# IamJerryXu/Multimodal-Diagnosis-HAM-Spine

Hardware: AMD Instinct MI355X
Metric: training images/sec, ResNet50+BERT-base 224px bs32 (higher is better)
Workload: dtype bf16; 1 GPU; C2: ResNet50 + BERT-base(L=128) + cross-attention FusionModule + MLP head, 224x224, batch 32 per GPU, CE(label_smoothing=0.02), fused AdamW, train-mode BatchNorm and dropout; per_gpu_batch=32, global_batch=32, seq_len=128, params=134897991, parallelism=dp1

## Files before the change

### include/hamspine.h

```cpp
#ifndef HAMSPINE_H
#define HAMSPINE_H

#include <stdint.h>

#ifdef __cplusplus
extern "C" {
#endif

typedef int hs_status;
enum { HS_OK = 0, HS_ERR_ARG = 1, HS_ERR_HIP = 2, HS_ERR_UNSUPPORTED = 3 };
enum { HS_F32 = 0, HS_BF16 = 1 };

const char* hs_last_error(void);
int hs_version(void);
int hs_device_ok(void);


enum {
    HS_A_KC = 0,
    HS_A_RC = 1,
    HS_A_CONV = 2,
    HS_A_DGRAD = 3
};
enum {
// ... 113 lines not shown
    const void* y;
    const void* x;
    const float* gamma;
    const float* save_mean;
    const float* save_invstd;
    void* dx;
    void* dres;
    float* dgamma;
    float* dbeta;
    void* ws;
    int64_t ws_bytes;
    const float* scale;
    const float* shift;
    int32_t partial_rows;
    int32_t sums_done;
} hs_bn_bwd_params;

hs_status hs_batchnorm_fwd(const hs_bn_params* p, void* stream);
hs_status hs_batchnorm_bwd(const hs_bn_bwd_params* p, void* stream);
int64_t hs_batchnorm_ws_bytes(int64_t M, int32_t C, int32_t dtype);

hs_status hs_layernorm_fwd(int32_t dtype, const void* x, const float* gamma, const float* beta, void* y,
                           float* mean, float* rstd, int64_t M, int32_t H, float eps, void* stream);
hs_status hs_layernorm_bwd(int32_t dtype, const void* dy, const void* x, const float* gamma, const float* mean,
                           const float* rstd, void* dx, float* dgamma, float* dbeta, void* ws, int64_t ws_bytes,
                           int64_t M, int32_t H, void* stream);
hs_status hs_layernorm_bwd_pre(int32_t dtype, const void* dy, const void* x, const float* gamma, const float* mean,
                               const float* rstd, void* dx, float* dgamma, float* dbeta, void* dx_dropped, float* dbias,
                               float dropout_p, uint64_t seed, void* ws, int64_t ws_bytes, int64_t M, int32_t H, void* stream);
int64_t hs_layernorm_bwd_ws_bytes(int64_t M, int32_t H);

#define HS_CAST_MAX 48
#define HS_ADAM_MAX 32

hs_status hs_maxpool_fwd(int32_t dtype, const void* x, void* y, void* idx, int32_t N, int32_t H, int32_t W, int32_t C,
                         int32_t ksize, int32_t stride, int32_t pad, void* stream);
hs_status hs_maxpool_bwd(int32_t dtype, const void* dy, const void* idx, void* dx, int32_t N, int32_t H, int32_t W,
                         int32_t C, int32_t ksize, int32_t stride, int32_t pad, void* stream);
hs_status hs_mean_tokens_fwd(int32_t dtype, const void* x, void* y, int32_t B, int32_t Nt, int32_t H, int32_t out_f32,
                             void* stream);
hs_status hs_mean_tokens_bwd(int32_t dtype, const void* dy, void* dx, int32_t B, int32_t Nt, int32_t H, int32_t dy_f32,
                             void* stream);
hs_status hs_pack_image(int32_t dtype, const float* x, void* y, int32_t N, int32_t Cin, int32_t H, int32_t W, int32_t Hp,
                        int32_t Wp, int32_t pad, void* stream);
hs_status hs_pack_stem_weight(int32_t dtype, const float* w, void* out, int32_t K, int32_t R, int32_t S, int32_t Cin,
                              void* stream);
hs_status hs_unpack_stem_wgrad(const float* g, float* dw, int32_t K, int32_t R, int32_t S, int32_t Cin, void* stream);
hs_status hs_cast_f32_to_bf16_multi(int32_t count, const float* const* src, void* const* dst, const int64_t* n,
                                    void* stream);
hs_status hs_transpose_bf16(const void* src, void* dst, int32_t R, int32_t C, int64_t ld_src, int64_t ld_dst, void* stream);
#define HS_TRANSPOSE_MAX 8
hs_status hs_transpose_bf16_multi(int32_t count, const void* const* src, void* const* dst, const int32_t* R, const int32_t* C,
                                  const int64_t* ld_src, const int64_t* ld_dst, void* stream);
hs_status hs_axpby(int32_t in_dtype, int32_t out_dtype, const void* x, const void* y, void* out, int64_t n, float a,
                   float b, void* stream);
hs_status hs_dropout(int32_t dtype, const void* x, void* out, int64_t n, float p, uint64_t seed, void* stream);
hs_status hs_relu_fwd(int32_t dtype, const void* x, void* out, int64_t n, void* stream);
hs_status hs_relu_bwd(int32_t dtype, const void* dy, const void* y, void* dx, int64_t n, void* stream);
hs_status hs_gelu_bwd(int32_t dtype, const void* dy, const void* u, void* dx, int64_t n, void* stream);
hs_status hs_mul_dev_scalar(const float* x, const float* scalar, float* out, int64_t n, void* stream);
hs_status hs_colsum(int32_t dtype, const void* x, int64_t M, int32_t N, int32_t ld, float* out, void* ws,
                    int64_t ws_bytes, int32_t accumulate, void* stream);
int64_t hs_colsum_ws_bytes(int64_t M, int32_t N);
hs_status hs_softmax_fwd(int32_t dtype, const float* S, const int64_t* mask, void* P, void* P_drop, int64_t rows,
                         int32_t Lk, int32_t ldS, int32_t ldP, int32_t rows_per_batch, float dropout_p, uint64_t seed,
                         void* stream);
hs_status hs_softmax_bwd(int32_t dtype, const float* dP, const void* P, void* dS, int64_t rows, int32_t Lk, int32_t ldG,
                         int32_t ldP, float dropout_p, uint64_t seed, void* stream);
hs_status hs_bert_embed_fwd(int32_t dtype, const int64_t* ids, const float* word, const float* pos, const float* type0,
                            const float* gamma, const float* beta, void* sum_out, void* y, float* mean, float* rstd,
                            int64_t tokens, int32_t L, int32_t H, int32_t V, float eps, float dropout_p, uint64_t seed,
                            void* stream);
hs_status hs_bert_embed_bwd(int32_t dtype, const int64_t* ids, const void* dsum, float* dword, float* dpos, int32_t B,
                            int32_t L, int32_t H, int32_t V, int32_t pad_id, void* stream);
hs_status hs_cross_entropy(const float* logits, const int64_t* labels, const float* weight, float label_smoothing,
                           int32_t B, int32_t C, float* loss, float* dlogits, float* row_loss, void* stream);
hs_status hs_adam_step_multi(int32_t count, float* const* params, const float* const* grads, float* const* exp_avg,
                             float* const* exp_avg_sq, const int64_t* n, float lr, float beta1, float beta2, float eps,
                             float weight_decay, int32_t step, int32_t decoupled, float grad_scale, void* stream);
hs_status hs_adam_step_multi_shadow(int32_t count, float* const* params, const float* const* grads, float* const* exp_avg,
                                    float* const* exp_avg_sq, void* const* bf16_shadow, const int64_t* n, float lr, float beta1,
                                    float beta2, float eps, float weight_decay, int32_t step, int32_t decoupled,
                                    float grad_scale, void* stream);
hs_status hs_wgrad_group_begin(void* stream);
hs_status hs_wgrad_group_end(void* stream);
hs_status hs_weight_shadow_set(const float* w, void* bf16);
void hs_weight_shadow_clear(void);

hs_status hs_sgd_step_multi(int32_t count, float* const* params, const float* const* grads, float* const* momentum_buf,
                            const int64_t* n, float lr, float momentum, float weight_decay, int32_t nesterov, int32_t first,
                            float grad_scale, void* stream);

#define HS_MUON_MAX 32
#define HS_MUON_PARTIALS 256
hs_status hs_muon_prepare_multi(int32_t dtype, int32_t count, float* const* momentum, const float* const* grads,
                                void* const* packed, const int32_t* rows, const int32_t* cols, float beta, float* partials,
                                void* stream);
hs_status hs_muon_orthogonalize(int32_t dtype, int32_t count, int32_t rows, int32_t cols, void* X, void* ws, int64_t ws_bytes,
                                void* stream);
int64_t hs_muon_ws_bytes(int32_t dtype, int32_t count, int32_t rows, int32_t cols);
hs_status hs_muon_apply_multi(int32_t dtype, int32_t count, float* const* params, void* const* bf16_shadow,
                              const void* const* packed, const int32_t* rows, const int32_t* cols, const float* scale,
                              float lr, float weight_decay, void* stream);

hs_status hs_select_token_fwd(int32_t dtype, const void* x, float* out, int32_t B, int32_t Nt, int32_t H, int32_t t,
                              void* stream);
// ... 120 lines not shown
hs_status hs_kan_features_fwd(const float* x, const float* grid, float* feat, int64_t B, int32_t in_f, int32_t grid_size,
                              int32_t order, int32_t base_act, void* stream);
hs_status hs_kan_features_bwd(const float* x, const float* grid, const float* dfeat, float* dx, int64_t B, int32_t in_f,
                              int32_t grid_size, int32_t order, int32_t base_act, void* stream);
hs_status hs_kan_pack_weight(const float* base_w, const float* spline_w, const float* scaler, float* wcat, int32_t out_f,
                             int32_t in_f, int32_t nb, void* stream);
hs_status hs_kan_unpack_wgrad(const float* dwcat, const float* spline_w, const float* scaler, float* d_base, float* d_spline,
                              float* d_scaler, int32_t out_f, int32_t in_f, int32_t nb, void* stream);
hs_status hs_moe_gate_fwd(const float* clean, const float* raw_noise, const float* noise, int32_t B, int32_t E, int32_t k, int32_t noisy,
                          float noise_eps, uint64_t seed, float coef, float* gates, float* p, int32_t* top, float* z,
                          float* sigma, float* loadrow, float* loss, float* d_imp, float* d_load, void* stream);
hs_status hs_moe_gate_bwd(const float* clean, const float* raw_noise, const float* p, const int32_t* top, const float* z,
                          const float* sigma, const float* dgates, const float* g_loss, const float* d_imp,
                          const float* d_load, int32_t B, int32_t E, int32_t k, int32_t noisy, float* d_clean, float* d_raw,
                          void* stream);
hs_status hs_moe_combine_fwd(const float* gates, const float* const* outs, float* y, int32_t B, int32_t E, int32_t O,
                             void* stream);
hs_status hs_moe_combine_bwd(const float* gates, const float* const* outs, const float* dy, float* const* douts,
                             float* dgates, int32_t B, int32_t E, int32_t O, void* stream);

int32_t hs_pointwise_stat_rows(int64_t M, int32_t N, int32_t K);
hs_status hs_pointwise_fwd(const void* x, int64_t M, int32_t K, int32_t ldx, const void* w, int32_t N, void* y, int32_t ldy,
                           float* stats, void* stream);

hs_status hs_moe_dispatch_index(const float* gates, int32_t B, int32_t E, int32_t* idx, int32_t* count, void* stream);
hs_status hs_rows_gather(const float* src, const int32_t* idx, float* dst, int32_t n, int32_t D, void* stream);
hs_status hs_rows_scatter_add(float* dst, const int32_t* idx, const float* scale, int32_t ld_scale, int32_t col, const float* src,
                              int32_t n, int32_t D, void* stream);
hs_status hs_rows_scatter_add_bwd(const float* dy, const int32_t* idx, const float* gates, int32_t E, int32_t col, const float* src,
                                  float* dsrc, float* dgates, int32_t n, int32_t D, void* stream);


typedef struct hs_attn_desc {
    int32_t dtype;
    int32_t B, H, Lq, Lk, hd;
    int64_t q_bs, k_bs, v_bs, o_bs;
    int32_t q_ld, k_ld, v_ld, o_ld;
    float scale;
    float dropout_p;
    uint64_t seed;
    const int64_t* key_mask;
} hs_attn_desc;
hs_status hs_attention_query(const hs_attn_desc* d, int64_t* saved_bytes, int64_t* ws_bytes);
hs_status hs_attention_fwd(const hs_attn_desc* d, const void* q, const void* k, const void* v, void* o, void* saved,
                           int64_t saved_bytes, void* ws, int64_t ws_bytes, void* stream);
hs_status hs_attention_bwd(const hs_attn_desc* d, const void* q, const void* k, const void* v, const void* d_o, void* dq,
                           void* dk, void* dv, void* saved, int64_t saved_bytes, void* ws, int64_t ws_bytes,
                           void* stream);

void hs_set_overlap(int32_t on);
hs_status hs_grad_milestones(int32_t n, const void* const* grad_ptrs, void* const* events);
int32_t hs_measure_build(void);
void hs_set_wgrad_nt(int32_t on);

typedef struct hs_conv_bn {
    int32_t Cin, Cout, R, stride, pad;
    const float* w;
    const float* gamma;
    const float* beta;
    float* running_mean;
    float* running_var;
    float* dw;
    float* dgamma;
    float* dbeta;
} hs_conv_bn;

typedef struct hs_resblock_desc {
    int32_t dtype;
    int32_t N, H, W;
    int32_t training;
    float eps, momentum;
    int32_t n_main;
    hs_conv_bn main[3];
    int32_t has_ds;
    hs_conv_bn ds;
    int32_t inference;
} hs_resblock_desc;
hs_status hs_resblock_query(const hs_resblock_desc* d, int64_t* saved_bytes, int64_t* ws_bytes);
hs_status hs_resblock_fwd(const hs_resblock_desc* d, const void* x, void* y, void* saved, int64_t saved_bytes, void* ws,
                          int64_t ws_bytes, void* stream);
hs_status hs_resblock_bwd(const hs_resblock_desc* d, const void* x, const void* y, const void* dy, void* dx, void* saved,
                          int64_t saved_bytes, void* ws, int64_t ws_bytes, void* stream);

typedef struct hs_stem_desc {
    int32_t dtype;
    int32_t N, H, W;
    int32_t training;
    float eps, momentum;
    hs_conv_bn cb;
    int32_t inference;
} hs_stem_desc;
hs_status hs_stem_query(const hs_stem_desc* d, int64_t* saved_bytes, int64_t* ws_bytes);
hs_status hs_stem_fwd(const hs_stem_desc* d, const float* image, void* y, void* saved, int64_t saved_bytes, void* ws,
                      int64_t ws_bytes, void* stream);
hs_status hs_stem_bwd(const hs_stem_desc* d, const void* y, const void* dy, void* saved, int64_t saved_bytes, void* ws,
                      int64_t ws_bytes, void* stream);

typedef struct hs_linear {
    int32_t in_f, out_f;
    const float* w;
    const float* b;
    float* dw;
    float* db;
} hs_linear;
typedef struct hs_norm {
    const float* gamma;
// ... 98 lines not shown
```

### multimodal-diagnosis-ham-spine_amd/hamspine/_lib.py

```python
import ctypes as C
import os
import re

_HERE = os.path.dirname(os.path.abspath(__file__))
LIB_PATH = os.path.join(_HERE, "libhamspine_hip.so")
HEADER_PATH = os.path.normpath(os.path.join(_HERE, "..", "..", "include", "hamspine.h"))

HS_OK = 0
HS_F32, HS_BF16 = 0, 1
A_KC, A_RC, A_CONV, A_DGRAD = 0, 1, 2, 3
B_KC, B_RC, B_WDGRAD, B_CONV = 0, 1, 2, 3
ACT_NONE, ACT_RELU, ACT_GELU = 0, 1, 2
MUL_NONE, MUL_GELU_GRAD, MUL_RELU_MASK = 0, 1, 2
CAST_MAX, ADAM_MAX = 48, 32
MUON_MAX, MUON_PARTIALS = 32, 256

i32, i64, u64, f32, vp = C.c_int32, C.c_int64, C.c_uint64, C.c_float, C.c_void_p


class HamspineError(RuntimeError):
    pass


class ConvGeom(C.Structure):
# ... 242 lines not shown
    l.hs_selective_scan_ws_bytes.argtypes = [i32, i32, i32]
    l.hs_selective_scan_ws_bytes.restype = i64
    l.hs_selective_scan_chunk_len.argtypes = []
    l.hs_selective_scan_chunk_len.restype = i32
    l.hs_selective_scan_chunk_len_n.argtypes = [i32]
    l.hs_selective_scan_chunk_len_n.restype = i32
    l.hs_selective_scan_ws_bytes_n.argtypes = [i32, i32, i32, i32]
    l.hs_selective_scan_ws_bytes_n.restype = i64
    l.hs_selective_scan_chunk_len_nogate.argtypes = [i32]
    l.hs_selective_scan_chunk_len_nogate.restype = i32
    l.hs_selective_scan_ws_bytes_nogate.argtypes = [i32, i32, i32, i32]
    l.hs_selective_scan_ws_bytes_nogate.restype = i64
    l.hs_conv1d_same_silu_fwd.argtypes = [i32, vp, i32, vp, vp, vp, i32, i32, i32, i32, i32, vp]
    l.hs_conv1d_same_silu_bwd.argtypes = [i32, vp, i32, vp, i32, vp, vp, vp, i32, vp, vp, vp, i64, i32, i32, i32, i32, vp]
    l.hs_conv1d_same_silu_ws_bytes.argtypes = [i32, i32]
    l.hs_conv1d_same_silu_ws_bytes.restype = i64
    l.hs_window_partition.argtypes = [i32, vp, vp, i32, i32, i32, i32, i32, vp]
    l.hs_window_reverse.argtypes = [i32, vp, vp, i32, i32, i32, i32, i32, vp]
    l.hs_conv3x3_fwd.argtypes = [i32, vp, vp, vp, vp, i32, i32, i32, i32, i32, i32, i32, i32, vp]
    l.hs_conv3x3_dgrad.argtypes = [i32, vp, vp, vp, i32, i32, i32, i32, i32, i32, i32, i32, vp]
    l.hs_conv3x3_pack_filter.argtypes = [i32, vp, vp, vp, i32, i32, i32, i32, vp]
    l.hs_conv3x3_unpack_wgrad.argtypes = [vp, vp, i32, i32, i32, vp]
    l.hs_pack_image_nhwc.argtypes = [i32, vp, vp, i32, i32, i32, i32, i32, vp]
    l.hs_unpack_image_nhwc.argtypes = [i32, vp, vp, i32, i32, i32, i32, i32, vp]
    l.hs_bn_gelu_tanh_fwd.argtypes = [i32, vp, vp, vp, vp, i64, i32, i32, vp]
    l.hs_bn_scale_residual_fwd.argtypes = [i32, vp, vp, vp, vp, vp, vp, vp, i64, i32, i32, i64, vp]
    l.hs_bn_epilogue_bwd.argtypes = [i32, i32, vp, vp, vp, vp, vp, vp, vp, vp, vp, vp, vp, vp, vp, vp, i32, i64, i32, i32, i64, vp, i64, vp]
    l.hs_bn_epilogue_ws_bytes.argtypes = [i64, i32]
    l.hs_bn_epilogue_ws_bytes.restype = i64
    l.hs_window_partition_nhwc.argtypes = [i32, vp, vp, i32, i32, i32, i32, i32, i32, vp]
    l.hs_window_reverse_nhwc.argtypes = [i32, vp, vp, i32, i32, i32, i32, i32, i32, vp]
    l.hs_add_token_bias_fwd.argtypes =[i32, vp, vp, vp, i32, i32, i32, vp]
    l.hs_add_token_bias_bwd.argtypes = [i32, vp, vp, i32, i32, i32, vp]
    l.hs_token_seq_assemble_fwd.argtypes = [vp, vp, vp, vp, vp, vp, i32, i32, i32, vp]
    l.hs_token_seq_assemble_bwd.argtypes = [vp, vp, vp, vp, vp, i32, i32, i32, vp]
    l.hs_transpose_batched_f32.argtypes = [vp, vp, i32, i32, i32, vp]
    l.hs_concat2_t.argtypes = [i32, vp, i32, vp, i32, vp, i64, vp]
    l.hs_split2_t.argtypes = [i32, vp, vp, i32, vp, i32, i64, vp]
    l.hs_prof_calibrate.argtypes = [vp, i32, C.POINTER(C.c_float)]
    l.hs_tta_expand.argtypes = [vp, vp, i64, i32, i32, P(i32), i32, vp]
    l.hs_group_mean.argtypes = [vp, vp, i32, i64, vp]
    l.hs_repeat.argtypes = [i32, vp, vp, i64, i32, vp]
    l.hs_gradcam.argtypes = [i32, vp, vp, vp, i32, i32, i32, vp]
    l.hs_stage_images_u8.argtypes = [vp, vp, i32, i32, i32, P(f32), P(f32), vp]
    l.hs_set_overlap.restype = None
    l.hs_grad_milestones.argtypes = [i32, P(vp), P(vp)]
    l.hs_pointwise_stat_rows.argtypes = [i64, i32, i32]
    l.hs_pointwise_stat_rows.restype = i32
    l.hs_pointwise_fwd.argtypes = [vp, i64, i32, i32, vp, i32, vp, i32, vp, vp]
    l.hs_measure_build.argtypes = []
    l.hs_measure_build.restype = i32
    l.hs_set_wgrad_nt.argtypes = [i32]
    l.hs_set_wgrad_nt.restype = None
    l.hs_bert_pack_rows_available.argtypes = []
    l.hs_bert_pack_rows_available.restype = i32
    l.hs_dwconv_ws_bytes.argtypes = [i32] * 5
    l.hs_dwconv_ws_bytes.restype = i64
    l.hs_dwconv_fwd.argtypes = [i32, vp, vp, vp, vp, i32, i32, i32, i32, i32, vp, i64, vp]
    l.hs_dwconv_bwd.argtypes = [i32, vp, vp, vp, vp, vp, vp, i32, i32, i32, i32, i32, vp, i64, vp]
    l.hs_layerscale_fwd.argtypes = [i32, vp, vp, vp, i32, vp, vp, i64, i32, vp]
    l.hs_layerscale_bwd.argtypes = [i32, vp, vp, vp, vp, i32, vp, vp, vp, i64, i64, i32, vp]
    l.hs_layerscale_ws_bytes.argtypes = [i64, i32]
    l.hs_layerscale_ws_bytes.restype = i64
    l.hs_patchify_fwd.argtypes = [i32, vp, vp, i32, i32, i32, i32, i32, i32, vp]
    l.hs_patchify_bwd.argtypes = [i32, vp, vp, i32, i32, i32, i32, i32, i32, vp]


ABI_STRUCTS = None


def abi_structs():
    return [(0, ConvGeom), (1, GemmParams), (2, BnParams), (3, BnBwdParams), (4, AttnDesc), (5, ConvBn), (6, ResblockDesc),
            (7, StemDesc), (8, Linear), (9, Norm), (10, BertLayerDesc), (11, ResnetDesc), (12, ResnetPlan), (13, BertDesc)]


def check(status, what=""):
    if status != HS_OK:
        msg = lib().hs_last_error().decode("utf-8", "replace")
        raise HamspineError(f"{what} failed (status {status}): {msg}")


def exported_symbols():
    txt = open(HEADER_PATH).read()
    txt = re.sub(r"/\*.*?\*/", "", txt, flags=re.S)
    return sorted(set(re.findall(r"\b(hs_[a-z0-9_]+)\s*\(", txt)))
```

### multimodal-diagnosis-ham-spine_amd/hamspine/csrc/blocks.hip

```cpp
#include <algorithm>
#include <mutex>
#include <unordered_map>
#include <vector>
#include <stdlib.h>
#include "hs_common.h"
#include "pw_stream.h"

namespace hs {

__global__ __launch_bounds__(256) void gather3_kernel(const float* __restrict__ a, const float* __restrict__ b,
                                                      const float* __restrict__ c, float* __restrict__ dst, int n) {
    const int i = blockIdx.x * 256 + threadIdx.x;
    if (i >= 3 * n) return;
    const int w = i / n, k = i - w * n;
    dst[i] = w == 0 ? a[k] : (w == 1 ? b[k] : c[k]);
}

int gemm_impl(const hs_gemm_params* p, hipStream_t stream);
int gemm_stat_rows(const hs_gemm_params* p);
int gemm_bn_finish_rows(const hs_gemm_params* p);
int gemm_tile_rows(const hs_gemm_params* p);
int gemm_bnb_finish_rows(const hs_gemm_params* p);
void gemm_group_set_immediate_hook(int (*fn)(void*), void* ctx);
struct GemmGroup;
GemmGroup* gemm_group_open(hipStream_t s, long long slot);
int gemm_group_add(GemmGroup* g, const hs_gemm_params* p, hipStream_t s);
int gemm_group_flush(GemmGroup* g, hipStream_t s);
bool fused_attention_enabled();
int attention_bwd_fused(const hs_attn_desc& d, const void* q, const void* k, const void* v, const void* dO, void* dq, void* dk,
                        void* dv, const void* P, int ldP, void* scratch, long long scratch_bytes, const void* O, hipStream_t s,
                        const int* cu);
int attention_fwd_fused(const hs_attn_desc& d, const void* q, const void* k, const void* v, void* o, void* P, void* Pd, int ldP,
                        hipStream_t s, const int* cu);
int ln_fwd(int dtype, const void* x, const float* gamma, const float* beta, void* y, float* mean, float* rstd, long long M, int H,
           float eps, hipStream_t s, const int* nrows);
int ln_bwd(int dtype, const void* dy, const void* x, const float* gamma, const float* mean, const float* rstd, void* dx, float* dgamma,
           float* dbeta, float* ws, long long ws_bytes, long long M, int H, hipStream_t s, const int* inv);
int ln_bwd_pre(int dtype, const void* dy, const void* x, const float* gamma, const float* mean, const float* rstd, void* dx,
               float* dgamma, float* dbeta, void* dx_dropped, float* dbias, float p, unsigned long long seed, float* ws,
               long long ws_bytes, long long M, int H, hipStream_t s, const int* inv);
int transpose_bf16_multi_rows(int count, const void* const* src, void* const* dst, const int32_t* R, const int32_t* Cc,
                              const int64_t* ld_src, const int64_t* ld_dst, const int* inv, const unsigned char* tok, hipStream_t stream);
int colsum_rows(int dtype, const void* x, long long M, int N, int ld, float* out, void* ws, long long ws_bytes, int accumulate,
                const int* inv, hipStream_t s);
int dropout_rows(int dtype, const void* x, void* out, long long M, int H, float p, unsigned long long seed, const int* nrows,
                 const int* row_of, hipStream_t s);
long long bert_row_map_bytes(int B, int L);
int bert_row_map(const int64_t* mask, int B, int L, int* map, hipStream_t s);
int bert_unpack_rows(const void* y, void* out, long long rows, long long row_bytes, const int* packed_of, hipStream_t s);
int bert_pack_rows(const void* dy, void* dst, long long rows, long long row_bytes, const int* nrows, const int* row_of,
                   hipStream_t s);
int bert_embed_fwd_rows(int dtype, const int64_t* ids, const float* word, const float* pos, const float* type0, const float* gamma,
                        const float* beta, void* sum_out, void* y, float* mean, float* rstd, long long tokens, int L, int H, int V,
                        float eps, float dropout_p, unsigned long long seed, const int* nrows, const int* row_of, hipStream_t stream);
int bert_embed_bwd_rows(int dtype, const int64_t* ids, const void* dsum, float* dword, float* dpos, int B, int L, int H, int V,
                        int pad_id, const int* nrows, const int* row_of, const int* packed_of, hipStream_t s);

static inline long long align_up(long long v, long long a) { return (v + a - 1) / a * a; }
static inline int esize(int dt) { return dt == HS_BF16 ? 2 : 4; }

struct Arena {
    char* base = nullptr;
    long long cap = 0, off = 0, peak = 0;
    bool plan = false;
    bool overflow = false;
    void* alloc(long long bytes) {
        bytes = align_up(bytes > 0 ? bytes : 1, 256);
        char* p = base ? base + off : nullptr;
        off += bytes;
        if (off > peak) peak = off;
        if (!plan && off > cap) overflow = true;
        return plan ? nullptr : p;
    }
    long long mark() const { return off; }
    void release(long long m) { off = m; }
};

struct Run {
    hipStream_t s;
    int dt;
    bool plan;
    Arena saved, ws;
    hipStream_t side = nullptr;
    bool side_used = false;
    bool defer_wgrad = false;
    GemmGroup *grp_pw = nullptr, *grp_conv = nullptr;
    bool group_nt = false;
    GemmGroup* grp_nt = nullptr;
    GemmGroup* tower_grp = nullptr;
    struct PendTr { const void* src; void* dst; int R, C; long long ld; bool tok; };
    std::vector<PendTr> pend_tr;
    const int *pk_T = nullptr, *pk_cu = nullptr, *pk_row = nullptr, *pk_inv = nullptr;
};

static hipStream_t g_side_stream[16] = {};
static hipEvent_t g_events[16][64] = {};
static int g_event_next[16] = {};
static std::mutex g_side_mu;
static int g_overlap = -1;
static bool overlap_enabled() {
    if (g_overlap < 0) {
        const char* e = getenv("HAMSPINE_OVERLAP");
        g_overlap = (e && e[0] == '1') ? 1 : 0;
    }
    return g_overlap == 1;
}
static int side_setup(Run& r) {
    if (r.plan || !overlap_enabled()) return HS_OK;
    int dev = 0;
    HS_CHECK_HIP(hipGetDevice(&dev));
    if (dev < 0 || dev >= 16) return HS_OK;
    std::lock_guard<std::mutex> lk(g_side_mu);
    if (!g_side_stream[dev]) HS_CHECK_HIP(hipStreamCreateWithFlags(&g_side_stream[dev], hipStreamNonBlocking));
    r.side = g_side_stream[dev];
    return HS_OK;
}
static int next_event(hipEvent_t* ev) {
    int dev = 0;
    HS_CHECK_HIP(hipGetDevice(&dev));
    std::lock_guard<std::mutex> lk(g_side_mu);
    int& n = g_event_next[dev & 15];
    hipEvent_t& e = g_events[dev & 15][n];
    n = (n + 1) & 63;
    if (!e) HS_CHECK_HIP(hipEventCreateWithFlags(&e, hipEventDisableTiming));
    *ev = e;
    return HS_OK;
}
template <typename F>
static int on_side(Run& r, F fn) {
    if (r.plan || !r.side) return fn();
    hipEvent_t ev;
    HS_PROPAGATE(next_event(&ev));
    HS_CHECK_HIP(hipEventRecord(ev, r.s));
    HS_CHECK_HIP(hipStreamWaitEvent(r.side, ev, 0));
    hipStream_t keep = r.s;
    r.s = r.side;
    const int st = fn();
    r.s = keep;
    r.side_used = true;
    return st;
}
static int side_join(Run& r) {
    if (r.plan || !r.side || !r.side_used) return HS_OK;
    hipEvent_t ev;
    HS_PROPAGATE(next_event(&ev));
// ... 240 lines not shown
    gk.b_elems = span_elems(d.B, d.q_bs, d.Lq, d.q_ld, d.H, d.hd);
    gk.lda = l.ldP; gk.ldb = d.q_ld;
    gk.batch = BH; gk.batch_inner = d.H;
    gk.a_bs0 = (long long)d.H * d.Lq * l.ldP; gk.a_bs1 = (long long)d.Lq * l.ldP;
    gk.b_bs0 = d.q_bs; gk.b_bs1 = d.hd;
    gk.d_bs0 = d.k_bs; gk.d_bs1 = d.hd;
    gk.D = dk; gk.ldd = d.k_ld;
    gk.alpha = d.scale;
    CALL(r, gemm_impl(&gk, r.s));
    RUN_CHECK_ARENAS(r, "attention_bwd");
    return HS_OK;
}

static int linear_fwd_run(Run& r, const void* x, long long M, int ldx, const hs_linear& lin, const void* w_c, void* y,
                          int ldy, int out_dtype, int act, void* preact, const void* residual, int ldr, float drop_p,
                          unsigned long long seed) {
    hs_gemm_params p = gemm_defaults(r.dt);
    p.a_kind = HS_A_KC; p.b_kind = HS_B_KC;
    p.M = (int)M; p.N = lin.out_f; p.K = lin.in_f;
    p.A = x; p.B = w_c;
    p.a_elems = (M - 1) * ldx + lin.in_f;
    p.b_elems = (long long)lin.out_f * lin.in_f;
    p.lda = ldx; p.ldb = lin.in_f;
    p.D = y; p.ldd = ldy; p.out_dtype = out_dtype;
    p.bias = lin.b;
    p.act = act;
    p.D_preact = preact;
    p.residual = residual; p.ldr = ldr;
    p.dropout_p = drop_p; p.dropout_seed = seed;
    p.m_rows = r.pk_T;
    p.drop_rows = drop_p > 0.f ? r.pk_row : nullptr;
    CALL(r, gemm_impl(&p, r.s));
    return HS_OK;
}
static bool fused_bias_grad_enabled() {
    static const bool on = [] {
        const char* e = getenv("HAMSPINE_FUSED_BIAS_GRAD");
        return !(e && e[0] == '0');
    }();
    return on;
}
static bool bias_in_wgrad(int dt, int out_f, int in_f, long long M) {
    return dt == HS_BF16 && fused_bias_grad_enabled() && hs_gemm_suggest_split(out_f, in_f, (int)M, dt) <= 1;
}
static std::mutex g_wg_mu;
static std::unordered_map<hipStream_t, GemmGroup*> g_wg_open;
static GemmGroup* open_wgrad_group(hipStream_t s) {
    std::lock_guard<std::mutex> lk(g_wg_mu);
    auto it = g_wg_open.find(s);
    return it == g_wg_open.end() ? nullptr : it->second;
}
static bool wgrad_nt_enabled();
static int linear_wgrad_nt_run(Run& r, const void* xT, const void* dyT, long long M, int in_f, int out_f, float* dw, float* db,
                               int seg_rows, float* const* dw_seg, float* const* db_seg);
static int linear_wgrad_run(Run& r, const void* x, long long M, int ldx, const hs_linear& lin, const void* dy, int ldy) {
    bool db_done = false;
    if (lin.dw && r.dt == HS_BF16 && wgrad_nt_enabled() && M >= 2048 && M % 8 == 0 && lin.in_f % 8 == 0 && lin.out_f % 8 == 0 &&
        ldx % 8 == 0 && ldy % 8 == 0 && ldx >= lin.in_f && ldy >= lin.out_f &&
        (long long)lin.in_f * lin.out_f >= 256ll * (lin.in_f + lin.out_f)) {
        const long long mk = r.ws.mark();
        char* tA = (char*)r.ws.alloc(M * (long long)lin.out_f * 2);
        char* tB = (char*)r.ws.alloc(M * (long long)lin.in_f * 2);
        const void* src[2] = {dy, x};
        void* dst[2] = {tA, tB};
        const int32_t R[2] = {(int32_t)M, (int32_t)M}, Cc[2] = {lin.out_f, lin.in_f};
        const int64_t lds[2] = {ldy, ldx}, ldd[2] = {M, M};
        const unsigned char tok[2] = {1, 1};
        CALLK(r, 4, transpose_bf16_multi_rows(2, src, dst, R, Cc, lds, ldd, r.pk_inv, tok, r.s));
        GemmGroup* og = r.plan ? nullptr : open_wgrad_group(r.s);
        const bool keep_flag = r.group_nt;
        GemmGroup* keep_grp = r.grp_nt;
        if (og) {
            r.group_nt = true;
            r.grp_nt = og;
        }
        const bool fused_b = lin.db && (r.group_nt || hs_gemm_suggest_split(lin.out_f, lin.in_f, (int)M, r.dt) <= 1) && fused_bias_grad_enabled();
        const int st_nt = linear_wgrad_nt_run(r, tB, tA, M, lin.in_f, lin.out_f, lin.dw, lin.db, 0, nullptr, nullptr);
        r.group_nt = keep_flag;
        r.grp_nt = keep_grp;
        HS_PROPAGATE(st_nt);
        if (lin.db && !fused_b) {
            const long long wsb = hs_colsum_ws_bytes(M, lin.out_f);
            void* w = r.ws.alloc(wsb);
            CALL(r, colsum_rows(r.dt, dy, M, lin.out_f, ldy, lin.db, w, wsb, 0, r.pk_inv, r.s));
        }
        if (!r.plan && !og && !r.side) r.ws.release(mk);
        return HS_OK;
    }
    if (lin.dw) {
        HS_REQUIRE(!r.pk_T, "linear_wgrad: packed rows need the transposed-operand weight gradients (HAMSPINE_WGRAD_NT)");
        hs_gemm_params p = gemm_defaults(r.dt);
        p.a_kind = HS_A_RC; p.b_kind = HS_B_RC;
        p.M = lin.out_f; p.N = lin.in_f; p.K = (int)M;
        p.A = dy; p.B = x;
        p.a_elems = (M - 1) * ldy + lin.out_f;
        p.b_elems = (M - 1) * ldx + lin.in_f;
        p.lda = ldy; p.ldb = ldx;
        p.D = lin.dw; p.ldd = lin.in_f; p.out_dtype = HS_F32;
        if (lin.db && bias_in_wgrad(r.dt, lin.out_f, lin.in_f, M)) {
            p.rowsum_a = lin.db;
            db_done = true;
        }
        HS_PROPAGATE(gemm_splitk(r, p));
    }
    if (lin.db && !db_done) {
        const long long mk = r.ws.mark();
        const long long wsb = hs_colsum_ws_bytes(M, lin.out_f);
        void* w = r.ws.alloc(wsb);
        CALL(r, colsum_rows(r.dt, dy, M, lin.out_f, ldy, lin.db, w, wsb, 0, r.pk_inv, r.s));
        if (r.plan ? !overlap_enabled() : !r.side) r.ws.release(mk);
    }
    return HS_OK;
}
static int g_wgrad_nt = -1;
static bool wgrad_nt_enabled() {
    if (g_wgrad_nt < 0) {
        const char* e = getenv("HAMSPINE_WGRAD_NT");
        g_wgrad_nt = (e && e[0] == '0') ? 0 : 1;
    }
    return g_wgrad_nt == 1;
}
static bool grouped_bert_wgrad_enabled() {
    static int v = -1;
    if (v < 0) {
        const char* e = getenv("HAMSPINE_GROUPED_BERT_WGRAD");
        v = (e && e[0] == '0') ? 0 : 1;
    }
    return v == 1;
}
static bool dgrad_nt_enabled() {
    static int v = -1;
    if (v < 0) {
        const char* e = getenv("HAMSPINE_DGRAD_NT");
        v = (e && e[0] == '0') ? 0 : 1;
    }
    return v == 1;
}
static bool deferred_transposes_enabled() {
    static const bool on = [] { const char* e = getenv("HAMSPINE_DEFER_TRANSPOSES"); return !(e && e[0] == '0'); }();
    return on;
}
static int transpose_run(Run& r, const void* src, void* dst, long long R, int Cc, int ld_src, bool for_grouped_wgrad = false,
                         bool tokens = false) {
    const bool tok = tokens && r.pk_T;
    if (for_grouped_wgrad && r.tower_grp && r.group_nt && !r.plan && deferred_transposes_enabled()) {
        r.pend_tr.push_back(Run::PendTr{src, dst, (int)R, Cc, ld_src, tok});
        return HS_OK;
    }
    if (tok) {
        const void* s1[1] = {src};
        void* d1[1] = {dst};
        const int32_t R1[1] = {(int32_t)R}, C1[1] = {Cc};
        const int64_t ls[1] = {ld_src}, ldst[1] = {R};
        const unsigned char t1[1] = {1};
        CALLK(r, 4, transpose_bf16_multi_rows(1, s1, d1, R1, C1, ls, ldst, r.pk_inv, t1, r.s));
        return HS_OK;
    }
    CALLK(r, 4, hs_transpose_bf16(src, dst, (int)R, Cc, ld_src, R, r.s));
    return HS_OK;
}
static int pending_transposes_flush(Run& r) {
    const int n = (int)r.pend_tr.size();
    if (n == 0) return HS_OK;
    std::vector<const void*> src(n);
    std::vector<void*> dst(n);
    std::vector<int32_t> R(n), Cc(n);
    std::vector<int64_t> lds(n), ldd(n);
    std::vector<unsigned char> tok(n);
    for (int i = 0; i < n; ++i) {
        src[i] = r.pend_tr[i].src; dst[i] = r.pend_tr[i].dst; R[i] = r.pend_tr[i].R; Cc[i] = r.pend_tr[i].C;
        lds[i] = r.pend_tr[i].ld; ldd[i] = r.pend_tr[i].R;
        tok[i] = r.pend_tr[i].tok ? 1 : 0;
    }
    r.pend_tr.clear();
    CALLK(r, 4, transpose_bf16_multi_rows(n, src.data(), dst.data(), R.data(), Cc.data(), lds.data(), ldd.data(), r.pk_inv, tok.data(), r.s));
    return HS_OK;
}
static int linear_wgrad_nt_run(Run& r, const void* xT, const void* dyT, long long M, int in_f, int out_f, float* dw, float* db,
                               int seg_rows, float* const* dw_seg, float* const* db_seg) {
    hs_gemm_params p = gemm_defaults(r.dt);
    p.a_kind = HS_A_KC; p.b_kind = HS_B_KC;
    p.M = out_f; p.N = in_f; p.K = (int)M;
    p.A = dyT; p.B = xT;
    p.a_elems = (long long)out_f * M;
    p.b_elems = (long long)in_f * M;
    p.lda = (int)M; p.ldb = (int)M;
    p.D = dw; p.ldd = in_f; p.out_dtype = HS_F32;
    if (seg_rows > 0) {
        p.seg_rows = seg_rows;
        p.D_seg[0] = dw_seg[0];
        p.D_seg[1] = dw_seg[1];
    }
    if (db && (r.group_nt || hs_gemm_suggest_split(out_f, in_f, (int)M, r.dt) <= 1) && fused_bias_grad_enabled()) {
        p.rowsum_a = db;
        if (seg_rows > 0) {
            p.rowsum_seg[0] = db_seg[0];
            p.rowsum_seg[1] = db_seg[1];
        }
    }
    if (r.group_nt) {
        if (!r.plan && !(knock() & 2)) HS_PROPAGATE(gemm_group_add(r.grp_nt, &p, r.s));
        return HS_OK;
    }
    if (!r.plan && (knock() & 2)) { const int sp = hs_gemm_suggest_split(p.M, p.N, p.K, p.dtype); p.split_k = sp; if (sp > 1) (void)r.ws.alloc(hs_gemm_splitk_ws_bytes(&p)); return HS_OK; }
    return gemm_splitk(r, p);
}
static int linear_dgrad_run(Run& r, const hs_linear& lin, const void* w_c, const void* dy, long long M, int ldy, void* dx,
                            int lddx, int dx_dtype, int mul_mode, const void* mul_src, int ldm, const void* residual,
                            const void* w_t = nullptr) {
    hs_gemm_params p = gemm_defaults(r.dt);
    p.a_kind = HS_A_KC; p.b_kind = HS_B_RC;
    p.M = (int)M; p.N = lin.in_f; p.K = lin.out_f;
    p.A = dy; p.B = w_c;
    p.a_elems = (M - 1) * ldy + lin.out_f;
    p.b_elems = (long long)lin.out_f * lin.in_f;
    p.lda = ldy; p.ldb = lin.in_f;
    long long mk = -1;
    if (!w_t && r.dt == HS_BF16 && dgrad_nt_enabled() && lin.out_f >= 1536 && M >= 2048 && lin.in_f % 8 == 0 && lin.out_f % 8 == 0) {
        mk = r.ws.mark();
        char* wt = (char*)r.ws.alloc((long long)lin.in_f * lin.out_f * 2);
        HS_PROPAGATE(transpose_run(r, w_c, wt, lin.out_f, lin.in_f, lin.in_f));
        w_t = wt;
    }
    if (w_t) {
        p.b_kind = HS_B_KC;
        p.B = w_t;
        p.ldb = lin.out_f;
    }
    p.D = dx; p.ldd = lddx; p.out_dtype = dx_dtype;
    p.mul_mode = mul_mode; p.mul_src = mul_src; p.ldm = ldm;
    p.residual = residual; p.ldr = lddx;
    p.m_rows = r.pk_T;
    CALLK(r, 1024, gemm_impl(&p, r.s));
    if (mk >= 0 && (r.plan ? !overlap_enabled() : !r.side)) r.ws.release(mk);
    return HS_OK;
}

struct ConvShape {
    int N, H, W, Cin, Cout, R, stride, pad, P, Q;
};
static ConvShape conv_shape(int N, int H, int W, const hs_conv_bn& c) {
    ConvShape s;
    s.N = N; s.H = H; s.W = W; s.Cin = c.Cin; s.Cout = c.Cout; s.R = c.R; s.stride = c.stride; s.pad = c.pad;
    s.P = (H + 2 * c.pad - c.R) / c.stride + 1;
    s.Q = (W + 2 * c.pad - c.R) / c.stride + 1;
    return s;
}
static hs_conv_geom geom_of(const ConvShape& s) {
    hs_conv_geom g;
    memset(&g, 0, sizeof(g));
    g.N = s.N; g.H = s.H; g.W = s.W; g.C = s.Cin; g.P = s.P; g.Q = s.Q; g.K = s.Cout; g.R = s.R; g.S = s.R;
    g.stride = s.stride; g.pad = s.pad;
    g.row_pitch = s.W * s.Cin;
    g.img_pitch = s.H * g.row_pitch;
// ... 680 lines not shown
    CALL(r, ln_fwd(r.dt, L.h2, d.ln2.gamma, d.ln2.beta, y, L.mean2, L.rstd2, M, Hd, d.ln_eps, r.s, r.pk_T));
    RUN_CHECK_ARENAS(r, "bert_layer_fwd");
    return HS_OK;
}
static int bert_layer_bwd_run(Run& r, const hs_bert_layer_desc& d, const void* x, const void* dy, void* dx) {
    BertLayout L;
    HS_PROPAGATE(bert_layout(r, d, L));
    const int Hd = d.hidden, I = d.inter;
    const long long M = (long long)d.B * d.L;
    const int es = esize(r.dt);
    hs_attn_desc a = bert_attn_desc(d, r.dt);
    void* dh2 = r.ws.alloc(M * Hd * es);
    void* dd2 = r.ws.alloc(M * Hd * es);
    void* dh1 = r.ws.alloc(M * Hd * es);
    void* dd1 = r.ws.alloc(M * Hd * es);
    void* du = r.ws.alloc(M * I * es);
    void* dx1 = r.ws.alloc(M * Hd * es);
    void* dctx = r.ws.alloc(M * Hd * es);
    void* dqkv = r.ws.alloc(M * 3 * Hd * es);
    const long long ln_ws_bytes = hs_layernorm_bwd_ws_bytes(M, Hd);
    float* ln_ws = (float*)r.ws.alloc(ln_ws_bytes);
    float* scratch = (float*)r.ws.alloc(2ll * Hd * 4);
    HS_PROPAGATE(side_setup(r));

    const bool fuse_ln = fused_ln_bwd_enabled();
    const void* g2 = d.hidden_dropout > 0.f ? dd2 : dh2;
    hs_linear out_l_w = d.out_l;
    if (fuse_ln) {
        CALL(r, ln_bwd_pre(r.dt, dy, L.h2, d.ln2.gamma, L.mean2, L.rstd2, dh2, d.ln2.dgamma ? d.ln2.dgamma : scratch,
                           d.ln2.dbeta ? d.ln2.dbeta : (scratch ? scratch + Hd : nullptr),
                           d.hidden_dropout > 0.f ? dd2 : nullptr, d.out_l.db, d.hidden_dropout, d.seed * 8 + 3,
                           ln_ws, ln_ws_bytes, M, Hd, r.s, r.pk_inv));
        out_l_w.db = nullptr;
    } else {
        CALLK(r, 128, ln_bwd(r.dt, dy, L.h2, d.ln2.gamma, L.mean2, L.rstd2, dh2, d.ln2.dgamma ? d.ln2.dgamma : scratch,
                             d.ln2.dbeta ? d.ln2.dbeta : (scratch ? scratch + Hd : nullptr), ln_ws, ln_ws_bytes, M, Hd, r.s, r.pk_inv));
        if (d.hidden_dropout > 0.f && r.pk_T) CALL(r, dropout_rows(r.dt, dh2, dd2, M, Hd, d.hidden_dropout, d.seed * 8 + 3, r.pk_T, r.pk_row, r.s));
        else if (d.hidden_dropout > 0.f) CALL(r, hs_dropout(r.dt, dh2, dd2, M * Hd, d.hidden_dropout, d.seed * 8 + 3, r.s));
    }
    const bool nt = r.dt == HS_BF16 && wgrad_nt_enabled() && M % 8 == 0 && Hd % 8 == 0 && I % 8 == 0;
    HS_REQUIRE(!r.pk_T || nt, "bert_layer_bwd: packed rows need the transposed-operand weight gradients (bf16, HAMSPINE_WGRAD_NT on)");
    const long long big_tiles = (long long)ceil_div(3 * Hd, 256) * ceil_div(Hd, 128) + (long long)ceil_div(Hd, 256) * ceil_div(Hd, 128) +
                                (long long)ceil_div(I, 256) * ceil_div(Hd, 128) + (long long)ceil_div(Hd, 256) * ceil_div(I, 128);
    const bool grouped = nt && grouped_bert_wgrad_enabled() && !overlap_enabled() && big_tiles >= 128;
    char* tA = nt ? (char*)r.ws.alloc(M * (long long)std::max(3 * Hd, I) * 2) : nullptr;
    char* tA_ffn2 = grouped ? (char*)r.ws.alloc(M * (long long)Hd * 2) : tA;
    char* tA_ao = grouped ? (char*)r.ws.alloc(M * (long long)Hd * 2) : tA;
    char* tA_qkv = grouped ? (char*)r.ws.alloc(M * 3ll * Hd * 2) : tA;
    r.group_nt = grouped;
    if (grouped && !r.plan) {
        r.grp_nt = r.tower_grp ? r.tower_grp : gemm_group_open(r.s, (long long)(uintptr_t)d.q.w + 16);
        HS_REQUIRE(r.grp_nt != nullptr, "bert_layer_bwd: cannot set up the grouped weight-gradient launch");
    }
    char* tX_g = nt ? (char*)r.ws.alloc(M * (long long)I * 2) : nullptr;
    char* tX_x1 = nt ? (char*)r.ws.alloc(M * (long long)Hd * 2) : nullptr;
    char* tX_ctx = nt ? (char*)r.ws.alloc(M * (long long)Hd * 2) : nullptr;
    char* tX_x = nt ? (char*)r.ws.alloc(M * (long long)Hd * 2) : nullptr;
    auto bias_by_colsum = [&](const hs_linear& lin, const void* dy_rm, int ldy) -> int {
        hs_linear only_b = lin;
        only_b.dw = nullptr;
        return linear_wgrad_run(r, nullptr, M, 0, only_b, dy_rm, ldy);
    };
    auto wgrad = [&](const void* x_rm, const void* xT, int in_f, const hs_linear& lin, const void* dy_rm, int ldy, char* tAk) -> int {
        if (!nt || !lin.dw) {
            const bool keep = r.group_nt;
            r.group_nt = false;
            const int st = linear_wgrad_run(r, x_rm, M, in_f, lin, dy_rm, ldy);
            r.group_nt = keep;
            return st;
        }
        HS_PROPAGATE(transpose_run(r, dy_rm, tAk, M, lin.out_f, ldy, true, true));
        const bool fused_b = lin.db && (r.group_nt || hs_gemm_suggest_split(lin.out_f, in_f, (int)M, r.dt) <= 1) && fused_bias_grad_enabled();
        HS_PROPAGATE(linear_wgrad_nt_run(r, xT, tAk, M, in_f, lin.out_f, lin.dw, lin.db, 0, nullptr, nullptr));
        if (lin.db && !fused_b) HS_PROPAGATE(bias_by_colsum(lin, dy_rm, ldy));
        return HS_OK;
    };
    const bool dnt = r.dt == HS_BF16 && dgrad_nt_enabled() && Hd % 8 == 0 && I % 8 == 0;
    char* wo_t = dnt ? (char*)r.ws.alloc((long long)Hd * I * 2) : nullptr;
    char* wi_t = dnt ? (char*)r.ws.alloc((long long)Hd * I * 2) : nullptr;
    char* wqkv_t = dnt ? (char*)r.ws.alloc(3ll * Hd * Hd * 2) : nullptr;
    {
        const void* src[7];
        void* dst[7];
        int32_t R[7], Cc[7];
        int64_t lds[7], ldd[7];
        unsigned char tok[7];
        int n = 0;
        auto add = [&](const void* s_, void* d_, long long rows, int cols, bool tokens = false) {
            src[n] = s_; dst[n] = d_; R[n] = (int32_t)rows; Cc[n] = cols; lds[n] = cols; ldd[n] = rows; tok[n] = tokens ? 1 : 0;
            ++n;
        };
        if (nt) {
            add(L.g, tX_g, M, I, true);
            add(L.x1, tX_x1, M, Hd, true);
            add(L.ctx, tX_ctx, M, Hd, true);
            add(x, tX_x, M, Hd, true);
        }
        if (dnt) {
            add(L.wo, wo_t, Hd, I);
            add(L.wi, wi_t, I, Hd);
            add(L.wqkv, wqkv_t, 3 * Hd, Hd);
        }
        if (n > 0) CALLK(r, 4, transpose_bf16_multi_rows(n, src, dst, R, Cc, lds, ldd, r.pk_inv, tok, r.s));
    }
    HS_PROPAGATE(on_side(r, [&]() { return wgrad(L.g, tX_g, I, out_l_w, g2, Hd, tA_ffn2); }));
    HS_PROPAGATE(linear_dgrad_run(r, d.out_l, L.wo, g2, M, Hd, du, I, r.dt, HS_MUL_GELU_GRAD, L.u, I, nullptr, wo_t));
    HS_PROPAGATE(on_side(r, [&]() { return wgrad(L.x1, tX_x1, Hd, d.inter_l, du, I, tA); }));
    HS_PROPAGATE(linear_dgrad_run(r, d.inter_l, L.wi, du, M, I, dx1, Hd, r.dt, HS_MUL_NONE, nullptr, 0, dh2, wi_t));
    const void* g1 = d.hidden_dropout > 0.f ? dd1 : dh1;
    hs_linear ao_w = d.ao;
    if (fuse_ln) {
        CALL(r, ln_bwd_pre(r.dt, dx1, L.h1, d.ln1.gamma, L.mean1, L.rstd1, dh1, d.ln1.dgamma ? d.ln1.dgamma : scratch,
                           d.ln1.dbeta ? d.ln1.dbeta : (scratch ? scratch + Hd : nullptr),
                           d.hidden_dropout > 0.f ? dd1 : nullptr, d.ao.db, d.hidden_dropout, d.seed * 8 + 2,
                           ln_ws, ln_ws_bytes, M, Hd, r.s, r.pk_inv));
        ao_w.db = nullptr;
    } else {
        CALLK(r, 128, ln_bwd(r.dt, dx1, L.h1, d.ln1.gamma, L.mean1, L.rstd1, dh1, d.ln1.dgamma ? d.ln1.dgamma : scratch,
                             d.ln1.dbeta ? d.ln1.dbeta : (scratch ? scratch + Hd : nullptr), ln_ws, ln_ws_bytes, M, Hd, r.s, r.pk_inv));
        if (d.hidden_dropout > 0.f && r.pk_T) CALL(r, dropout_rows(r.dt, dh1, dd1, M, Hd, d.hidden_dropout, d.seed * 8 + 2, r.pk_T, r.pk_row, r.s));
        else if (d.hidden_dropout > 0.f) CALL(r, hs_dropout(r.dt, dh1, dd1, M * Hd, d.hidden_dropout, d.seed * 8 + 2, r.s));
    }
    HS_PROPAGATE(on_side(r, [&]() { return wgrad(L.ctx, tX_ctx, Hd, ao_w, g1, Hd, tA_ao); }));
    HS_PROPAGATE(linear_dgrad_run(r, d.ao, L.wao, g1, M, Hd, dctx, Hd, r.dt, HS_MUL_NONE, nullptr, 0, nullptr));
    const char* qkv = (const char*)L.qkv;
    char* dq = (char*)dqkv;
    HS_PROPAGATE(attention_bwd_run(r, a, qkv, qkv ? qkv + (long long)Hd * es : nullptr, qkv ? qkv + 2ll * Hd * es : nullptr,
                                   dctx, dq, dq ? dq + (long long)Hd * es : nullptr, dq ? dq + 2ll * Hd * es : nullptr, L.ctx));
    HS_PROPAGATE(on_side(r, [&]() -> int {
        const bool fused = d.q.dw && d.k.dw && d.v.dw;
        if (fused && nt) {
            HS_PROPAGATE(transpose_run(r, dqkv, tA_qkv, M, 3 * Hd, 3 * Hd, true, true));
            const bool bias_too = d.q.db && d.k.db && d.v.db && (r.group_nt || hs_gemm_suggest_split(3 * Hd, Hd, (int)M, r.dt) <= 1) &&
                                  fused_bias_grad_enabled();
            float* dws[2] = {d.k.dw, d.v.dw};
            float* dbs[2] = {d.k.db, d.v.db};
            HS_PROPAGATE(linear_wgrad_nt_run(r, tX_x, tA_qkv, M, Hd, 3 * Hd, d.q.dw, bias_too ? d.q.db : nullptr, Hd, dws, dbs));
            if (bias_too) return HS_OK;
            const hs_linear* lins[3] = {&d.q, &d.k, &d.v};
            for (int i = 0; i < 3; ++i) HS_PROPAGATE(bias_by_colsum(*lins[i], dq ? dq + (long long)i * Hd * es : nullptr, 3 * Hd));
            return HS_OK;
        }
        if (fused) {
            hs_gemm_params p = gemm_defaults(r.dt);
            p.a_kind = HS_A_RC; p.b_kind = HS_B_RC;
            p.M = 3 * Hd; p.N = Hd; p.K = (int)M;
            p.A = dqkv; p.B = x;
            p.a_elems = M * 3 * Hd;
            p.b_elems = M * Hd;
            p.lda = 3 * Hd; p.ldb = Hd;
            p.D = d.q.dw; p.ldd = Hd; p.out_dtype = HS_F32;
            p.seg_rows = Hd;
            p.D_seg[0] = d.k.dw;
            p.D_seg[1] = d.v.dw;
            const bool bias_too = d.q.db && d.k.db && d.v.db && bias_in_wgrad(r.dt, 3 * Hd, Hd, M);
            if (bias_too) {
                p.rowsum_a = d.q.db;
                p.rowsum_seg[0] = d.k.db;
                p.rowsum_seg[1] = d.v.db;
            }
            HS_PROPAGATE(gemm_splitk(r, p));
            if (bias_too) return HS_OK;
        }
        const hs_linear* lins[3] = {&d.q, &d.k, &d.v};
        for (int i = 0; i < 3; ++i) {
            hs_linear li = *lins[i];
            if (fused) li.dw = nullptr;
            HS_PROPAGATE(linear_wgrad_run(r, x, M, Hd, li, dq ? dq + (long long)i * Hd * es : nullptr, 3 * Hd));
        }
        return HS_OK;
    }));
    if (dx) {
        hs_linear qkv_lin;
        memset(&qkv_lin, 0, sizeof(qkv_lin));
        qkv_lin.in_f = Hd; qkv_lin.out_f = 3 * Hd;
        HS_PROPAGATE(linear_dgrad_run(r, qkv_lin, L.wqkv, dqkv, M, 3 * Hd, dx, Hd, r.dt, HS_MUL_NONE, nullptr, 0, dh1, wqkv_t));
    }
    if (r.group_nt && !r.plan && !r.tower_grp) HS_PROPAGATE(gemm_group_flush(r.grp_nt, r.s));
    r.group_nt = false;
    HS_PROPAGATE(side_join(r));
    RUN_CHECK_ARENAS(r, "bert_layer_bwd");
    return HS_OK;
}


static long long out_bytes_of(const hs_resblock_desc& d, int dt, int* Cout, int* Ho, int* Wo) {
    int H = d.H, W = d.W;
    for (int i = 0; i < d.n_main; ++i) {
        const hs_conv_bn& c = d.main[i];
        H = (H + 2 * c.pad - c.R) / c.stride + 1;
        W = (W + 2 * c.pad - c.R) / c.stride + 1;
    }
    const int C = d.main[d.n_main - 1].Cout;
    if (Cout) *Cout = C;
    if (Ho) *Ho = H;
    if (Wo) *Wo = W;
    return (long long)d.N * H * W * C * esize(dt);
}
struct ResnetLayout {
    long long y_off[HS_RESNET_MAX_BLOCKS + 1];
    long long lay_off[HS_RESNET_MAX_BLOCKS + 1];
    long long y_bytes[HS_RESNET_MAX_BLOCKS + 1];
    long long max_act = 0;
};
static int resnet_check(const hs_resnet_desc& d) {
    HS_REQUIRE(d.n_blocks >= 1 && d.n_blocks <= HS_RESNET_MAX_BLOCKS, "resnet: n_blocks %d out of range", d.n_blocks);
    HS_REQUIRE(d.n_taps >= 1 && d.n_taps <= HS_RESNET_MAX_TAPS, "resnet: n_taps %d out of range", d.n_taps);
    for (int t = 0; t < d.n_taps; ++t)
        HS_REQUIRE(d.tap_block[t] >= 0 && d.tap_block[t] < d.n_blocks && (t == 0 || d.tap_block[t] > d.tap_block[t - 1]),
                   "resnet: tap blocks must be ascending block indices");
    HS_REQUIRE(d.tap_block[d.n_taps - 1] == d.n_blocks - 1, "resnet: the last tap must be the last block");
    for (int i = 0; i < d.n_blocks; ++i)
        HS_REQUIRE(d.blocks[i].dtype == d.stem.dtype && d.blocks[i].N == d.stem.N, "resnet: block %d dtype / batch mismatch", i);
    return HS_OK;
}
static int resnet_fwd_run(Run& r, const hs_resnet_desc& d, const float* image, ResnetLayout& lo) {
    const int dt = d.stem.dtype;
    const int es = esize(dt);
    const int P = (d.stem.H + 6 - 7) / 2 + 1, Q = (d.stem.W + 6 - 7) / 2 + 1;
    const int P2 = (P + 2 - 3) / 2 + 1, Q2 = (Q + 2 - 3) / 2 + 1;
    lo.y_off[0] = r.saved.mark();
    lo.y_bytes[0] = (long long)d.stem.N * P2 * Q2 * d.stem.cb.Cout * es;
    lo.max_act = lo.y_bytes[0];
    char* x = (char*)r.saved.alloc(lo.y_bytes[0]);
    lo.lay_off[0] = r.saved.mark();
    long long wm = r.ws.mark();
    HS_PROPAGATE(stem_fwd_run(r, d.stem, image, x));
    r.ws.release(wm);
    HS_REQUIRE(d.blocks[0].H == P2 && d.blocks[0].W == Q2 && d.blocks[0].main[0].Cin == d.stem.cb.Cout,
               "resnet: block 0 does not take the stem's output shape");
    int C = d.stem.cb.Cout, H = P2, W = Q2;
    for (int i = 0; i < d.n_blocks; ++i) {
// ... 85 lines not shown
        HS_PROPAGATE(resblock_bwd_run(r, d.blocks[i], x, y, dy, dx, nb, own_next.rows > 0 ? &own_next : nullptr));
        own_next = OwnSums{};
        if (nb && xs_rows > 0) own_next = OwnSums{xs_buf[i & 1], xs_bytes, xs_rows, xs_done};
        if (!r.defer_wgrad) r.ws.release(wm);
        if (staged) {
            const hs_resblock_desc& bd = d.blocks[i];
            for (int k = 0; k < bd.n_main; ++k) {
                seg_ptrs.push_back(bd.main[k].dw); seg_ptrs.push_back(bd.main[k].dgamma); seg_ptrs.push_back(bd.main[k].dbeta);
            }
            if (bd.has_ds) {
                seg_ptrs.push_back(bd.ds.dw); seg_ptrs.push_back(bd.ds.dgamma); seg_ptrs.push_back(bd.ds.dbeta);
            }
            if (bd.has_ds && i > 0) {
                HS_PROPAGATE(gemm_group_flush(r.grp_pw, r.s));
                HS_PROPAGATE(gemm_group_flush(r.grp_conv, r.s));
                HS_PROPAGATE(milestones_hit(r, seg_ptrs.data(), (int)seg_ptrs.size()));
                seg_ptrs.clear();
                ++seg;
                r.grp_pw = gemm_group_open(r.s, 8 + 2 * seg);
                r.grp_conv = gemm_group_open(r.s, 9 + 2 * seg);
                HS_REQUIRE(r.grp_pw && r.grp_conv, "resnet_bwd: cannot set up the grouped weight-gradient launches");
            }
        }
        dy = dx;
        cur ^= 1;
    }
    if (r.defer_wgrad && !r.plan) {
        HS_PROPAGATE(gemm_group_flush(r.grp_pw, r.s));
        HS_PROPAGATE(gemm_group_flush(r.grp_conv, r.s));
    }
    r.defer_wgrad = false;
    const hs_conv_bn& cb = d.stem.cb;
    if (cb.dw || cb.dgamma || cb.dbeta) {
        r.saved.off = lo.lay_off[0];
        const long long wm = r.ws.mark();
        HS_PROPAGATE(stem_bwd_run(r, d.stem, r.saved.base ? r.saved.base + lo.y_off[0] : nullptr, dy));
        r.ws.release(wm);
    }
    return milestones_flush(r);
}

struct BertTowerLayout {
    long long ssum_off, stats_off;
    long long y_off[HS_BERT_MAX_LAYERS + 1], lay_off[HS_BERT_MAX_LAYERS + 1];
    long long act_bytes;
    long long map_off, out_off;
};
static void bert_pack_pointers(Run& r, const hs_bert_desc& d, const BertTowerLayout& lo) {
    const int* map = (const int*)(r.saved.base + lo.map_off);
    r.pk_T = map;
    r.pk_cu = map + 4;
    r.pk_row = r.pk_cu + (d.B + 1 + 3) / 4 * 4;
    r.pk_inv = r.pk_row + (long long)d.B * d.L;
}
static int bert_check(const hs_bert_desc& d) {
    HS_REQUIRE(d.n_layers >= 0 && d.n_layers <= HS_BERT_MAX_LAYERS, "bert: n_layers %d out of range", d.n_layers);
    HS_REQUIRE(d.B > 0 && d.L > 0 && d.hidden > 0 && d.vocab > 0, "bert: bad dims");
    HS_REQUIRE(d.word && d.pos && d.type0 && d.gamma && d.beta, "bert: null embedding parameter");
    for (int i = 0; i < d.n_layers; ++i)
        HS_REQUIRE(d.layers[i].dtype == d.dtype && d.layers[i].B == d.B && d.layers[i].L == d.L && d.layers[i].hidden == d.hidden,
                   "bert: layer %d shape mismatch", i);
    if (d.pack_rows) {
        HS_REQUIRE(d.dtype == HS_BF16 && d.L <= 128 && d.hidden % 8 == 0 && ((long long)d.B * d.L) % 8 == 0, "bert: pack_rows needs bf16, L <= 128 and hidden %% 8 == 0");
        for (int i = 0; i < d.n_layers; ++i) {
            const hs_bert_layer_desc& l = d.layers[i];
            HS_REQUIRE(l.heads > 0 && d.hidden == 64 * l.heads && l.inter % 8 == 0, "bert: pack_rows needs head dim 64 (layer %d)", i);
            const int wanted = (l.q.dw != nullptr) + (l.k.dw != nullptr) + (l.v.dw != nullptr);
            HS_REQUIRE(wanted == 0 || wanted == 3, "bert: pack_rows needs the q / k / v weight gradients of layer %d all wanted or all frozen", i);
        }
    }
    return HS_OK;
}
static hs_bert_layer_desc bert_layer_of(const hs_bert_desc& d, int i, const int64_t* mask) {
    hs_bert_layer_desc l = d.layers[i];
    l.attention_mask = mask;
    l.seed = d.seed + 16ull * (unsigned)(i + 1);
    return l;
}
static int bert_fwd_run(Run& r, const hs_bert_desc& d, const int64_t* ids, const int64_t* mask, BertTowerLayout& lo) {
    const long long M = (long long)d.B * d.L;
    const int es = esize(d.dtype);
    lo.act_bytes = M * d.hidden * es;
    lo.map_off = lo.out_off = 0;
    char* out_pad = nullptr;
    if (d.pack_rows) {
        HS_REQUIRE(r.plan || mask, "bert_fwd: pack_rows needs an attention mask");
        lo.map_off = r.saved.mark();
        int* map = (int*)r.saved.alloc(bert_row_map_bytes(d.B, d.L));
        lo.out_off = r.saved.mark();
        out_pad = (char*)r.saved.alloc(lo.act_bytes);
        if (!r.plan) {
            RUN_CHECK_ARENAS(r, "bert_fwd(row map)");
            HS_PROPAGATE(bert_row_map(mask, d.B, d.L, map, r.s));
            bert_pack_pointers(r, d, lo);
        }
    }
    lo.ssum_off = r.saved.mark();
    void* ssum = r.saved.alloc(lo.act_bytes);
    lo.stats_off = r.saved.mark();
    float* stats = (float*)r.saved.alloc(2 * M * 4);
    lo.y_off[0] = r.saved.mark();
    char* x = (char*)r.saved.alloc(lo.act_bytes);
    lo.lay_off[0] = r.saved.mark();
    CALL(r, bert_embed_fwd_rows(d.dtype, ids, d.word, d.pos, d.type0, d.gamma, d.beta, ssum, x, stats, stats + M, M, d.L, d.hidden,
                                d.vocab, d.ln_eps, d.embed_dropout, d.seed, r.pk_T, r.pk_row, r.s));
    for (int i = 0; i < d.n_layers; ++i) {
        lo.y_off[i + 1] = r.saved.mark();
        char* y = (char*)r.saved.alloc(lo.act_bytes);
        lo.lay_off[i + 1] = r.saved.mark();
        const hs_bert_layer_desc l = bert_layer_of(d, i, mask);
        const long long wm = r.ws.mark();
        HS_PROPAGATE(bert_layer_fwd_run(r, l, x, y));
        r.ws.release(wm);
        x = y;
    }
    if (d.pack_rows) CALL(r, bert_unpack_rows(x, out_pad, M, (long long)d.hidden * es, r.pk_inv, r.s));
    return HS_OK;
}
static int bert_bwd_run(Run& r, const hs_bert_desc& d, const int64_t* ids, const int64_t* mask, const void* dy_in,
                        const BertTowerLayout& lo) {
    const long long M = (long long)d.B * d.L;
    const int Hd = d.hidden;
    char* dy_packed = d.pack_rows ? (char*)r.ws.alloc(lo.act_bytes) : nullptr;
    char* gbuf[2] = {(char*)r.ws.alloc(lo.act_bytes), (char*)r.ws.alloc(lo.act_bytes)};
    int cur = 0;
    const void* dy = dy_in;
    char* base = r.saved.base;
    if (d.pack_rows && !r.plan) {
        RUN_CHECK_ARENAS(r, "bert_bwd(row map)");
        bert_pack_pointers(r, d, lo);
        HS_PROPAGATE(bert_pack_rows(dy_in, dy_packed, M, (long long)Hd * esize(d.dtype), r.pk_T, r.pk_row, r.s));
        dy = dy_packed;
    }
    static const int span = [] { const char* e = getenv("HAMSPINE_WGRAD_LAYERS"); const int v = e ? atoi(e) : 2; return v >= 1 && v <= 8 ? v : 2; }();
    int pending = 0;
    long long wm = 0;
    const void* gps[8][16];
    struct HookGuard {
        explicit HookGuard(Run* rr) { gemm_group_set_immediate_hook([](void* c) -> int { return pending_transposes_flush(*(Run*)c); }, rr); }
        ~HookGuard() { gemm_group_set_immediate_hook(nullptr, nullptr); }
    } hook_guard(&r);
    for (int i = d.n_layers - 1; i >= 0; --i) {
        const hs_bert_layer_desc l = bert_layer_of(d, i, mask);
        char* dx = gbuf[cur];
        r.saved.off = lo.lay_off[i + 1];
        if (pending == 0) {
            wm = r.ws.mark();
            r.tower_grp = (span > 1 && !r.plan) ? gemm_group_open(r.s, (long long)(uintptr_t)l.q.w + 24) : nullptr;
        }
        HS_PROPAGATE(bert_layer_bwd_run(r, l, base ? base + lo.y_off[i] : nullptr, dy, dx));
        {
            const void* gp[16] = {l.q.dw, l.q.db, l.k.dw, l.k.db, l.v.dw, l.v.db, l.ao.dw, l.ao.db, l.ln1.dgamma, l.ln1.dbeta,
                                  l.inter_l.dw, l.inter_l.db, l.out_l.dw, l.out_l.db, l.ln2.dgamma, l.ln2.dbeta};
            memcpy(gps[pending], gp, sizeof(gp));
        }
        ++pending;
        if (pending == span || i == 0) {
            HS_PROPAGATE(pending_transposes_flush(r));
            if (r.tower_grp) HS_PROPAGATE(gemm_group_flush(r.tower_grp, r.s));
            r.tower_grp = nullptr;
            r.ws.release(wm);
            for (int k = 0; k < pending; ++k) HS_PROPAGATE(milestones_hit(r, gps[k], 16));
            pending = 0;
        }
        dy = dx;
        cur ^= 1;
    }
    const bool any = d.dword || d.dpos || d.dtype0 || d.dgamma || d.dbeta;
    if (!any) return milestones_flush(r);
    const void* g = dy;
    if (d.embed_dropout > 0.f) {
        char* gd = gbuf[cur];
        if (r.pk_T) CALL(r, dropout_rows(d.dtype, dy, gd, M, Hd, d.embed_dropout, d.seed, r.pk_T, r.pk_row, r.s));
        else CALL(r, hs_dropout(d.dtype, dy, gd, M * Hd, d.embed_dropout, d.seed, r.s));
        g = gd;
        cur ^= 1;
    }
    char* dsum = gbuf[cur];
    const long long lnb = hs_layernorm_bwd_ws_bytes(M, Hd);
    const long long csb = hs_colsum_ws_bytes(M, Hd);
    void* lnws = r.ws.alloc(lnb);
    void* csws = r.ws.alloc(csb);
    float* scratch = (float*)r.ws.alloc(2ll * Hd * 4);
    const float* stats = base ? (const float*)(base + lo.stats_off) : nullptr;
// ... 403 lines not shown
        HS_REQUIRE(pl.saved.peak <= saved_bytes && pl.ws.peak <= ws_bytes,
                   "bert_fwd: arena too small (saved %lld needed / %lld given, ws %lld needed / %lld given)", pl.saved.peak,
                   (long long)saved_bytes, pl.ws.peak, (long long)ws_bytes);
    }
    Run r;
    run_init(r, d->dtype, false, saved, saved_bytes, ws, ws_bytes, (hipStream_t)stream);
    HS_PROPAGATE(bert_fwd_run(r, *d, ids, mask, lo));
    RUN_CHECK_ARENAS(r, "bert_fwd");
    return HS_OK;
}
hs_status hs_bert_bwd(const hs_bert_desc* d, const int64_t* ids, const int64_t* mask, const void* dy, void* saved,
                      int64_t saved_bytes, void* ws, int64_t ws_bytes, void* stream) {
    HS_REQUIRE(d && ids && dy && saved && ws, "bert_bwd: null argument");
    HS_PROPAGATE(bert_check(*d));
    BertTowerLayout lo;
    {
        Run pl;
        run_init(pl, d->dtype, true, nullptr, 0, nullptr, 0, nullptr);
        HS_PROPAGATE(bert_fwd_run(pl, *d, nullptr, nullptr, lo));
        Run pb;
        run_init(pb, d->dtype, true, nullptr, 0, nullptr, 0, nullptr);
        HS_PROPAGATE(bert_bwd_run(pb, *d, nullptr, nullptr, nullptr, lo));
        HS_REQUIRE(pl.saved.peak <= saved_bytes && pb.ws.peak <= ws_bytes,
                   "bert_bwd: arena too small (saved %lld needed / %lld given, ws %lld needed / %lld given)", pl.saved.peak,
                   (long long)saved_bytes, pb.ws.peak, (long long)ws_bytes);
    }
    Run r;
    run_init(r, d->dtype, false, saved, saved_bytes, ws, ws_bytes, (hipStream_t)stream);
    HS_PROPAGATE(bert_bwd_run(r, *d, ids, mask, dy, lo));
    RUN_CHECK_ARENAS(r, "bert_bwd");
    return HS_OK;
}
void hs_set_overlap(int32_t on) { hs::g_overlap = on ? 1 : 0; }
int32_t hs_bert_pack_rows_available(void) { return (hs::wgrad_nt_enabled() && hs::fused_attention_enabled()) ? 1 : 0; }
hs_status hs_grad_milestones(int32_t n, const void* const* grad_ptrs, void* const* events) {
    HS_REQUIRE(n >= 0 && n <= kMaxMilestones, "grad_milestones: %d entries (max %d)", n, kMaxMilestones);
    HS_REQUIRE(n == 0 || (grad_ptrs && events), "grad_milestones: null argument");
    g_ms.n = n;
    for (int i = 0; i < n; ++i) {
        HS_REQUIRE(grad_ptrs[i] && events[i], "grad_milestones: null entry %d", i);
        g_ms.ptr[i] = grad_ptrs[i];
        g_ms.ev[i] = (hipEvent_t)events[i];
    }
    return HS_OK;
}
int32_t hs_measure_build(void) {
#ifdef HS_MEASURE
    return 1;
#else
    return 0;
#endif
}
void hs_set_wgrad_nt(int32_t on) { hs::g_wgrad_nt = on ? 1 : 0; }
}
```

### multimodal-diagnosis-ham-spine_amd/hamspine/csrc/elem.hip

```cpp
#include <algorithm>
#include "hs_common.h"

namespace hs {

static inline int grid_for(long long n, int cap = 4096) {
    long long b = (n + 255) / 256;
    if (b > cap) b = cap;
    if (b < 1) b = 1;
    return (int)b;
}

template <typename T>
__global__ __launch_bounds__(256) void maxpool_fwd_kernel(const T* __restrict__ x, T* __restrict__ y,
                                                          unsigned char* __restrict__ idx, int N, int H, int W, int C,
                                                          int P, int Q, int ks, int st, int pad) {
    constexpr int E = Chunk<T>::N;
    const int cg = C / E;
    const long long total = (long long)N * P * Q * cg;
    for (long long i = (long long)blockIdx.x * 256 + threadIdx.x; i < total; i += (long long)gridDim.x * 256) {
        const int c = (int)(i % cg);
        long long t = i / cg;
        const int q = (int)(t % Q);
        t /= Q;
        const int p = (int)(t % P);
// ... 643 lines not shown
        if (lane >= o) incl += up;
    }
    if (lane == 63) s_wave[wv] = incl;
    __syncthreads();
    int off = incl - c;
    for (int w = 0; w < wv; ++w) off += s_wave[w];
    const int n = s_wave[0] + s_wave[1] + s_wave[2] + s_wave[3];
    for (int i = lo; i < hi; ++i)
        if (id_at(i) == id) s_list[off++] = i;
    __syncthreads();
    if (s_list[0] != t) return;
    for (int h = threadIdx.x; h < H; h += 256) {
        float acc = 0.f;
        for (int k = 0; k < n; ++k) acc += to_f32(dsum[(long long)s_list[k] * H + h]);
        dword[id * H + h] = acc;
    }
}
template <typename T>
__global__ __launch_bounds__(256) void embed_word_bwd_atomic_kernel(const long long* __restrict__ ids,
                                                                    const T* __restrict__ dsum, float* __restrict__ dword,
                                                                    long long tokens_pad, int H, int V, int pad_id,
                                                                    const int* __restrict__ nrows, const int* __restrict__ row_of) {
    const long long total = packed_rows(nrows, tokens_pad) * H;
    for (long long i = (long long)blockIdx.x * 256 + threadIdx.x; i < total; i += (long long)gridDim.x * 256) {
        const long long t = i / H;
        const int h = (int)(i % H);
        long long srow = row_of ? (long long)row_of[t] : t;
        if (srow < 0 || srow >= tokens_pad) srow = t;
        const long long id = clamp_id(ids[srow], V);
        if (id == pad_id) continue;
        atomicAdd(dword + id * H + h, to_f32(dsum[i]));
    }
}
template <typename T>
__global__ __launch_bounds__(256) void embed_pos_bwd_kernel(const T* __restrict__ dsum, float* __restrict__ dpos, int B,
                                                            int L, int H, const int* __restrict__ packed_of) {
    const long long total = (long long)L * H;
    for (long long i = (long long)blockIdx.x * 256 + threadIdx.x; i < total; i += (long long)gridDim.x * 256) {
        float acc = 0.f;
        if (packed_of) {
            const int l = (int)(i / H), h = (int)(i - (long long)l * H);
            for (int b = 0; b < B; ++b) {
                const int pr = packed_of[(long long)b * L + l];
                if (pr >= 0 && pr < B * L) acc += to_f32(dsum[(long long)pr * H + h]);
            }
        } else {
            for (int b = 0; b < B; ++b) acc += to_f32(dsum[(long long)b * L * H + i]);
        }
        dpos[i] = acc;
    }
}

__global__ __launch_bounds__(256) void bert_row_map_kernel(const long long* __restrict__ mask, int B, int L, int* __restrict__ map) {
    int* cu = map + 4;
    int* row_of = cu + (B + 1 + 3) / 4 * 4;
    int* packed_of = row_of + (long long)B * L;
    const int lane = threadIdx.x & 63, wave = threadIdx.x >> 6;
    for (int b = wave; b < B; b += 4) {
        int n = 0;
        for (int l0 = 0; l0 < L; l0 += 64) {
            const int l = l0 + lane;
            const bool v = l < L && mask[(long long)b * L + l] != 0;
            n += __popcll(__ballot(v));
        }
        if (lane == 0) cu[b + 1] = n;
    }
    __syncthreads();
    if (threadIdx.x == 0) {
        int run = 0;
        cu[0] = 0;
        for (int b = 0; b < B; ++b) {
            run += cu[b + 1];
            cu[b + 1] = run;
        }
        map[0] = run;
        map[1] = map[2] = map[3] = 0;
    }
    __syncthreads();
    const int T = cu[B];
    for (int b = wave; b < B; b += 4) {
        int at = cu[b];
        for (int l0 = 0; l0 < L; l0 += 64) {
            const int l = l0 + lane;
            const bool v = l < L && mask[(long long)b * L + l] != 0;
            const unsigned long long bal = __ballot(v);
            const int before = __popcll(bal & ((1ull << lane) - 1ull));
            if (l < L) {
                if (v) {
                    row_of[at + before] = b * L + l;
                    packed_of[(long long)b * L + l] = at + before;
                } else {
                    packed_of[(long long)b * L + l] = -1;
                }
            }
            at += __popcll(bal);
        }
    }
    for (int t = T + (int)threadIdx.x; t < B * L; t += 256) row_of[t] = t;
}
__global__ __launch_bounds__(256) void bert_unpack_rows_kernel(const u32x4* __restrict__ y, u32x4* __restrict__ out, long long rows, int cpr,
                                                               const int* __restrict__ packed_of) {
    const long long total = rows * cpr;
    for (long long i = (long long)blockIdx.x * 256 + threadIdx.x; i < total; i += (long long)gridDim.x * 256) {
        const long long r = i / cpr;
        const int pr = packed_of[r];
        u32x4 v = {0u, 0u, 0u, 0u};
        if (pr >= 0 && pr < rows) v = y[(long long)pr * cpr + (i - r * cpr)];
        out[i] = v;
    }
}
__global__ __launch_bounds__(256) void bert_pack_rows_kernel(const u32x4* __restrict__ dy, u32x4* __restrict__ dst, long long rows, int cpr,
                                                             const int* __restrict__ nrows, const int* __restrict__ row_of) {
    const long long T = packed_rows(nrows, rows), total = T * cpr;
    for (long long i = (long long)blockIdx.x * 256 + threadIdx.x; i < total; i += (long long)gridDim.x * 256) {
        const long long t = i / cpr;
        long long srow = row_of[t];
        if (srow < 0 || srow >= rows) srow = t;
        dst[i] = dy[srow * cpr + (i - t * cpr)];
    }
}

__device__ __forceinline__ void transpose_bf16_tile(const unsigned short* __restrict__ src, unsigned short* __restrict__ dst,
                                                    int R, int Cc, long long lds_, long long ldd, int bx, int by,
                                                    unsigned (*tile)[33], const int* __restrict__ inv) {
    const int r0 = by * 64, c0 = bx * 64;
    for (int i = threadIdx.x; i < 512; i += 256) {
        const int r = i >> 3, ch = i & 7;
        u32x4 v = {0u, 0u, 0u, 0u};
        int sr = r0 + r;
        if (inv && sr < R) {
            sr = inv[sr];
            if (sr >= R) sr = -1;
        }
        if (sr >= 0 && sr < R && c0 + ch * 8 < Cc) v = *(const u32x4*)(src + (long long)sr * lds_ + c0 + ch * 8);
#pragma unroll
        for (int w = 0; w < 4; ++w) tile[r][(ch * 4 + w) ^ ((r >> 5) << 2)] = v[w];
    }
    __syncthreads();
    for (int i = threadIdx.x; i < 512; i += 256) {
        const int j = i >> 3, k = i & 7;
        if (c0 + j >= Cc || r0 + k * 8 >= R) continue;
        unsigned e[8];
#pragma unroll
        for (int q = 0; q < 8; ++q) {
            const unsigned w = tile[k * 8 + q][(j >> 1) ^ (((k * 8 + q) >> 5) << 2)];
            e[q] = (j & 1) ? (w >> 16) : (w & 0xffffu);
        }
        const u32x4 o = {e[0] | (e[1] << 16), e[2] | (e[3] << 16), e[4] | (e[5] << 16), e[6] | (e[7] << 16)};
        *(u32x4*)(dst + (long long)(c0 + j) * ldd + r0 + k * 8) = o;
    }
}
__global__ __launch_bounds__(256) void transpose_bf16_kernel(const unsigned short* __restrict__ src,
                                                             unsigned short* __restrict__ dst, int R, int Cc, long long lds_,
                                                             long long ldd) {
    __shared__ unsigned tile[64][33];
    transpose_bf16_tile(src, dst, R, Cc, lds_, ldd, blockIdx.x, blockIdx.y, tile, nullptr);
}
struct TransposeTable {
    const unsigned short* src[HS_TRANSPOSE_MAX];
    unsigned short* dst[HS_TRANSPOSE_MAX];
    int R[HS_TRANSPOSE_MAX], C[HS_TRANSPOSE_MAX];
    long long ld_src[HS_TRANSPOSE_MAX], ld_dst[HS_TRANSPOSE_MAX];
    int first[HS_TRANSPOSE_MAX + 1];
    int count;
    const int* inv;
    unsigned tok_mask;
};
__global__ __launch_bounds__(256) void transpose_bf16_multi_kernel(const TransposeTable t) {
    __shared__ unsigned tile[64][33];
    int e = 0;
    for (int i = 1; i < t.count; ++i) e += (int)blockIdx.x >= t.first[i];
    const int local = blockIdx.x - t.first[e];
    const int tx = (t.C[e] + 63) / 64;
    const int* inv = (t.inv && ((t.tok_mask >> e) & 1u)) ? t.inv : nullptr;
    transpose_bf16_tile(t.src[e], t.dst[e], t.R[e], t.C[e], t.ld_src[e], t.ld_dst[e], local % tx, local / tx, tile, inv);
}

__global__ __launch_bounds__(1024) void ce_kernel(const float* __restrict__ logits, const long long* __restrict__ labels,
                                                 const float* __restrict__ weight, float smoothing, int B, int C,
                                                 float* __restrict__ loss_out, float* __restrict__ dlogits,
                                                 float* __restrict__ row_loss) {
    __shared__ float s_num[16], s_den[16];
    const int lane = threadIdx.x & 63, wv = threadIdx.x >> 6, nwv = blockDim.x >> 6;
    float num = 0.f, den = 0.f;
    for (int r = wv; r < B; r += nwv) {
        const float* z = logits + (long long)r * C;
        float mx = -INFINITY;
        for (int c = lane; c < C; c += 64) mx = fmaxf(mx, z[c]);
        mx = wave_max(mx);
        float se = 0.f;
        for (int c = lane; c < C; c += 64) se += __expf(z[c] - mx);
        const float lse = mx + __logf(wave_sum(se));
        const int y = (int)labels[r];
        const float wy = weight ? weight[y] : 1.f;
        float sm = 0.f;
        for (int c = lane; c < C; c += 64) sm += (weight ? weight[c] : 1.f) * (lse - z[c]);
        sm = wave_sum(sm);
        const float l = (1.f - smoothing) * wy * (lse - z[y]) + smoothing / (float)C * sm;
        if (lane == 0 && row_loss) row_loss[r] = l;
        num += l;
        den += wy;
    }
    if (lane == 0) {
        s_num[wv] = num;
        s_den[wv] = den;
    }
    __syncthreads();
    float tn = 0.f, td = 0.f;
    for (int w = 0; w < nwv; ++w) {
        tn += s_num[w];
        td += s_den[w];
    }
    if (threadIdx.x == 0) loss_out[0] = tn / td;
    if (!dlogits) return;
    for (int r = wv; r < B; r += nwv) {
        const float* z = logits + (long long)r * C;
        float mx = -INFINITY;
        for (int c = lane; c < C; c += 64) mx = fmaxf(mx, z[c]);
        mx = wave_max(mx);
        float se = 0.f;
        for (int c = lane; c < C; c += 64) se += __expf(z[c] - mx);
        const float inv = 1.f / wave_sum(se);
        const int y = (int)labels[r];
        const float wy = weight ? weight[y] : 1.f;
        float wsum = 0.f;
        for (int c = lane; c < C; c += 64) wsum += weight ? weight[c] : 1.f;
        wsum = wave_sum(wsum);
        for (int c = lane; c < C; c += 64) {
// ... 155 lines not shown
    if (direct) return HS_OK;
    hipLaunchKernelGGL(colsum_final_kernel, dim3(ceil_div(N, 64)), dim3(256), 0, s, ws, gy, N, out, accumulate);
    HS_LAUNCH_CHECK();
    return HS_OK;
}

static inline int softmax_group(int Lk, int ldP) {
    if (Lk % 4 || ldP % 4 || ldP > 256) return 0;
    const int need = ldP / 4;
    return need <= 16 ? 16 : (need <= 32 ? 32 : 64);
}
template <typename T>
static int softmax_fwd_t(const float* S, const long long* mask, void* P, void* Pd, long long rows, int Lk, int ldS,
                         int ldP, int rpb, float p, unsigned long long seed, hipStream_t s) {
    HS_REQUIRE(Lk <= 64 * SM_MAXV && ldP <= 64 * SM_MAXV, "softmax: Lk=%d too long (max %d)", Lk, 64 * SM_MAXV);
    const unsigned th = p > 0.f ? dropout_thresh(p) : 0u;
    const float ik = p > 0.f ? 1.f / (1.f - p) : 1.f;
    const int G = (ldS % 4 == 0 && ((((uintptr_t)S) | ((uintptr_t)P) | ((uintptr_t)Pd)) & 15) == 0) ? softmax_group(Lk, ldP) : 0;
#define SM_FWD(GG)                                                                                                       \
    hipLaunchKernelGGL((softmax_fwd_vec_kernel<T, GG>), dim3(ceil_div(rows, 4 * (64 / GG))), dim3(256), 0, s, S, mask, (T*)P, \
                       (T*)Pd, rows, Lk, ldS, ldP, rpb, th, ik, seed)
    if (G == 16) SM_FWD(16);
    else if (G == 32) SM_FWD(32);
    else if (G == 64) SM_FWD(64);
    else
        hipLaunchKernelGGL(softmax_fwd_kernel<T>, dim3(ceil_div(rows, 4)), dim3(256), 0, s, S, mask, (T*)P, (T*)Pd, rows, Lk,
                           ldS, ldP, rpb, th, ik, seed);
#undef SM_FWD
    HS_LAUNCH_CHECK();
    return HS_OK;
}
template <typename T>
static int softmax_bwd_t(const float* dP, const void* P, void* dS, long long rows, int Lk, int ldG, int ldP, float p,
                         unsigned long long seed, hipStream_t s) {
    HS_REQUIRE(Lk <= 64 * SM_MAXV && ldP <= 64 * SM_MAXV, "softmax_bwd: Lk=%d too long", Lk);
    const unsigned th = p > 0.f ? dropout_thresh(p) : 0u;
    const float ik = p > 0.f ? 1.f / (1.f - p) : 1.f;
    const int G = (ldG % 4 == 0 && ((((uintptr_t)dP) | ((uintptr_t)P) | ((uintptr_t)dS)) & 15) == 0) ? softmax_group(Lk, ldP) : 0;
#define SM_BWD(GG)                                                                                                      \
    hipLaunchKernelGGL((softmax_bwd_vec_kernel<T, GG>), dim3(ceil_div(rows, 4 * (64 / GG))), dim3(256), 0, s, dP, (const T*)P, \
                       (T*)dS, rows, Lk, ldG, ldP, th, ik, seed)
    if (G == 16) SM_BWD(16);
    else if (G == 32) SM_BWD(32);
    else if (G == 64) SM_BWD(64);
    else
        hipLaunchKernelGGL(softmax_bwd_kernel<T>, dim3(ceil_div(rows, 4)), dim3(256), 0, s, dP, (const T*)P, (T*)dS, rows, Lk,
                           ldG, ldP, th, ik, seed);
#undef SM_BWD
    HS_LAUNCH_CHECK();
    return HS_OK;
}

int transpose_bf16_multi_rows(int count, const void* const* src, void* const* dst, const int32_t* R, const int32_t* Cc,
                              const int64_t* ld_src, const int64_t* ld_dst, const int* inv, const unsigned char* tok, hipStream_t stream) {
    HS_REQUIRE(count >= 0 && (count == 0 || (src && dst && R && Cc && ld_src && ld_dst)), "transpose_bf16_multi: bad argument");
    for (int base = 0; base < count; base += HS_TRANSPOSE_MAX) {
        TransposeTable t;
        memset(&t, 0, sizeof(t));
        t.count = std::min(HS_TRANSPOSE_MAX, count - base);
        int blocks = 0;
        for (int i = 0; i < t.count; ++i) {
            const int k = base + i;
            HS_REQUIRE(src[k] && dst[k] && R[k] > 0 && Cc[k] > 0 && R[k] % 8 == 0 && Cc[k] % 8 == 0 && ld_src[k] % 8 == 0 &&
                           ld_dst[k] % 8 == 0 && ld_src[k] >= Cc[k] && ld_dst[k] >= R[k] &&
                           (((uintptr_t)src[k] | (uintptr_t)dst[k]) & 15) == 0,
                       "transpose_bf16_multi: entry %d: dims / leading dimensions must be multiples of 8 and bases 16-byte aligned", k);
            t.src[i] = (const unsigned short*)src[k];
            t.dst[i] = (unsigned short*)dst[k];
            t.R[i] = R[k]; t.C[i] = Cc[k];
            t.ld_src[i] = ld_src[k]; t.ld_dst[i] = ld_dst[k];
            t.first[i] = blocks;
            blocks += ceil_div(Cc[k], 64) * ceil_div(R[k], 64);
            if (inv && tok && tok[k]) t.tok_mask |= 1u << i;
        }
        t.first[t.count] = blocks;
        t.inv = t.tok_mask ? inv : nullptr;
        hipLaunchKernelGGL(transpose_bf16_multi_kernel, dim3(blocks), dim3(256), 0, stream, t);
        HS_LAUNCH_CHECK();
    }
    return HS_OK;
}
int colsum_rows(int dtype, const void* x, long long M, int N, int ld, float* out, void* ws, long long ws_bytes, int accumulate,
                const int* inv, hipStream_t s) {
    HS_REQUIRE(x && out && M > 0 && N > 0, "colsum: bad argument");
    return DISPATCH_T(dtype, colsum_t, x, M, N, ld, out, (float*)ws, ws_bytes, accumulate, s, inv);
}
int dropout_rows(int dtype, const void* x, void* out, long long M, int H, float p, unsigned long long seed, const int* nrows,
                 const int* row_of, hipStream_t s) {
    HS_REQUIRE(x && out && nrows && row_of && p >= 0.f && p < 1.f, "dropout_rows: bad argument");
    HS_REQUIRE(H % 8 == 0 && al16(x, out), "dropout_rows: H %% 8 != 0 or unaligned base");
    const unsigned th = dropout_thresh(p);
    const float ik = 1.f / (1.f - p);
    if (dtype == HS_BF16)
        hipLaunchKernelGGL(dropout_rows_kernel<bf16_t>, dim3(grid_for(M * (H / 8))), dim3(256), 0, s, (const bf16_t*)x, (bf16_t*)out, M, H,
                           nrows, row_of, th, ik, seed);
    else
        hipLaunchKernelGGL(dropout_rows_kernel<float>, dim3(grid_for(M * (H / 4))), dim3(256), 0, s, (const float*)x, (float*)out, M, H,
                           nrows, row_of, th, ik, seed);
    HS_LAUNCH_CHECK();
    return HS_OK;
}
long long bert_row_map_bytes(int B, int L) { return (4ll + (B + 1 + 3) / 4 * 4 + 2ll * B * L) * 4; }
int bert_row_map(const int64_t* mask, int B, int L, int* map, hipStream_t s) {
    HS_REQUIRE(mask && map && B > 0 && L > 0, "bert_row_map: bad argument");
    hipLaunchKernelGGL(bert_row_map_kernel, dim3(1), dim3(256), 0, s, (const long long*)mask, B, L, map);
    HS_LAUNCH_CHECK();
    return HS_OK;
}
int bert_unpack_rows(const void* y, void* out, long long rows, long long row_bytes, const int* packed_of, hipStream_t s) {
    HS_REQUIRE(y && out && packed_of && row_bytes % 16 == 0 && al16(y, out), "bert_unpack_rows: bad argument");
    const int cpr = (int)(row_bytes / 16);
    hipLaunchKernelGGL(bert_unpack_rows_kernel, dim3(grid_for(rows * cpr)), dim3(256), 0, s, (const u32x4*)y, (u32x4*)out, rows, cpr, packed_of);
    HS_LAUNCH_CHECK();
    return HS_OK;
}
int bert_pack_rows(const void* dy, void* dst, long long rows, long long row_bytes, const int* nrows, const int* row_of,
                   hipStream_t s) {
    HS_REQUIRE(dy && dst && nrows && row_of && row_bytes % 16 == 0 && al16(dy, dst), "bert_pack_rows: bad argument");
    const int cpr = (int)(row_bytes / 16);
    hipLaunchKernelGGL(bert_pack_rows_kernel, dim3(grid_for(rows * cpr)), dim3(256), 0, s, (const u32x4*)dy, (u32x4*)dst, rows, cpr, nrows,
                       row_of);
    HS_LAUNCH_CHECK();
    return HS_OK;
}
int bert_embed_fwd_rows(int dtype, const int64_t* ids, const float* word, const float* pos, const float* type0, const float* gamma,
                        const float* beta, void* sum_out, void* y, float* mean, float* rstd, long long tokens, int L, int H, int V,
                        float eps, float dropout_p, unsigned long long seed, const int* nrows, const int* row_of, hipStream_t stream) {
    HS_REQUIRE(ids && word && pos && type0 && gamma && beta && sum_out && y && mean && rstd, "bert_embed: null argument");
    HS_REQUIRE(H % 4 == 0 && H <= 1024, "bert_embed: H=%d unsupported", H);
    const unsigned th = dropout_p > 0.f ? dropout_thresh(dropout_p) : 0u;
    const float ik = dropout_p > 0.f ? 1.f / (1.f - dropout_p) : 1.f;
    const dim3 g(ceil_div(tokens, 4)), b(256);
    if (dtype == HS_BF16)
        hipLaunchKernelGGL(embed_fwd_kernel<bf16_t>, g, b, 0, stream, (const long long*)ids, word, pos, type0,
                           gamma, beta, (bf16_t*)sum_out, (bf16_t*)y, mean, rstd, tokens, L, H, V, eps, th, ik, seed, nrows, row_of);
    else
        hipLaunchKernelGGL(embed_fwd_kernel<float>, g, b, 0, stream, (const long long*)ids, word, pos, type0,
                           gamma, beta, (float*)sum_out, (float*)y, mean, rstd, tokens, L, H, V, eps, th, ik, seed, nrows, row_of);
    HS_LAUNCH_CHECK();
    return HS_OK;
}
int bert_embed_bwd_rows(int dtype, const int64_t* ids, const void* dsum, float* dword, float* dpos, int B, int L, int H, int V,
                        int pad_id, const int* nrows, const int* row_of, const int* packed_of, hipStream_t s) {
    HS_REQUIRE(ids && dsum, "bert_embed_bwd: null argument");
    const long long tokens = (long long)B * L;
    if (dword) {
        const bool det = tokens <= 15360;
        const size_t lds = det ? (size_t)(tokens + 8) * sizeof(int) : 0;
        if (det && dtype == HS_BF16)
            hipLaunchKernelGGL(embed_word_bwd_kernel<bf16_t>, dim3((unsigned)tokens), dim3(256), lds, s, (const long long*)ids,
                               (const bf16_t*)dsum, dword, (int)tokens, H, V, pad_id, nrows, row_of);
        else if (det)
            hipLaunchKernelGGL(embed_word_bwd_kernel<float>, dim3((unsigned)tokens), dim3(256), lds, s, (const long long*)ids,
                               (const float*)dsum, dword, (int)tokens, H, V, pad_id, nrows, row_of);
        else if (dtype == HS_BF16)
            hipLaunchKernelGGL(embed_word_bwd_atomic_kernel<bf16_t>, dim3(grid_for(tokens * H)), dim3(256), 0, s,
                               (const long long*)ids, (const bf16_t*)dsum, dword, tokens, H, V, pad_id, nrows, row_of);
        else
            hipLaunchKernelGGL(embed_word_bwd_atomic_kernel<float>, dim3(grid_for(tokens * H)), dim3(256), 0, s,
                               (const long long*)ids, (const float*)dsum, dword, tokens, H, V, pad_id, nrows, row_of);
        HS_LAUNCH_CHECK();
    }
    if (dpos) {
        if (dtype == HS_BF16)
            hipLaunchKernelGGL(embed_pos_bwd_kernel<bf16_t>, dim3(grid_for((long long)L * H)), dim3(256), 0, s,
                               (const bf16_t*)dsum, dpos, B, L, H, packed_of);
        else
            hipLaunchKernelGGL(embed_pos_bwd_kernel<float>, dim3(grid_for((long long)L * H)), dim3(256), 0, s,
                               (const float*)dsum, dpos, B, L, H, packed_of);
        HS_LAUNCH_CHECK();
    }
    return HS_OK;
}
}
// ... 135 lines not shown
    else
        hipLaunchKernelGGL(gelu_bwd_kernel<float>, dim3(grid_for(n)), dim3(256), 0, (hipStream_t)stream, (const float*)dy,
                           (const float*)u, (float*)dx, n, (int)al16(dy, u, dx));
    HS_LAUNCH_CHECK();
    return HS_OK;
}
hs_status hs_mul_dev_scalar(const float* x, const float* scalar, float* out, int64_t n, void* stream) {
    HS_REQUIRE(x && scalar && out, "mul_dev_scalar: null argument");
    hipLaunchKernelGGL(mul_dev_scalar_kernel, dim3(grid_for(n)), dim3(256), 0, (hipStream_t)stream, x, scalar, out, n);
    HS_LAUNCH_CHECK();
    return HS_OK;
}
hs_status hs_colsum(int32_t dtype, const void* x, int64_t M, int32_t N, int32_t ld, float* out, void* ws,
                    int64_t ws_bytes, int32_t accumulate, void* stream) {
    HS_REQUIRE(x && out && M > 0 && N > 0, "colsum: bad argument");
    return DISPATCH_T(dtype, colsum_t, x, M, N, ld, out, (float*)ws, ws_bytes, accumulate, (hipStream_t)stream);
}
int64_t hs_colsum_ws_bytes(int64_t M, int32_t N) { return (int64_t)colsum_gy(M, N) * N * 4; }
hs_status hs_softmax_fwd(int32_t dtype, const float* S, const int64_t* mask, void* P, void* P_drop, int64_t rows,
                         int32_t Lk, int32_t ldS, int32_t ldP, int32_t rows_per_batch, float dropout_p, uint64_t seed,
                         void* stream) {
    HS_REQUIRE(S && P && rows > 0 && Lk > 0 && rows_per_batch > 0, "softmax: bad argument");
    return DISPATCH_T(dtype, softmax_fwd_t, S, (const long long*)mask, P, P_drop, rows, Lk, ldS, ldP, rows_per_batch,
                      dropout_p, seed, (hipStream_t)stream);
}
hs_status hs_softmax_bwd(int32_t dtype, const float* dP, const void* P, void* dS, int64_t rows, int32_t Lk, int32_t ldG,
                         int32_t ldP, float dropout_p, uint64_t seed, void* stream) {
    HS_REQUIRE(dP && P && dS && rows > 0 && Lk > 0, "softmax_bwd: bad argument");
    return DISPATCH_T(dtype, softmax_bwd_t, dP, P, dS, rows, Lk, ldG, ldP, dropout_p, seed, (hipStream_t)stream);
}
hs_status hs_bert_embed_fwd(int32_t dtype, const int64_t* ids, const float* word, const float* pos, const float* type0,
                            const float* gamma, const float* beta, void* sum_out, void* y, float* mean, float* rstd,
                            int64_t tokens, int32_t L, int32_t H, int32_t V, float eps, float dropout_p, uint64_t seed,
                            void* stream) {
    return hs::bert_embed_fwd_rows(dtype, ids, word, pos, type0, gamma, beta, sum_out, y, mean, rstd, tokens, L, H, V, eps, dropout_p,
                                   seed, nullptr, nullptr, (hipStream_t)stream);
}
hs_status hs_bert_embed_bwd(int32_t dtype, const int64_t* ids, const void* dsum, float* dword, float* dpos, int32_t B,
                            int32_t L, int32_t H, int32_t V, int32_t pad_id, void* stream) {
    return hs::bert_embed_bwd_rows(dtype, ids, dsum, dword, dpos, B, L, H, V, pad_id, nullptr, nullptr, nullptr, (hipStream_t)stream);
}
hs_status hs_transpose_bf16(const void* src, void* dst, int32_t R, int32_t Cc, int64_t ld_src, int64_t ld_dst, void* stream) {
    HS_REQUIRE(src && dst && R > 0 && Cc > 0, "transpose_bf16: bad argument");
    HS_REQUIRE(R % 8 == 0 && Cc % 8 == 0 && ld_src % 8 == 0 && ld_dst % 8 == 0 && ld_src >= Cc && ld_dst >= R &&
                   (((uintptr_t)src | (uintptr_t)dst) & 15) == 0,
               "transpose_bf16: dims / leading dimensions must be multiples of 8 and bases 16-byte aligned");
    hipLaunchKernelGGL(transpose_bf16_kernel, dim3(ceil_div(Cc, 64), ceil_div(R, 64)), dim3(256), 0, (hipStream_t)stream,
                       (const unsigned short*)src, (unsigned short*)dst, R, Cc, (long long)ld_src, (long long)ld_dst);
    HS_LAUNCH_CHECK();
    return HS_OK;
}
hs_status hs_transpose_bf16_multi(int32_t count, const void* const* src, void* const* dst, const int32_t* R, const int32_t* Cc,
                                  const int64_t* ld_src, const int64_t* ld_dst, void* stream) {
    return hs::transpose_bf16_multi_rows(count, src, dst, R, Cc, ld_src, ld_dst, nullptr, nullptr, (hipStream_t)stream);
}
hs_status hs_cross_entropy(const float* logits, const int64_t* labels, const float* weight, float label_smoothing,
                           int32_t B, int32_t C, float* loss, float* dlogits, float* row_loss, void* stream) {
    HS_REQUIRE(logits && labels && loss && B > 0 && C > 0, "cross_entropy: bad argument");
    const int waves = B >= 32 ? 16 : B >= 16 ? 8 : 4;
    hipLaunchKernelGGL(ce_kernel, dim3(1), dim3(64 * waves), 0, (hipStream_t)stream, logits, (const long long*)labels, weight,
                       label_smoothing, B, C, loss, dlogits, row_loss);
    HS_LAUNCH_CHECK();
    return HS_OK;
}
hs_status hs_sgd_step_multi(int32_t count, float* const* params, const float* const* grads, float* const* momentum_buf,
                            const int64_t* n, float lr, float momentum, float weight_decay, int32_t nesterov, int32_t first,
                            float grad_scale, void* stream) {
    HS_REQUIRE(count >= 0 && (momentum == 0.f || momentum_buf), "sgd: bad argument");
    for (int base = 0; base < count; base += HS_ADAM_MAX) {
        AdamTable t;
        memset(&t, 0, sizeof(t));
        const int cnt = std::min(HS_ADAM_MAX, count - base);
        long long mx = 0;
        for (int i = 0; i < cnt; ++i) {
            t.p[i] = params[base + i];
            t.g[i] = grads[base + i];
            t.m[i] = momentum != 0.f ? momentum_buf[base + i] : nullptr;
            t.n[i] = n[base + i];
            mx = std::max<long long>(mx, t.n[i]);
        }
        const int gx = (int)std::min<long long>(std::max<long long>((mx + 1023) / 1024, 1), 512);
        hipLaunchKernelGGL(sgd_multi_kernel, dim3(gx, cnt), dim3(256), 0, (hipStream_t)stream, t, lr, momentum, weight_decay,
                           nesterov, first, grad_scale);
        HS_LAUNCH_CHECK();
    }
    return HS_OK;
}
hs_status hs_adam_step_multi(int32_t count, float* const* params, const float* const* grads, float* const* exp_avg,
                             float* const* exp_avg_sq, const int64_t* n, float lr, float beta1, float beta2, float eps,
                             float weight_decay, int32_t step, int32_t decoupled, float grad_scale, void* stream) {
    return hs_adam_step_multi_shadow(count, params, grads, exp_avg, exp_avg_sq, nullptr, n, lr, beta1, beta2, eps, weight_decay, step,
                                     decoupled, grad_scale, stream);
}
hs_status hs_adam_step_multi_shadow(int32_t count, float* const* params, const float* const* grads, float* const* exp_avg,
                                    float* const* exp_avg_sq, void* const* bf16_shadow, const int64_t* n, float lr, float beta1,
                                    float beta2, float eps, float weight_decay, int32_t step, int32_t decoupled,
                                    float grad_scale, void* stream) {
    HS_REQUIRE(count >= 0 && step >= 1, "adam: bad argument");
    const float bc1 = 1.f - powf(beta1, (float)step);
    const float bc2s = sqrtf(1.f - powf(beta2, (float)step));
    for (int base = 0; base < count; base += HS_ADAM_MAX) {
        AdamTable t;
        memset(&t, 0, sizeof(t));
        const int cnt = std::min(HS_ADAM_MAX, count - base);
        long long mx = 0;
        for (int i = 0; i < cnt; ++i) {
            t.p[i] = params[base + i];
// ... 16 lines not shown
```

### multimodal-diagnosis-ham-spine_amd/hamspine/csrc/gemm.hip

```cpp
#include <mutex>
#include <unordered_set>
#include <vector>
#include <stdarg.h>
#include <math.h>
#include <map>
#include <tuple>
#include "gemm_launch.h"
#include "gemm_p8.h"

namespace hs {

static thread_local char g_err[512] = "";
void set_error(const char* fmt, ...) {
    va_list ap;
    va_start(ap, fmt);
    vsnprintf(g_err, sizeof(g_err), fmt, ap);
    va_end(ap);
}
const char* last_error() { return g_err; }

bool lds_attr_needed(const void* fn) {
    static std::mutex mu;
    static std::unordered_set<const void*> seen;
    std::lock_guard<std::mutex> lk(mu);
    return seen.insert(fn).second;
}

struct ProfRec {
    hipEvent_t a, b;
    double flops;
    int cls;
    int M, N, K, combo, cfg, split, batch, conv_r, conv_stride;
    double bytes = 0;
};
static std::mutex g_prof_mu;
static bool g_prof_on = false;
static std::vector<ProfRec> g_prof;
static std::vector<std::pair<hipEvent_t, hipEvent_t>> g_prof_pool;

static bool prof_begin(hipStream_t s, double flops, int cls, ProfRec& r) {
    std::lock_guard<std::mutex> lk(g_prof_mu);
    if (!g_prof_on) return false;
    if (!g_prof_pool.empty()) {
        r.a = g_prof_pool.back().first;
        r.b = g_prof_pool.back().second;
        g_prof_pool.pop_back();
    } else if (hipEventCreate(&r.a) != hipSuccess || hipEventCreate(&r.b) != hipSuccess) {
        return false;
    }
    r.flops = flops;
    r.cls = cls;
    (void)hipEventRecord(r.a, s);
// ... 51 lines not shown
    const long long z = (long long)(p->batch > 0 ? p->batch : 1) * (p->split_k > 1 ? p->split_k : 1);
    const long long t12864 = (long long)ceil_div(p->M, 128) * ceil_div(p->N, 64) * z;
    const long long t128 = (long long)ceil_div(p->M, 128) * ceil_div(p->N, 128) * z;
    if (p->dtype == HS_BF16) {
        const bool plain = (p->a_kind == HS_A_KC || p->a_kind == HS_A_RC) && (p->b_kind == HS_B_KC || p->b_kind == HS_B_RC);
        if (plain && batch_is_one(p)) {
            if (p->a_kind == HS_A_KC && p->split_k <= 1 && p->N >= 2048 && p->K <= 1024 && p->M >= 2048 && p->K % 32 == 0) return CFG_128x128x32;
            if (p->a_kind == HS_A_KC && p->b_kind == HS_B_KC && p->split_k <= 1 && p->K >= 2048 && t12864 >= 256) return CFG_128x64;
        }
        return t12864 >= 1536 ? CFG_128x64 : CFG_64x64;
    }
    return (vec && t128 >= 200) ? CFG_128x128 : CFG_64x64;
}
static bool conv3_enabled() {
    static const bool on = [] { const char* e = getenv("HAMSPINE_CONV3"); return !(e && e[0] == '0'); }();
    return on;
}
static bool conv3_plan(const hs_gemm_params* p, int* rows, int* tpi, int* fm) {
    if (!conv3_enabled() || g_dbg_cfg >= 0) return false;
    const hs_conv_geom& g = p->g;
    if (p->dtype != HS_BF16 || p->a_kind != HS_A_CONV || p->b_kind != HS_B_KC || p->split_k > 1 || p->batch > 1) return false;
    if (g.R != 3 || g.S != 3 || g.stride != 1 || g.pad != 1 || g.P != g.H || g.Q != g.W || g.C % 64 != 0 || p->N % 64 != 0) return false;
    if (g.row_pitch != g.W * g.C || g.img_pitch != g.H * g.W * g.C || g.qstep != g.C || g.no_bounds) return false;
    if (p->bias || p->colscale || p->act != HS_ACT_NONE || p->residual || p->D_preact || p->mul_mode != HS_MUL_NONE || p->dropout_p > 0.f ||
        p->accumulate || p->seg_rows > 0 || p->alpha != 1.f || p->out_dtype != HS_BF16 || p->rowsum_a || p->bnb_partials)
        return false;
    if (p->ldd % 8 != 0 || (((uintptr_t)p->D) & 15) != 0 || p->ldb != 9 * g.C || p->K != 9 * g.C || p->N != g.K) return false;
    if (g.W > 112 || g.W < 1) return false;
    const int rmax = std::min(g.H, 112 / g.W);
    const int t = ceil_div(g.H, rmax), r = ceil_div(g.H, t);
    const int tp = r * g.W;
    if (tp < 32 || (r + 2) * (g.W + 2) > 256) return false;
    *rows = r;
    *tpi = t;
    *fm = tp > 64 ? 7 : 4;
    return true;
}
int gemm_stat_rows(const hs_gemm_params* p) {
    if (!p || p->dtype != HS_BF16 || p->split_k > 1 || p->batch > 1) return 0;
    {
        int r, t, fm;
        if (conv3_plan(p, &r, &t, &fm)) return p->g.N * t;
    }
    int cfg = (p->a_kind == HS_A_CONV && p->b_kind == HS_B_KC && p->g.C % 64 != 0) ? CFG_STEM : auto_cfg(p, true);
    if (g_dbg_cfg >= 0 && g_dbg_cfg <= CFG_64x64 && cfg != CFG_STEM) cfg = g_dbg_cfg;
    if (g_dbg_cfg >= CFG_256x128 && g_dbg_cfg <= CFG_256x128x32 && !(p->a_kind == HS_A_CONV || p->a_kind == HS_A_DGRAD || p->b_kind == HS_B_CONV)) cfg = g_dbg_cfg;
    return ceil_div(p->M, cfg == CFG_64x64 ? 64 : (cfg == CFG_256x128 || cfg == CFG_256x128x32) ? 256 : 128);
}

static bool bn_finish_variant(int cfg, int combo) {
    return (combo == 0 && (cfg == CFG_64x64 || cfg == CFG_128x64)) || (combo == 3 && (cfg == CFG_64x64 || cfg == CFG_128x64 || cfg == CFG_STEM || cfg == CFG_C3));
}

struct Prepared {
    GemmArgs a;
    int cfg, combo, split, batch;
    bool bf16, conv, vec;
    dim3 grid;
    double flops;
};
static int gemm_prepare(const hs_gemm_params* p, hipStream_t stream, Prepared& q, int force_cfg = -1) {
    HS_REQUIRE(p != nullptr, "hs_gemm: null params");
    HS_REQUIRE(p->dtype == HS_F32 || p->dtype == HS_BF16, "hs_gemm: bad dtype %d", p->dtype);
    HS_REQUIRE(p->M > 0 && p->N > 0 && p->K >= 0, "hs_gemm: bad dims %d %d %d", p->M, p->N, p->K);
    HS_REQUIRE(p->A && p->B && p->D, "hs_gemm: null operand");
    const int combo = combo_of(p->a_kind, p->b_kind);
    HS_REQUIRE(combo >= 0, "hs_gemm: unsupported operand kinds (%d,%d)", p->a_kind, p->b_kind);
    const bool bf16 = p->dtype == HS_BF16;
    const int esz = bf16 ? 2 : 4, epc = bf16 ? 8 : 4;
    const int batch = p->batch > 0 ? p->batch : 1;
    const int split = p->split_k > 1 ? p->split_k : 1;
    HS_REQUIRE(!(batch > 1 && split > 1), "hs_gemm: batch and split_k are exclusive");
    HS_REQUIRE((long long)p->a_elems * esz < 0x7fffff00ll && (long long)p->b_elems * esz < 0x7fffff00ll,
               "hs_gemm: operand larger than 2 GiB");
    HS_REQUIRE(p->out_dtype == HS_F32 || p->out_dtype == p->dtype, "hs_gemm: out_dtype must be f32 or the operand type");
    HS_REQUIRE(!p->accumulate || p->out_dtype == HS_F32, "hs_gemm: accumulate needs an f32 output");

    GemmArgs a;
    memset(&a, 0, sizeof(a));
    a.A = (const char*)p->A;
    a.B = (const char*)p->B;
    a.a_bytes = (unsigned long long)p->a_elems * esz;
    a.b_bytes = (unsigned long long)p->b_elems * esz;
    a.lda = p->lda;
    a.ldb = p->ldb;
    a.M = p->M;
    a.N = p->N;
    a.K = p->K;
    a.g = p->g;
    a.batch_inner = p->batch_inner > 0 ? p->batch_inner : 1;
    a.a_bs0 = p->a_bs0; a.a_bs1 = p->a_bs1;
    a.b_bs0 = p->b_bs0; a.b_bs1 = p->b_bs1;
    a.d_bs0 = p->d_bs0; a.d_bs1 = p->d_bs1;
    a.D = (char*)p->D;
    a.ldd = p->ldd;
    a.out_f32 = p->out_dtype == HS_F32;
    a.alpha = p->alpha;
    a.bias = p->bias;
    a.act = p->act;
    a.D_preact = (char*)p->D_preact;
    a.residual = (const char*)p->residual;
    a.ldr = p->ldr;
    if (p->dropout_p > 0.f) {
        HS_REQUIRE(p->dropout_p < 1.f, "hs_gemm: dropout_p must be < 1");
        a.drop_thresh = dropout_thresh(p->dropout_p);
        a.drop_inv_keep = 1.f / (1.f - p->dropout_p);
// ... 191 lines not shown
                   "hs_gemm: bnb_finish needs bnb_partials and a launch hs_gemm_bnb_finish_rows accepts");
        HS_REQUIRE(f->C == p->N && f->M > 0 && f->dgamma && f->dbeta, "hs_gemm: bnb_finish needs the BatchNorm's C, M, dgamma, dbeta");
        HS_REQUIRE((long long)a.tiles_n * (1 + stat_groups(a.tiles_m)) <= kTicketPool, "hs_gemm: bnb_finish: too many column tiles");
        a.bnb_gamma = f->gamma; a.bnb_dgamma = f->dgamma; a.bnb_dbeta = f->dbeta;
        a.bnb_invm = 1.f / (float)f->M; a.bnb_train = f->training;
        a.bnb_tickets = ticket_pool(stream);
        HS_REQUIRE(a.bnb_tickets != nullptr, "hs_gemm: cannot allocate the arrival counters");
    }
    if (p->bn_finish) {
        const hs_bn_params* f = p->bn_finish;
        HS_REQUIRE(a.colstats && bn_finish_variant(cfg, combo), "hs_gemm: bn_finish needs colstats and a tile / layout hs_gemm_bn_finish_rows accepts");
        HS_REQUIRE(f->training && f->C == p->N && f->M == p->M && f->save_mean && f->save_invstd && f->scale && f->shift,
                   "hs_gemm: bn_finish needs a training-mode hs_bn_params of the result's shape with save_mean / save_invstd / scale / shift");
        HS_REQUIRE((long long)a.tiles_n * (1 + stat_groups(a.tiles_m)) <= kTicketPool, "hs_gemm: bn_finish: too many column tiles");
        a.bnf_gamma = f->gamma; a.bnf_beta = f->beta;
        a.bnf_rmean = f->running_var ? f->running_mean : nullptr; a.bnf_rvar = f->running_var;
        a.bnf_mean = f->save_mean; a.bnf_invstd = f->save_invstd; a.bnf_scale = f->scale; a.bnf_shift = f->shift;
        a.bnf_eps = f->eps; a.bnf_momentum = f->momentum;
        a.bnf_tickets = ticket_pool(stream);
        HS_REQUIRE(a.bnf_tickets != nullptr, "hs_gemm: cannot allocate the arrival counters");
    }
    {
        static const bool hist = [] { const char* e = getenv("HAMSPINE_EPI_HIST"); return e && e[0] == '1'; }();
        if (hist) {
            static std::mutex mu;
            static std::map<std::pair<unsigned, int>, long long> cnt;
            static const bool reg = [] {
                atexit([] {
                    for (auto& kv : cnt) fprintf(stderr, "[epi] flags 0x%05x bf16 %d : %lld launches\n", kv.first.first, kv.first.second, kv.second);
                });
                return true;
            }();
            (void)reg;
            unsigned f = 0;
            if (p->bias) f |= EPI_BIAS;
            if (p->colscale) f |= EPI_COLSCALE;
            if (p->mul_mode == HS_MUL_GELU_GRAD) f |= EPI_MUL_GELU;
            else if (p->mul_mode != HS_MUL_NONE) f |= EPI_MUL_RELU;
            if (p->seg_rows > 0) f |= EPI_SEG;
            if (p->D_preact) f |= EPI_PREACT;
            if (p->residual) f |= p->residual_before_act ? EPI_RES_PRE : EPI_RES_POST;
            if (p->act == HS_ACT_RELU) f |= EPI_RELU;
            else if (p->act == HS_ACT_GELU) f |= EPI_GELU;
            if (p->dropout_p > 0.f) f |= EPI_DROP;
            if (p->out_dtype == HS_F32) f |= EPI_OUT_F32;
            if (p->accumulate) f |= EPI_ACCUM;
            if (a.vec_store) f |= EPI_VEC;
            if (a.parity) f |= EPI_PARITY;
            if (split > 1) f |= 0x80000;
            std::lock_guard<std::mutex> lk(mu);
            cnt[{f, p->dtype == HS_BF16 ? 1 : 0}]++;
        }
    }
    dim3 grid(a.tiles_m * a.tiles_n, 1, split > 1 ? split : batch);
    {
        static const bool on = [] { const char* e = getenv("HAMSPINE_PERSISTENT"); return e && e[0] == '1'; }();
        static const int cus = [] { hipDeviceProp_t pr; int d = 0; return (hipGetDevice(&d) == hipSuccess && hipGetDeviceProperties(&pr, d) == hipSuccess) ? pr.multiProcessorCount : 256; }();
        if ((on || (g_dbg_ablate & 64)) && bf16 && split == 1 && batch == 1 && !a.stamps && !a.m_rows && !a.drop_rows && !p->rowsum_a && !p->bnb_partials && !p->bn_finish && (cfg == CFG_64x64 || cfg == CFG_128x64) &&
            (combo == 0 || combo == 1 || combo == 3 || combo == 4)) {
            const int lds = a.lds_stages * (BM + BN) * 64 * 2;
            const int per_cu = std::max(1, std::min(cfg == CFG_64x64 ? 3 : 2, (160 * 1024) / lds));
            const int slots = cus * per_cu;
            if ((int)grid.x > slots) {
                a.persist = slots;
                grid.x = slots;
            }
        }
    }
    double flops = 2.0 * p->M * p->N * (double)p->K * batch;
    if (a.parity) {
        int kept = 0;
        for (int c = 0; c < 4; ++c)
            for (int r = 0; r < p->g.R; ++r)
                for (int q = 0; q < p->g.S; ++q)
                    kept += ((((c >> 1) + p->g.pad - r) & 1) == 0 && (((c & 1) + p->g.pad - q) & 1) == 0) ? 1 : 0;
        flops *= (double)kept / (4.0 * p->g.R * p->g.S);
    }
    q.a = a;
    q.cfg = cfg; q.combo = combo; q.split = split; q.batch = batch;
    q.bf16 = bf16; q.conv = conv; q.vec = vec;
    q.grid = grid;
    q.flops = flops;
    return HS_OK;
}

int gemm_tile_rows(const hs_gemm_params* p) {
    if (!p) return 0;
    hs_gemm_params c = *p;
    unsigned char dummy[16];
    if (c.split_k > 1 && !c.splitk_ws) c.splitk_ws = (float*)dummy;
    Prepared q;
    if (gemm_prepare(&c, nullptr, q) != HS_OK) return 0;
    return q.a.tiles_m;
}

int gemm_bn_finish_rows(const hs_gemm_params* p) {
    if (!p || !p->colstats) return 0;
    hs_gemm_params c = *p;
    c.bn_finish = nullptr;
    Prepared q;
    if (gemm_prepare(&c, nullptr, q) != HS_OK) return 0;
    if (!q.bf16 || q.split != 1 || q.batch != 1 || q.a.persist > 0 || !bn_finish_variant(q.cfg, q.combo)) return 0;
    if ((long long)q.a.tiles_n * (1 + stat_groups(q.a.tiles_m)) > kTicketPool) return 0;
    return q.a.tiles_m + stat_groups(q.a.tiles_m);
}

// ... 103 lines not shown
    fw[n] = g->total;
    memcpy(host.data() + kHead, g->items.data(), (size_t)n * sizeof(GemmArgs));
    if (host != g->shadow) {
        static const bool dbg = [] { const char* e = getenv("HAMSPINE_GROUP_DEBUG"); return e && e[0] == '1'; }();
        if (dbg) {
            size_t diff = 0;
            for (size_t i = 0; i < std::min(host.size(), g->shadow.size()); ++i) diff += host[i] != g->shadow[i];
            fprintf(stderr, "[group] table upload: %d problems, %zu bytes (%zu before), %zu bytes differ\n", n, bytes, g->shadow.size(), diff);
        }
        HS_CHECK_HIP(hipStreamSynchronize(s));
        if (bytes > g->dev_cap) {
            if (g->dev) (void)hipFree(g->dev);
            g->dev = nullptr;
            g->dev_cap = 0;
            HS_CHECK_HIP(hipMalloc(&g->dev, bytes * 2));
            g->dev_cap = bytes * 2;
        }
        HS_CHECK_HIP(hipMemcpy(g->dev, host.data(), bytes, hipMemcpyHostToDevice));
        g->shadow.swap(host);
    }
    ProfRec rec;
    const bool timed = prof_begin(s, g->flops, g->combo == 5 ? 1 : 0, rec);
    const int st = g->combo == 5   ? launch_bf16_grouped_conv(5, (const GemmArgs*)(g->dev + kHead), (const int*)g->dev, n, g->total, s)
                   : (g->combo == 0 && g->cfg == CFG_P8_256) ? launch_bf16_p8_grouped((const GemmArgs*)(g->dev + kHead), (const int*)g->dev, n, g->total, g->rs, s)
                   : g->combo == 0 ? launch_bf16_grouped_big(0, (const GemmArgs*)(g->dev + kHead), (const int*)g->dev, n, g->total, s)
                                   : launch_bf16_grouped_plain(2, (const GemmArgs*)(g->dev + kHead), (const int*)g->dev, n, g->total, s);
    if (timed) {
        rec.M = n; rec.N = 0; rec.K = 0; rec.combo = g->combo == 5 ? 7 : g->combo == 0 ? 8 : 6;
        rec.cfg = g->combo == 0 ? (g->cfg == CFG_P8_256 ? CFG_P8_256 : CFG_256x128) : CFG_64x64; rec.split = 0; rec.batch = 1;
        rec.conv_r = 0; rec.conv_stride = 0;
        rec.bytes = g->bytes;
        prof_end(s, rec);
    }
    g->combo = -1;
    g->cfg = -1;
    g->rs = false;
    g->items.clear();
    g->first.clear();
    g->total = 0;
    g->ticket_off = 0;
    g->flops = g->bytes = 0;
    return st;
}
static thread_local int (*g_group_immediate_hook)(void*) = nullptr;
static thread_local void* g_group_immediate_ctx = nullptr;
void gemm_group_set_immediate_hook(int (*fn)(void*), void* ctx) {
    g_group_immediate_hook = fn;
    g_group_immediate_ctx = ctx;
}
static int launch_ungrouped(const hs_gemm_params* p, hipStream_t s) {
    if (g_group_immediate_hook) HS_PROPAGATE(g_group_immediate_hook(g_group_immediate_ctx));
    return gemm_impl(p, s);
}
int gemm_group_add(GemmGroup* g, const hs_gemm_params* p, hipStream_t s) {
    if (!g) return launch_ungrouped(p, s);
    Prepared q;
    const bool big = p->a_kind == HS_A_KC && p->b_kind == HS_B_KC;
    static const bool p8w = [] { const char* e = getenv("HAMSPINE_P8_WGRAD"); return !(e && e[0] == '0'); }();
    const bool want_p8 = big && p8w && p->dtype == HS_BF16 && p->M % 256 == 0 && p->N % 256 == 0 && p->K % 64 == 0 && p->K >= 2048 &&
                         (p->batch <= 1) && p->split_k <= 1 && g_dbg_cfg < 0 && (g->items.empty() || g->combo != 0 || g->cfg == CFG_P8_256);
    HS_PROPAGATE(gemm_prepare(p, s, q, big ? (want_p8 ? CFG_P8_256 : CFG_256x128) : -1));
    if (want_p8 && !(p8_epilogue_supported(q.a) && !q.a.colstats && !q.a.bnb_partials && (long long)p->M * p->lda * 2 < 0x7fffff00ll &&
                     (long long)p->N * p->ldb * 2 < 0x7fffff00ll))
        HS_PROPAGATE(gemm_prepare(p, s, q, CFG_256x128));
    const bool ok = big ? (q.bf16 && (q.cfg == CFG_256x128 || q.cfg == CFG_P8_256) && q.combo == 0 && q.batch == 1 && q.split == 1 && !q.a.stamps && !q.a.colstats)
                        : (q.bf16 && q.cfg == CFG_64x64 && (q.combo == 2 || q.combo == 5) && q.batch == 1 && !q.a.stamps &&
                           (q.split == 1 || q.a.tickets != nullptr) && !q.a.rowsum[0] && !q.a.colstats);
    if (!ok) return launch_ungrouped(p, s);
    const long long ngroups = q.split > 1 ? (q.split + kSplitGroup - 1) / kSplitGroup : 0;
    const long long need = q.split > 1 ? (long long)q.a.tiles_m * q.a.tiles_n * (1 + (ngroups > 1 ? ngroups : 0)) : 0;
    if (!g->items.empty() && (g->combo != q.combo || (big && g->cfg != q.cfg) || (int)g->items.size() >= kGroupMax || g->ticket_off + need > kTicketPool)) {
        if (g_group_immediate_hook) HS_PROPAGATE(g_group_immediate_hook(g_group_immediate_ctx));
        HS_PROPAGATE(gemm_group_flush(g, s));
    }
    if (need > kTicketPool) return launch_ungrouped(p, s);
    g->combo = q.combo;
    if (big) {
        g->cfg = q.cfg;
        g->rs = g->rs || q.a.rowsum[0] != nullptr;
    }
    if (q.split > 1) q.a.tickets += g->ticket_off;
    g->ticket_off += (int)need;
    g->first.push_back(g->total);
    g->total += (int)(q.grid.x * q.grid.z);
    g->items.push_back(q.a);
    g->flops += q.flops;
    const double R2 = q.conv ? (double)p->g.R * p->g.S : 1.0, st2 = q.conv ? (double)p->g.stride * p->g.stride : 1.0;
    g->bytes += 2.0 * ((double)p->M * p->K + (double)p->N * p->K / R2 * st2) + 4.0 * (double)p->M * p->N;
    return HS_OK;
}

}

extern "C" {
void hs_gemm_debug_stamps(void* device_buffer) { hs::g_dbg_stamps = (unsigned long long*)device_buffer; }
void hs_gemm_debug(int32_t cfg_override, int32_t ablate) {
    hs::g_dbg_cfg = cfg_override;
    hs::g_dbg_ablate = ablate;
}
void hs_prof_enable(int32_t on) {
    std::lock_guard<std::mutex> lk(hs::g_prof_mu);
    hs::g_prof_on = on != 0;
}
hs_status hs_prof_collect(double* flops, double* ms, int64_t* launches) {
    HS_CHECK_HIP(hipDeviceSynchronize());
    std::lock_guard<std::mutex> lk(hs::g_prof_mu);
    for (int i = 0; i < 4; ++i) {
        flops[i] = 0;
        ms[i] = 0;
        launches[i] = 0;
    }
    for (auto& r : hs::g_prof) {
        float t = 0.f;
        if (hipEventElapsedTime(&t, r.a, r.b) == hipSuccess) {
            flops[r.cls] += r.flops;
            ms[r.cls] += t;
            launches[r.cls] += 1;
        }
        hs::g_prof_pool.emplace_back(r.a, r.b);
    }
    hs::g_prof.clear();
    return HS_OK;
}
hs_status hs_prof_calibrate(void* stream, int32_t n, float* avg_us) {
    HS_REQUIRE(n > 0 && avg_us, "hs_prof_calibrate: bad argument");
    hipStream_t s = (hipStream_t)stream;
    std::vector<std::pair<hipEvent_t, hipEvent_t>> ev(n);
    for (auto& e : ev) {
        HS_CHECK_HIP(hipEventCreate(&e.first));
        HS_CHECK_HIP(hipEventCreate(&e.second));
    }
    for (auto& e : ev) {
        HS_CHECK_HIP(hipEventRecord(e.first, s));
        hipLaunchKernelGGL(hs::null_kernel, dim3(1), dim3(64), 0, s);
        HS_CHECK_HIP(hipEventRecord(e.second, s));
    }
    HS_CHECK_HIP(hipStreamSynchronize(s));
    double tot = 0;
    for (auto& e : ev) {
        float t = 0.f;
        HS_CHECK_HIP(hipEventElapsedTime(&t, e.first, e.second));
        tot += t;
        (void)hipEventDestroy(e.first);
        (void)hipEventDestroy(e.second);
    }
    *avg_us = (float)(tot / n * 1e3);
    return HS_OK;
}
// ... 57 lines not shown
```

### multimodal-diagnosis-ham-spine_amd/hamspine/csrc/gemm_core.h

```cpp
#pragma once
#include <type_traits>
#include "hs_common.h"

namespace hs {

struct GemmArgs {
    const char* A;
    const char* B;
    unsigned long long a_bytes, b_bytes;
    int lda, ldb;
    int M, N, K;
    hs_conv_geom g;
    FastDiv div_mhw, div_mw;
    FastDiv div_sc, div_c;
    int batch_inner;
    long long a_bs0, a_bs1, b_bs0, b_bs1, d_bs0, d_bs1;
    int tiles_m, tiles_n;
    int group_m;
    int parity;
    int quarter;
    FastDiv div_qhw, div_qw;
    const float* colscale;
    int res_pre_act;
    float* colstats;
    int persist;
    int lds_stages;
    int split_k;
    int k_per_split;
    float* splitk_ws;
    unsigned* tickets;
    char* D;
    int ldd;
    int out_f32;
    float alpha;
    const float* bias;
    int act;
    char* D_preact;
    const char* residual;
    int ldr;
    unsigned drop_thresh;
    float drop_inv_keep;
    unsigned long long drop_seed;
    int mul_mode;
    const char* mul_src;
    int ldm;
    int accumulate;
    int vec_store;
    int seg_rows;
    char* D_seg[2];
    const char* bnb_x;
    const float *bnb_scale, *bnb_shift, *bnb_mean, *bnb_invstd;
    float* bnb_partials;
    const char* bnb_y;
    const float* bnb_gamma;
    float *bnb_dgamma, *bnb_dbeta;
    float bnb_invm;
    int bnb_train;
    unsigned* bnb_tickets;
    const float *bnf_gamma, *bnf_beta;
    float *bnf_rmean, *bnf_rvar, *bnf_mean, *bnf_invstd, *bnf_scale, *bnf_shift;
    float bnf_eps, bnf_momentum;
    unsigned* bnf_tickets;
    float* rowsum[3];
    int c3_rows, c3_tpi, c3_fm;
    int vec16;
    int epi_generic;
    int dbg;
    unsigned long long* stamps;
    const int* m_rows;
    const int* drop_rows;
};

#define HS_STAMP(k)                                                                                              \
    do {                                                                                                         \
        if (a.stamps && threadIdx.x == 0)                                                                        \
            a.stamps[((long long)blockIdx.z * gridDim.x + blockIdx.x) * 6 + (k)] = __builtin_readcyclecounter(); \
    } while (0)

__device__ __forceinline__ int parity_class(const GemmArgs& a, int m) {
    return (m >= a.quarter) + (m >= 2 * a.quarter) + (m >= 3 * a.quarter);
}
__device__ __forceinline__ void parity_pixel(const GemmArgs& a, int m, unsigned& n, unsigned& h, unsigned& w) {
    const int cls = parity_class(a, m);
    const unsigned idx = m - cls * a.quarter;
    n = fdiv(idx, a.div_qhw);
    const unsigned ij = idx - n * a.div_qhw.d;
    const unsigned i = fdiv(ij, a.div_qw);
    h = 2 * i + (cls >> 1);
    w = 2 * (ij - i * a.div_qw.d) + (cls & 1);
}
__device__ __forceinline__ long long parity_row(const GemmArgs& a, int m) {
    unsigned n, h, w;
    parity_pixel(a, m, n, h, w);
    return ((long long)n * a.g.H + h) * a.g.W + w;
}


#define HS_GLOBAL __attribute__((address_space(1)))
template <typename T>
__device__ __forceinline__ void load4(const char* base, long long idx, bool vec, int nvalid, float* f) {
    const HS_GLOBAL T* p = (const HS_GLOBAL T*)((const T*)base + idx);
    if (vec) {
        if constexpr (sizeof(T) == 4) {
            f32x4 v = *(const HS_GLOBAL f32x4*)p;
            f[0] = v[0]; f[1] = v[1]; f[2] = v[2]; f[3] = v[3];
        } else {
            u32x2 v = *(const HS_GLOBAL u32x2*)p;
            f[0] = __uint_as_float(v[0] << 16);
            f[1] = __uint_as_float(v[0] & 0xffff0000u);
            f[2] = __uint_as_float(v[1] << 16);
            f[3] = __uint_as_float(v[1] & 0xffff0000u);
        }
    } else {
#pragma unroll
        for (int j = 0; j < 4; ++j) f[j] = j < nvalid ? to_f32(p[j]) : 0.f;
    }
}
template <typename T>
__device__ __forceinline__ void store4(char* base, long long idx, bool vec, int nvalid, const float* f) {
    HS_GLOBAL T* p = (HS_GLOBAL T*)((T*)base + idx);
    if (vec) {
        if constexpr (sizeof(T) == 4) {
            f32x4 v = {f[0], f[1], f[2], f[3]};
// ... 282 lines not shown
    }
    return ok ? (unsigned)off * ESZ : kOOB;
}

template <typename T>
__device__ __forceinline__ u32x4 load_chunk(__amdgpu_buffer_rsrc_t rs, unsigned off, bool vec, int nvalid) {
    if (vec) return buf_load16(rs, off);
    u32x4 c = {0, 0, 0, 0};
    if (off == kOOB) return c;
    if constexpr (sizeof(T) == 4) {
#pragma unroll
        for (int j = 0; j < 4; ++j)
            if (j < nvalid) c[j] = buf_load4(rs, off + 4 * j);
    } else {
#pragma unroll
        for (int j = 0; j < 8; ++j)
            if (j < nvalid) {
                unsigned v = buf_load2(rs, off + 2 * j);
                c[j >> 1] |= (j & 1) ? (v << 16) : v;
            }
    }
    return c;
}

template <typename T>
__device__ __forceinline__ void mask_tail(u32x4& c, int nvalid) {
    if constexpr (sizeof(T) == 4) {
#pragma unroll
        for (int j = 0; j < 4; ++j)
            if (j >= nvalid) c[j] = 0u;
    } else {
#pragma unroll
        for (int j = 0; j < 8; ++j)
            if (j >= nvalid) c[j >> 1] &= (j & 1) ? 0x0000ffffu : 0xffff0000u;
    }
}

template <int I, int N, typename F>
__device__ __forceinline__ void static_for(F&& f) {
    if constexpr (I < N) {
        f(std::integral_constant<int, I>{});
        static_for<I + 1, N>(f);
    }
}

constexpr int kSplitGroup = 8;
constexpr int kStatGroup = 32;
__host__ __device__ inline int stat_groups(int tiles_m) { return tiles_m <= kStatGroup ? 0 : (tiles_m + kStatGroup - 1) / kStatGroup; }
inline long long splitk_slabs(int split) { return split <= kSplitGroup ? split : split + (split + kSplitGroup - 1) / kSplitGroup; }

constexpr bool a_is_rc(int k) { return k == HS_A_RC; }
constexpr bool b_is_rc(int k) { return k != HS_B_KC; }

__device__ __forceinline__ void tile_from_block(const GemmArgs& a, int& tm, int& tn, int bid) {
    const int nwg = a.tiles_m * a.tiles_n;
    const int xcd = bid & 7, q = nwg >> 3, r = nwg & 7;
    const int id = (xcd < r ? xcd * (q + 1) : r * (q + 1) + (xcd - r) * q) + (bid >> 3);
    const int gsz = a.group_m * a.tiles_n;
    const int grp = id / gsz;
    const int first_m = grp * a.group_m;
    const int gm = min(a.group_m, a.tiles_m - first_m);
    const int within = id - grp * gsz;
    tn = within / gm;
    tm = first_m + (within - tn * gm);
}

template <int BR>
__device__ __forceinline__ int rc_logical_chunk(int k, int pcc) {
    constexpr int G = BR / 16;
    int f;
    if constexpr (G >= 8) f = (k & 3) | (((k >> 3) & 1) << 2);
    else f = ((k >> 1) & 1) | (((k >> 3) & 1) << 1);
    return ((((pcc >> 1) ^ f) & (G - 1)) << 1) | (pcc & 1);
}

template <typename T, int CF, bool FULL, int FM, int FN, int WM, int WN>
__device__ __forceinline__ void run_epilogue(const GemmArgs& a, const unsigned epi, f32x4 (&acc)[FM][FN], int m0, int n0, int wm,
                                             int wn, int l15, int g, long long d_boff, int z, const int (&mdrop)[FM]) {
        if constexpr (FULL && CF >= 0 && !(CF & (EPI_OUT_F32 | EPI_SEG | EPI_PARITY)) && (FN % 2 == 0) && sizeof(T) == 2) {
            const bool odd = g & 1;
#pragma unroll
            for (int i = 0; i < FM; ++i) {
                const int m = m0 + wm * WM + i * 16 + l15;
#pragma unroll
                for (int j = 0; j < FN; j += 2) {
                    const int n = n0 + wn * WN + j * 16 + 4 * g;
                    float v0[4] = {acc[i][j][0], acc[i][j][1], acc[i][j][2], acc[i][j][3]};
                    float v1[4] = {acc[i][j + 1][0], acc[i][j + 1][1], acc[i][j + 1][2], acc[i][j + 1][3]};
                    float p0[4], p1[4];
                    epilogue4<T, CF, true, true>(a, epi, d_boff, z, m, n, v0, p0, mdrop[i]);
                    epilogue4<T, CF, true, true>(a, epi, d_boff, z, m, n + 16, v1, p1, mdrop[i]);
                    const long long didx = d_boff + (long long)m * a.ldd + (odd ? n + 12 : n);
                    auto pair_store = [&](char* base, const float* x0, const float* x1) {
                        const bf16x4 b0 = {(bf16_t)x0[0], (bf16_t)x0[1], (bf16_t)x0[2], (bf16_t)x0[3]};
                        const bf16x4 b1 = {(bf16_t)x1[0], (bf16_t)x1[1], (bf16_t)x1[2], (bf16_t)x1[3]};
                        const u32x2 a0 = __builtin_bit_cast(u32x2, b0), a1 = __builtin_bit_cast(u32x2, b1);
                        const u32x2 send = odd ? a0 : a1;
                        u32x2 recv;
                        recv[0] = __shfl_xor(send[0], 16, 64);
                        recv[1] = __shfl_xor(send[1], 16, 64);
                        const u32x4 o = odd ? u32x4{recv[0], recv[1], a1[0], a1[1]} : u32x4{a0[0], a0[1], recv[0], recv[1]};
                        *(HS_GLOBAL u32x4*)((HS_GLOBAL bf16_t*)base + didx) = o;
                    };
                    if constexpr (CF & EPI_PREACT) pair_store(a.D_preact, p0, p1);
                    pair_store(a.D, v0, v1);
                    if (i == 0 && j == 0) HS_STAMP(5);
                }
            }
            return;
        }
#pragma unroll
        for (int i = 0; i < FM; ++i) {
            const int m = m0 + wm * WM + i * 16 + l15;
#pragma unroll
// ... 193 lines not shown
                __hip_atomic_store(o, t1, __ATOMIC_RELAXED, __HIP_MEMORY_SCOPE_AGENT);
                __hip_atomic_store(o + 1, t2, __ATOMIC_RELAXED, __HIP_MEMORY_SCOPE_AGENT);
            }
            first = tiles_m;
            count = ngroups;
            ticket = a.bnb_tickets + tn;
        }
    }
    if (sub == 0 && cok) {
        float* coef = a.bnb_partials + (long long)(tiles_m + ngroups) * a.N * 2;
        a.bnb_dbeta[n] = t1;
        a.bnb_dgamma[n] = t2;
        const float gm = a.bnb_gamma ? a.bnb_gamma[n] : 1.f, is = a.bnb_invstd[n];
        const float ca = gm * is;
        coef[n] = ca;
        coef[a.N + n] = a.bnb_train ? -ca * is * t2 * a.bnb_invm : 0.f;
        coef[2 * a.N + n] = a.bnb_train ? -ca * t1 * a.bnb_invm : 0.f;
        coef[3 * a.N + n] = a.bnb_mean[n];
    }
}
template <int BM, int BN, int BK, int AK, int BKIND, bool VEC, int WGM = 2, bool RS = false, int NS = 3, bool SK = true, bool PS = false,
          bool BNS = false, bool BNF = false>
__device__ __forceinline__ void gemm_bf16_body(const GemmArgs& a, const int bx, const int bz) {
    typedef bf16_t T;
    constexpr int ESZ = 2;
    constexpr bool A_RC = a_is_rc(AK), B_RC = b_is_rc(BKIND);
    constexpr bool ROWSUM = A_RC || RS;
    constexpr int NW = 2 * WGM;
    constexpr int WM = BM / WGM, WN = BN / 2, FM = WM / 16, FN = WN / 16;
    constexpr int A_BYTES = BM * BK * 2, B_BYTES = BN * BK * 2, STAGE = A_BYTES + B_BYTES;
    constexpr int A_NI = A_BYTES / 1024 / NW, B_NI = B_BYTES / 1024 / NW;
    constexpr int CPR = BK / 8;
    static_assert(A_NI >= 1 && B_NI >= 1, "tile too small for its DMA waves");
    extern __shared__ __attribute__((aligned(16))) char smem[];
    typedef __attribute__((address_space(3))) char lds_char;

    const int tid = threadIdx.x, lane = tid & 63;
    const int wave = __builtin_amdgcn_readfirstlane(tid >> 6);
    const int wm = wave >> 1, wn = wave & 1;
    const int g = lane >> 4, l15 = lane & 15;
    int tm, tn;
    const unsigned long long t_entry = __builtin_readcyclecounter();
    {
        const int q0 = a.tiles_m, q1 = a.tiles_n, q2 = a.group_m, q3 = a.split_k, q4 = a.k_per_split, q5 = a.batch_inner;
        const int q6 = a.M, q7 = a.N, q8 = a.K, q9 = a.lda, q10 = a.ldb;
        const char* pa = a.A;
        const char* pb = a.B;
        const unsigned long long ba = a.a_bytes, bb = a.b_bytes;
        asm volatile("" ::"s"(q0), "s"(q1), "s"(q2), "s"(q3), "s"(q4), "s"(q5), "s"(q6), "s"(q7), "s"(q8), "s"(q9), "s"(q10),
                     "s"(pa), "s"(pb), "s"(ba), "s"(bb));
    }
    int m0, n0;
    const int z = bz;
    if (a.m_rows) {
        tile_from_block(a, tm, tn, bx);
        if (tm * BM >= __builtin_amdgcn_readfirstlane(a.m_rows[0])) return;
    }

    long long a_boff = 0, b_boff = 0, d_boff = 0;
    int kbeg = 0, kend = a.K;
    if (a.split_k > 1) {
        kbeg = z * a.k_per_split;
        kend = min(a.K, kbeg + a.k_per_split);
    } else {
        const int zo = z / a.batch_inner, zi = z - zo * a.batch_inner;
        a_boff = zo * a.a_bs0 + zi * a.a_bs1;
        b_boff = zo * a.b_bs0 + zi * a.b_bs1;
        d_boff = zo * a.d_bs0 + zi * a.d_bs1;
    }
    const unsigned long long a_rem = a.a_bytes - (unsigned long long)a_boff * ESZ;
    const unsigned long long b_rem = a.b_bytes - (unsigned long long)b_boff * ESZ;
    const __amdgpu_buffer_rsrc_t rsA = make_rsrc(a.A + a_boff * ESZ, (unsigned)min(a_rem, 0x7fffff00ull));
    const __amdgpu_buffer_rsrc_t rsB = make_rsrc(a.B + b_boff * ESZ, (unsigned)min(b_rem, 0x7fffff00ull));

    KcRow<A_RC ? HS_A_KC : AK> a_rows[A_RC ? 1 : A_NI];
    KcRow<HS_A_KC> b_rows[B_RC ? 1 : B_NI];
    RcCol a_cols[A_RC ? A_NI : 1], b_cols[B_RC ? B_NI : 1];
    int a_kl[A_NI], b_kl[B_NI];
    constexpr int NDMA = A_NI + B_NI;
    static_assert(NS >= 3 && NS <= 8 && (NS - 1) * NDMA <= 63, "ring depth: the vmcnt field holds 6 bits");
    constexpr int KS = BK / 32;
    int ntiles = 0;
    unsigned long long taps = 0;
    int tiles_per_tap = 1;
    bool filtered = false;
    auto setup_tile = [&](const int vb) {
    tile_from_block(a, tm, tn, vb);
    m0 = tm * BM;
    n0 = tn * BN;
#pragma unroll
    for (int i = 0; i < A_NI; ++i) {
        const int s = (wave * A_NI + i) * 64 + lane;
        if constexpr (!A_RC) {
            const int r = s / CPR;
            kc_row_setup<AK>(a, m0 + r, a_rows[i]);
            a_kl[i] = ((s % CPR) ^ kc_swz<CPR>(r)) * 8;
        } else {
            const int k = s / (BM / 8);
            a_kl[i] = k;
            rc_col_setup<AK, true>(a, m0 + rc_logical_chunk<BM>(k, s % (BM / 8)) * 8, a_cols[i]);
        }
    }
#pragma unroll
    for (int i = 0; i < B_NI; ++i) {
        const int s = (wave * B_NI + i) * 64 + lane;
        if constexpr (!B_RC) {
            const int r = s / CPR;
            const int n = n0 + r;
            b_rows[i].valid = n < a.N;
            b_rows[i].base = n * a.ldb;
            b_rows[i].hb = b_rows[i].wb = 0;
            b_kl[i] = ((s % CPR) ^ kc_swz<CPR>(r)) * 8;
        } else {
            const int k = s / (BN / 8);
            b_kl[i] = k;
            rc_col_setup<BKIND, false>(a, n0 + rc_logical_chunk<BN>(k, s % (BN / 8)) * 8, b_cols[i]);
        }
    }
    ntiles = (kend - kbeg + BK - 1) / BK;
    taps = 0;
    tiles_per_tap = 1;
    filtered = false;
    if constexpr (AK == HS_A_DGRAD) {
        if (a.parity) {
            const int c_first = parity_class(a, m0), c_last = parity_class(a, min(m0 + BM, a.M) - 1);
            if (c_first == c_last) {
                filtered = true;
                tiles_per_tap = a.g.K / BK;
                int kept = 0;
                for (int r = 0; r < a.g.R; ++r)
                    for (int q = 0; q < a.g.S; ++q)
                        if ((((c_first >> 1) + a.g.pad - r) & 1) == 0 && (((c_first & 1) + a.g.pad - q) & 1) == 0) {
                            taps |= (unsigned long long)(r * a.g.S + q) << (4 * kept);
                            ++kept;
                        }
                ntiles = kept * tiles_per_tap;
            }
        }
    }
    };
// ... 596 lines not shown
__global__ __launch_bounds__(256) __attribute__((amdgpu_waves_per_eu(3, 3))) void gemm_bf16_kernel_w3(const GemmArgs a) {
    gemm_bf16_body<128, 128, 32, AK, BKIND, true, 2, false, HS_W3_RING, false>(a, blockIdx.x, blockIdx.z);
}

template <int AK, int BKIND>
__global__ __launch_bounds__(256) void gemm_bf16_grouped_kernel(const GemmArgs* __restrict__ list, const int* __restrict__ first_wg, int n) {
    const int bid = blockIdx.x, lane = threadIdx.x & 63;
    const int lo = lane < n ? first_wg[lane] : 0x7fffffff;
    const int p = __builtin_amdgcn_readfirstlane(__popcll(__ballot(lo <= bid)) - 1);
    const int local = bid - __builtin_amdgcn_readfirstlane(first_wg[p]);
    const GemmArgs& a = list[p];
    const int tiles = a.tiles_m * a.tiles_n;
    const int bz = local / tiles;
    gemm_bf16_body<64, 64, 64, AK, BKIND, true>(a, local - bz * tiles, bz);
}

template <int AK, int BKIND>
__global__ __launch_bounds__(512) void gemm_bf16_grouped_big_kernel(const GemmArgs* __restrict__ list, const int* __restrict__ first_wg, int n) {
    const int bid = blockIdx.x, lane = threadIdx.x & 63;
    const int lo = lane < n ? first_wg[lane] : 0x7fffffff;
    const int p = __builtin_amdgcn_readfirstlane(__popcll(__ballot(lo <= bid)) - 1);
    const int local = bid - __builtin_amdgcn_readfirstlane(first_wg[p]);
    gemm_bf16_body<256, 128, 64, AK, BKIND, true, 4, true, 3, false>(list[p], local, 0);
}

struct GemmArgsPack4 {
    GemmArgs a[4];
    int first[5];
    int n;
};
template <int AK, int BKIND>
__global__ __launch_bounds__(512) void gemm_bf16_grouped_big4_kernel(const GemmArgsPack4 pk) {
    const int bid = blockIdx.x;
    int p = 0;
    for (int i = 1; i < pk.n; ++i) p += bid >= pk.first[i];
    p = __builtin_amdgcn_readfirstlane(p);
    gemm_bf16_body<256, 128, 64, AK, BKIND, true, 4, true, 3, false>(pk.a[p], bid - pk.first[p], 0);
}

template <int BM, int BN, int AK, int BKIND, bool VEC>
__global__ __launch_bounds__(256) void gemm_f32_kernel(const GemmArgs a) {
    typedef float T;
    constexpr int BK = 32, EPC = 4, ESZ = 4;
    constexpr bool A_RC = a_is_rc(AK), B_RC = b_is_rc(BKIND);
    constexpr int WM = BM / 2, WN = BN / 2, FM = WM / 32, FN = WN / 32;
    constexpr int A_BYTES = BM * BK * 4, B_BYTES = BN * BK * 4, STAGE = A_BYTES + B_BYTES;
    constexpr int A_NCH = BM * BK / 4 / 256, B_NCH = BN * BK / 4 / 256;
    extern __shared__ __attribute__((aligned(16))) char smem[];

    const int tid = threadIdx.x, lane = tid & 63, wave = tid >> 6;
    const int wm = wave >> 1, wn = wave & 1;
    const int l31 = lane & 31, hh = lane >> 5;
    int tm, tn;
    tile_from_block(a, tm, tn, blockIdx.x);
    const int m0 = tm * BM, n0 = tn * BN;
    const int z = blockIdx.z;

    long long a_boff = 0, b_boff = 0, d_boff = 0;
    int kbeg = 0, kend = a.K;
    if (a.split_k > 1) {
        kbeg = z * a.k_per_split;
        kend = min(a.K, kbeg + a.k_per_split);
    } else {
        const int zo = z / a.batch_inner, zi = z - zo * a.batch_inner;
        a_boff = zo * a.a_bs0 + zi * a.a_bs1;
        b_boff = zo * a.b_bs0 + zi * a.b_bs1;
        d_boff = zo * a.d_bs0 + zi * a.d_bs1;
    }
    const unsigned long long a_rem = a.a_bytes - (unsigned long long)a_boff * ESZ;
    const unsigned long long b_rem = a.b_bytes - (unsigned long long)b_boff * ESZ;
    const __amdgpu_buffer_rsrc_t rsA = make_rsrc(a.A + a_boff * ESZ, (unsigned)min(a_rem, 0x7fffff00ull));
    const __amdgpu_buffer_rsrc_t rsB = make_rsrc(a.B + b_boff * ESZ, (unsigned)min(b_rem, 0x7fffff00ull));

    KcRow<A_RC ? HS_A_KC : AK> a_row;
    KcRow<HS_A_KC> b_row;
    RcCol a_col, b_col;
    if constexpr (!A_RC) kc_row_setup<AK>(a, m0 + tid % BM, a_row);
    else rc_col_setup<AK, true>(a, m0 + (tid % (BM / 4)) * 4, a_col);
    if constexpr (!B_RC) {
        const int n = n0 + tid % BN;
        b_row.valid = n < a.N;
        b_row.base = n * a.ldb;
        b_row.hb = b_row.wb = 0;
    } else {
        rc_col_setup<BKIND, false>(a, n0 + (tid % (BN / 4)) * 4, b_col);
    }

    u32x4 a_reg[A_NCH], b_reg[B_NCH];
    auto stage_load = [&](int k0) {
        KTile kta = {0, 0, 0}, ktb = {0, 0, 0};
        if constexpr (AK == HS_A_CONV) kta = ktile_rsc(k0, a.g.C, a.g.S);
        if constexpr (AK == HS_A_DGRAD) kta = ktile_rsc(k0, a.g.K, a.g.S);
        if constexpr (BKIND == HS_B_WDGRAD) ktb = ktile_rsc(k0, a.g.K, a.g.S);
#pragma unroll
        for (int i = 0; i < A_NCH; ++i) {
            const int id = tid + 256 * i;
            unsigned off;
            int nvalid = 4;
            if constexpr (!A_RC) {
                const int k = k0 + (id / BM) * 4;
                off = kc_chunk_off<AK, ESZ>(a, a_row, kta, k, kend);
                nvalid = kend - k;
            } else {
                const int k = k0 + id / (BM / 4);
                off = rc_chunk_off<AK, true, ESZ>(a, a_col, kta, k, kend);
                if constexpr (!VEC) nvalid = a.M - a_col.base;
            }
// ... 133 lines not shown
```

### multimodal-diagnosis-ham-spine_amd/hamspine/csrc/gemm_p8.h

```cpp
#pragma once
#include "gemm_core.h"

namespace hs {

template <int N>
__device__ __forceinline__ void wait_vmcnt() {
    asm volatile("s_waitcnt vmcnt(%0)" ::"n"(N) : "memory");
}

template <int BM, int BN, int WGM, int WGN, bool RS, bool STAG, bool DIAG = false, int TAG = 0>
__device__ __forceinline__ void gemm_bf16_p8_body(const GemmArgs& a, const int bx) {
    typedef bf16_t T;
    constexpr int BK = 64, NW = WGM * WGN;
    constexpr int WM = BM / WGM, WN = BN / WGN;
    constexpr int QM = WM / 2, QN = WN / 2;
    constexpr int FMQ = QM / 16, FNQ = QN / 16;
    constexpr int FM = 2 * FMQ, FN = 2 * FNQ;
    constexpr int A_SLOT = (BM / 2) * BK * 2, B_SLOT = (BN / 2) * BK * 2;
    constexpr int BUF = 2 * A_SLOT + 2 * B_SLOT;
    constexpr int NA = A_SLOT / 1024 / NW, NB = B_SLOT / 1024 / NW;
    static_assert(QM % 16 == 0 && QN % 16 == 0 && NA >= 1 && NB >= 1 && A_SLOT % (1024 * NW) == 0 && B_SLOT % (1024 * NW) == 0, "tile / wave shape");
    static_assert(3 * NA + 3 * NB <= 63, "vmcnt field");
    extern __shared__ __attribute__((aligned(16))) char smem[];
    typedef __attribute__((address_space(3))) char lds_char;

    const int tid = threadIdx.x, lane = tid & 63;
    const int wave = __builtin_amdgcn_readfirstlane(tid >> 6);
    const int wm = wave / WGN, wn = wave % WGN;
    const int g = lane >> 4, l15 = lane & 15;
    int tm, tn;
    tile_from_block(a, tm, tn, bx);
    const int m0 = tm * BM, n0 = tn * BN;
    if (a.m_rows && m0 >= __builtin_amdgcn_readfirstlane(a.m_rows[0])) return;
    const int ntiles = a.K / BK;

    const __amdgpu_buffer_rsrc_t rsA = make_rsrc(a.A, (unsigned)min(a.a_bytes, 0x7fffff00ull));
    const __amdgpu_buffer_rsrc_t rsB = make_rsrc(a.B, (unsigned)min(a.b_bytes, 0x7fffff00ull));

    unsigned offA[2][NA], offB[2][NB];
#pragma unroll
    for (int q = 0; q < 2; ++q) {
#pragma unroll
        for (int i = 0; i < NA; ++i) {
            const int r = 8 * (wave * NA + i) + (lane >> 3);
            const int row = m0 + (r / QM) * WM + q * QM + (r % QM);
            offA[q][i] = (unsigned)row * (unsigned)a.lda * 2u + (unsigned)(((lane & 7) ^ kc_swz<8>(r)) << 4);
        }
#pragma unroll
        for (int i = 0; i < NB; ++i) {
            const int r = 8 * (wave * NB + i) + (lane >> 3);
            const int col = n0 + (r / QN) * WN + q * QN + (r % QN);
            offB[q][i] = (unsigned)col * (unsigned)a.ldb * 2u + (unsigned)(((lane & 7) ^ kc_swz<8>(r)) << 4);
        }
    }
    auto dma_a = [&](int t, int q) {
        if (t >= ntiles) return;
        lds_char* dst = (lds_char*)smem + (t & 1) * BUF + q * A_SLOT + wave * (NA * 1024);
        const int koff = t * (BK * 2);
#pragma unroll
        for (int i = 0; i < NA; ++i)
            __builtin_amdgcn_raw_ptr_buffer_load_lds(rsA, (__attribute__((address_space(3))) void*)(dst + i * 1024), 16, offA[q][i], koff, 0, 0);
    };
    auto dma_b = [&](int t, int q) {
        if (t >= ntiles) return;
        lds_char* dst = (lds_char*)smem + (t & 1) * BUF + 2 * A_SLOT + q * B_SLOT + wave * (NB * 1024);
        const int koff = t * (BK * 2);
#pragma unroll
        for (int i = 0; i < NB; ++i)
            __builtin_amdgcn_raw_ptr_buffer_load_lds(rsB, (__attribute__((address_space(3))) void*)(dst + i * 1024), 16, offB[q][i], koff, 0, 0);
    };

    bf16x8 af[FMQ][2], bq[2][FNQ][2];
    auto read_a = [&](int buf, int q) {
        const char* s = smem + buf * BUF + q * A_SLOT;
#pragma unroll
        for (int i = 0; i < FMQ; ++i)
#pragma unroll
            for (int ks = 0; ks < 2; ++ks) af[i][ks] = *(const bf16x8*)(s + kc_off_bf16<BK>(wm * QM + i * 16 + l15, ks * 4 + g));
    };
    auto read_b = [&](int buf, auto qc) {
        constexpr int q = decltype(qc)::value;
        const char* s = smem + buf * BUF + 2 * A_SLOT + q * B_SLOT;
#pragma unroll
        for (int j = 0; j < FNQ; ++j)
#pragma unroll
            for (int ks = 0; ks < 2; ++ks) bq[q][j][ks] = *(const bf16x8*)(s + kc_off_bf16<BK>(wn * QN + j * 16 + l15, ks * 4 + g));
    };
// ... 231 lines not shown
```

Before: 3058 images/s.

## Compact padded-token K columns in BERT weight-gradient GEMMs and spread packed tiles across XCDs

The row-map kernel now also builds a list of 32-token chunks that contain any unmasked token, plus a count. The token transposes feeding BERT weight-gradient GEMMs place only those chunks contiguously, so the grouped NT GEMMs can stop their K loop early and skip padded tokens. A second change remaps the tile-to-block assignment for row-packed GEMMs so the live tiles are spread evenly over XCDs rather than leaving idle blocks that exit early. This adds device-side bookkeeping and a new transpose mode, and risks mistakes in indexing or masking when reading the K bound from the device.

```diff
diff --git a/include/hamspine.h b/include/hamspine.h
--- a/include/hamspine.h
+++ b/include/hamspine.h
@@ -189,6 +189,10 @@
 #define HS_TRANSPOSE_MAX 8
 hs_status hs_transpose_bf16_multi(int32_t count, const void* const* src, void* const* dst, const int32_t* R, const int32_t* C,
                                   const int64_t* ld_src, const int64_t* ld_dst, void* stream);
+int64_t hs_bert_row_map_bytes(int32_t B, int32_t L);
+hs_status hs_bert_row_map(const int64_t* mask, int32_t B, int32_t L, int32_t* map, void* stream);
+hs_status hs_transpose_bf16_tokens(const void* src, void* dst, int32_t R, int32_t C, int64_t ld_src, int64_t ld_dst,
+                                   const int32_t* packed_of, const int32_t* kc_n, const int32_t* kc_pos, void* stream);
 hs_status hs_axpby(int32_t in_dtype, int32_t out_dtype, const void* x, const void* y, void* out, int64_t n, float a,
                    float b, void* stream);
 hs_status hs_dropout(int32_t dtype, const void* x, void* out, int64_t n, float p, uint64_t seed, void* stream);
@@ -415,6 +419,9 @@
 hs_status hs_grad_milestones(int32_t n, const void* const* grad_ptrs, void* const* events);
 int32_t hs_measure_build(void);
 void hs_set_wgrad_nt(int32_t on);
+void hs_set_bert_wgrad_chunks(int32_t on);
+void hs_set_pack_xcd_spread(int32_t on);
+int64_t hs_gemm_k_cols_queued(void);
 
 typedef struct hs_conv_bn {
     int32_t Cin, Cout, R, stride, pad;
diff --git a/multimodal-diagnosis-ham-spine_amd/hamspine/_lib.py b/multimodal-diagnosis-ham-spine_amd/hamspine/_lib.py
--- a/multimodal-diagnosis-ham-spine_amd/hamspine/_lib.py
+++ b/multimodal-diagnosis-ham-spine_amd/hamspine/_lib.py
@@ -318,6 +318,16 @@
     l.hs_measure_build.restype = i32
     l.hs_set_wgrad_nt.argtypes = [i32]
     l.hs_set_wgrad_nt.restype = None
+    l.hs_set_bert_wgrad_chunks.argtypes = [i32]
+    l.hs_set_bert_wgrad_chunks.restype = None
+    l.hs_set_pack_xcd_spread.argtypes = [i32]
+    l.hs_set_pack_xcd_spread.restype = None
+    l.hs_gemm_k_cols_queued.argtypes = []
+    l.hs_gemm_k_cols_queued.restype = i64
+    l.hs_bert_row_map_bytes.argtypes = [i32, i32]
+    l.hs_bert_row_map_bytes.restype = i64
+    l.hs_bert_row_map.argtypes = [vp, i32, i32, vp, vp]
+    l.hs_transpose_bf16_tokens.argtypes = [vp, vp, i32, i32, i64, i64, vp, vp, vp, vp]
     l.hs_bert_pack_rows_available.argtypes = []
     l.hs_bert_pack_rows_available.restype = i32
     l.hs_dwconv_ws_bytes.argtypes = [i32] * 5
diff --git a/multimodal-diagnosis-ham-spine_amd/hamspine/csrc/blocks.hip b/multimodal-diagnosis-ham-spine_amd/hamspine/csrc/blocks.hip
--- a/multimodal-diagnosis-ham-spine_amd/hamspine/csrc/blocks.hip
+++ b/multimodal-diagnosis-ham-spine_amd/hamspine/csrc/blocks.hip
@@ -24,7 +24,8 @@
 void gemm_group_set_immediate_hook(int (*fn)(void*), void* ctx);
 struct GemmGroup;
 GemmGroup* gemm_group_open(hipStream_t s, long long slot);
-int gemm_group_add(GemmGroup* g, const hs_gemm_params* p, hipStream_t s);
+int gemm_group_add(GemmGroup* g, const hs_gemm_params* p, hipStream_t s, const int* k_cols = nullptr);
+bool gemm_group_takes_k_cols();
 int gemm_group_flush(GemmGroup* g, hipStream_t s);
 bool fused_attention_enabled();
 int attention_bwd_fused(const hs_attn_desc& d, const void* q, const void* k, const void* v, const void* dO, void* dq, void* dk,
@@ -40,7 +41,8 @@
                float* dgamma, float* dbeta, void* dx_dropped, float* dbias, float p, unsigned long long seed, float* ws,
                long long ws_bytes, long long M, int H, hipStream_t s, const int* inv);
 int transpose_bf16_multi_rows(int count, const void* const* src, void* const* dst, const int32_t* R, const int32_t* Cc,
-                              const int64_t* ld_src, const int64_t* ld_dst, const int* inv, const unsigned char* tok, hipStream_t stream);
+                              const int64_t* ld_src, const int64_t* ld_dst, const int* inv, const unsigned char* tok, const int* kc,
+                              const int* kc_pos, hipStream_t stream);
 int colsum_rows(int dtype, const void* x, long long M, int N, int ld, float* out, void* ws, long long ws_bytes, int accumulate,
                 const int* inv, hipStream_t s);
 int dropout_rows(int dtype, const void* x, void* out, long long M, int H, float p, unsigned long long seed, const int* nrows,
@@ -49,7 +51,7 @@
 int bert_row_map(const int64_t* mask, int B, int L, int* map, hipStream_t s);
 int bert_unpack_rows(const void* y, void* out, long long rows, long long row_bytes, const int* packed_of, hipStream_t s);
 int bert_pack_rows(const void* dy, void* dst, long long rows, long long row_bytes, const int* nrows, const int* row_of,
-                   hipStream_t s);
+                   const int* word_src, int* word_dst, hipStream_t s);
 int bert_embed_fwd_rows(int dtype, const int64_t* ids, const float* word, const float* pos, const float* type0, const float* gamma,
                         const float* beta, void* sum_out, void* y, float* mean, float* rstd, long long tokens, int L, int H, int V,
                         float eps, float dropout_p, unsigned long long seed, const int* nrows, const int* row_of, hipStream_t stream);
@@ -88,9 +90,11 @@
     bool group_nt = false;
     GemmGroup* grp_nt = nullptr;
     GemmGroup* tower_grp = nullptr;
-    struct PendTr { const void* src; void* dst; int R, C; long long ld; bool tok; };
+    struct PendTr { const void* src; void* dst; int R, C; long long ld; unsigned char tok; };
     std::vector<PendTr> pend_tr;
     const int *pk_T = nullptr, *pk_cu = nullptr, *pk_row = nullptr, *pk_inv = nullptr;
+    const int *pk_kc = nullptr, *pk_kcpos = nullptr, *pk_kcols = nullptr;
+    bool kc_on = false;
 };
 
 static hipStream_t g_side_stream[16] = {};
@@ -437,7 +441,7 @@
 }
 static bool wgrad_nt_enabled();
 static int linear_wgrad_nt_run(Run& r, const void* xT, const void* dyT, long long M, int in_f, int out_f, float* dw, float* db,
-                               int seg_rows, float* const* dw_seg, float* const* db_seg);
+                               int seg_rows, float* const* dw_seg, float* const* db_seg, const int* k_cols = nullptr);
 static int linear_wgrad_run(Run& r, const void* x, long long M, int ldx, const hs_linear& lin, const void* dy, int ldy) {
     bool db_done = false;
     if (lin.dw && r.dt == HS_BF16 && wgrad_nt_enabled() && M >= 2048 && M % 8 == 0 && lin.in_f % 8 == 0 && lin.out_f % 8 == 0 &&
@@ -451,7 +455,7 @@
         const int32_t R[2] = {(int32_t)M, (int32_t)M}, Cc[2] = {lin.out_f, lin.in_f};
         const int64_t lds[2] = {ldy, ldx}, ldd[2] = {M, M};
         const unsigned char tok[2] = {1, 1};
-        CALLK(r, 4, transpose_bf16_multi_rows(2, src, dst, R, Cc, lds, ldd, r.pk_inv, tok, r.s));
+        CALLK(r, 4, transpose_bf16_multi_rows(2, src, dst, R, Cc, lds, ldd, r.pk_inv, tok, nullptr, nullptr, r.s));
         GemmGroup* og = r.plan ? nullptr : open_wgrad_group(r.s);
         const bool keep_flag = r.group_nt;
         GemmGroup* keep_grp = r.grp_nt;
@@ -505,6 +509,14 @@
     }
     return g_wgrad_nt == 1;
 }
+static int g_bert_wgrad_chunks = -1;
+static bool bert_wgrad_chunks_enabled() {
+    if (g_bert_wgrad_chunks < 0) {
+        const char* e = getenv("HAMSPINE_BERT_WGRAD_CHUNKS");
+        g_bert_wgrad_chunks = (e && e[0] == '0') ? 0 : 1;
+    }
+    return g_bert_wgrad_chunks == 1;
+}
 static bool grouped_bert_wgrad_enabled() {
     static int v = -1;
     if (v < 0) {
@@ -527,7 +539,7 @@
 }
 static int transpose_run(Run& r, const void* src, void* dst, long long R, int Cc, int ld_src, bool for_grouped_wgrad = false,
                          bool tokens = false) {
-    const bool tok = tokens && r.pk_T;
+    const unsigned char tok = (tokens && r.pk_T) ? ((for_grouped_wgrad && r.kc_on) ? 2 : 1) : 0;
     if (for_grouped_wgrad && r.tower_grp && r.group_nt && !r.plan && deferred_transposes_enabled()) {
         r.pend_tr.push_back(Run::PendTr{src, dst, (int)R, Cc, ld_src, tok});
         return HS_OK;
@@ -537,8 +549,8 @@
         void* d1[1] = {dst};
         const int32_t R1[1] = {(int32_t)R}, C1[1] = {Cc};
         const int64_t ls[1] = {ld_src}, ldst[1] = {R};
-        const unsigned char t1[1] = {1};
-        CALLK(r, 4, transpose_bf16_multi_rows(1, s1, d1, R1, C1, ls, ldst, r.pk_inv, t1, r.s));
+        const unsigned char t1[1] = {tok};
+        CALLK(r, 4, transpose_bf16_multi_rows(1, s1, d1, R1, C1, ls, ldst, r.pk_inv, t1, r.pk_kc, r.pk_kcpos, r.s));
         return HS_OK;
     }
     CALLK(r, 4, hs_transpose_bf16(src, dst, (int)R, Cc, ld_src, R, r.s));
@@ -555,14 +567,16 @@
     for (int i = 0; i < n; ++i) {
         src[i] = r.pend_tr[i].src; dst[i] = r.pend_tr[i].dst; R[i] = r.pend_tr[i].R; Cc[i] = r.pend_tr[i].C;
         lds[i] = r.pend_tr[i].ld; ldd[i] = r.pend_tr[i].R;
-        tok[i] = r.pend_tr[i].tok ? 1 : 0;
+        tok[i] = r.pend_tr[i].tok;
     }
     r.pend_tr.clear();
-    CALLK(r, 4, transpose_bf16_multi_rows(n, src.data(), dst.data(), R.data(), Cc.data(), lds.data(), ldd.data(), r.pk_inv, tok.data(), r.s));
+    CALLK(r, 4, transpose_bf16_multi_rows(n, src.data(), dst.data(), R.data(), Cc.data(), lds.data(), ldd.data(), r.pk_inv, tok.data(), r.pk_kc,
+                                          r.pk_kcpos, r.s));
     return HS_OK;
 }
 static int linear_wgrad_nt_run(Run& r, const void* xT, const void* dyT, long long M, int in_f, int out_f, float* dw, float* db,
-                               int seg_rows, float* const* dw_seg, float* const* db_seg) {
+                               int seg_rows, float* const* dw_seg, float* const* db_seg, const int* k_cols) {
+    HS_REQUIRE(!k_cols || r.group_nt, "linear_wgrad_nt: chunk-compacted operands outside a grouped weight-gradient grid");
     hs_gemm_params p = gemm_defaults(r.dt);
     p.a_kind = HS_A_KC; p.b_kind = HS_B_KC;
     p.M = out_f; p.N = in_f; p.K = (int)M;
@@ -584,7 +598,7 @@
         }
     }
     if (r.group_nt) {
-        if (!r.plan && !(knock() & 2)) HS_PROPAGATE(gemm_group_add(r.grp_nt, &p, r.s));
+        if (!r.plan && !(knock() & 2)) HS_PROPAGATE(gemm_group_add(r.grp_nt, &p, r.s, k_cols));
         return HS_OK;
     }
     if (!r.plan && (knock() & 2)) { const int sp = hs_gemm_suggest_split(p.M, p.N, p.K, p.dtype); p.split_k = sp; if (sp > 1) (void)r.ws.alloc(hs_gemm_splitk_ws_bytes(&p)); return HS_OK; }
@@ -1371,6 +1385,8 @@
         r.grp_nt = r.tower_grp ? r.tower_grp : gemm_group_open(r.s, (long long)(uintptr_t)d.q.w + 16);
         HS_REQUIRE(r.grp_nt != nullptr, "bert_layer_bwd: cannot set up the grouped weight-gradient launch");
     }
+    r.kc_on = r.pk_T && r.pk_kcols && grouped && !r.plan && bert_wgrad_chunks_enabled() && gemm_group_takes_k_cols();
+    const int* const k_cols = r.kc_on ? r.pk_kcols : nullptr;
     char* tX_g = nt ? (char*)r.ws.alloc(M * (long long)I * 2) : nullptr;
     char* tX_x1 = nt ? (char*)r.ws.alloc(M * (long long)Hd * 2) : nullptr;
     char* tX_ctx = nt ? (char*)r.ws.alloc(M * (long long)Hd * 2) : nullptr;
@@ -1390,7 +1406,7 @@
         }
         HS_PROPAGATE(transpose_run(r, dy_rm, tAk, M, lin.out_f, ldy, true, true));
         const bool fused_b = lin.db && (r.group_nt || hs_gemm_suggest_split(lin.out_f, in_f, (int)M, r.dt) <= 1) && fused_bias_grad_enabled();
-        HS_PROPAGATE(linear_wgrad_nt_run(r, xT, tAk, M, in_f, lin.out_f, lin.dw, lin.db, 0, nullptr, nullptr));
+        HS_PROPAGATE(linear_wgrad_nt_run(r, xT, tAk, M, in_f, lin.out_f, lin.dw, lin.db, 0, nullptr, nullptr, k_cols));
         if (lin.db && !fused_b) HS_PROPAGATE(bias_by_colsum(lin, dy_rm, ldy));
         return HS_OK;
     };
@@ -1406,7 +1422,7 @@
         unsigned char tok[7];
         int n = 0;
         auto add = [&](const void* s_, void* d_, long long rows, int cols, bool tokens = false) {
-            src[n] = s_; dst[n] = d_; R[n] = (int32_t)rows; Cc[n] = cols; lds[n] = cols; ldd[n] = rows; tok[n] = tokens ? 1 : 0;
+            src[n] = s_; dst[n] = d_; R[n] = (int32_t)rows; Cc[n] = cols; lds[n] = cols; ldd[n] = rows; tok[n] = tokens ? (r.kc_on ? 2 : 1) : 0;
             ++n;
         };
         if (nt) {
@@ -1420,7 +1436,7 @@
             add(L.wi, wi_t, I, Hd);
             add(L.wqkv, wqkv_t, 3 * Hd, Hd);
         }
-        if (n > 0) CALLK(r, 4, transpose_bf16_multi_rows(n, src, dst, R, Cc, lds, ldd, r.pk_inv, tok, r.s));
+        if (n > 0) CALLK(r, 4, transpose_bf16_multi_rows(n, src, dst, R, Cc, lds, ldd, r.pk_inv, tok, r.pk_kc, r.pk_kcpos, r.s));
     }
     HS_PROPAGATE(on_side(r, [&]() { return wgrad(L.g, tX_g, I, out_l_w, g2, Hd, tA_ffn2); }));
     HS_PROPAGATE(linear_dgrad_run(r, d.out_l, L.wo, g2, M, Hd, du, I, r.dt, HS_MUL_GELU_GRAD, L.u, I, nullptr, wo_t));
@@ -1454,7 +1470,7 @@
                                   fused_bias_grad_enabled();
             float* dws[2] = {d.k.dw, d.v.dw};
             float* dbs[2] = {d.k.db, d.v.db};
-            HS_PROPAGATE(linear_wgrad_nt_run(r, tX_x, tA_qkv, M, Hd, 3 * Hd, d.q.dw, bias_too ? d.q.db : nullptr, Hd, dws, dbs));
+            HS_PROPAGATE(linear_wgrad_nt_run(r, tX_x, tA_qkv, M, Hd, 3 * Hd, d.q.dw, bias_too ? d.q.db : nullptr, Hd, dws, dbs, k_cols));
             if (bias_too) return HS_OK;
             const hs_linear* lins[3] = {&d.q, &d.k, &d.v};
             for (int i = 0; i < 3; ++i) HS_PROPAGATE(bias_by_colsum(*lins[i], dq ? dq + (long long)i * Hd * es : nullptr, 3 * Hd));
@@ -1497,6 +1513,7 @@
     }
     if (r.group_nt && !r.plan && !r.tower_grp) HS_PROPAGATE(gemm_group_flush(r.grp_nt, r.s));
     r.group_nt = false;
+    r.kc_on = false;
     HS_PROPAGATE(side_join(r));
     RUN_CHECK_ARENAS(r, "bert_layer_bwd");
     return HS_OK;
@@ -1688,6 +1705,8 @@
     r.pk_cu = map + 4;
     r.pk_row = r.pk_cu + (d.B + 1 + 3) / 4 * 4;
     r.pk_inv = r.pk_row + (long long)d.B * d.L;
+    r.pk_kc = map + 1;
+    r.pk_kcpos = r.pk_inv + (long long)d.B * d.L;
 }
 static int bert_check(const hs_bert_desc& d) {
     HS_REQUIRE(d.n_layers >= 0 && d.n_layers <= HS_BERT_MAX_LAYERS, "bert: n_layers %d out of range", d.n_layers);
@@ -1758,6 +1777,7 @@
     const long long M = (long long)d.B * d.L;
     const int Hd = d.hidden;
     char* dy_packed = d.pack_rows ? (char*)r.ws.alloc(lo.act_bytes) : nullptr;
+    int* kcols = d.pack_rows ? (int*)r.ws.alloc(sizeof(int)) : nullptr;
     char* gbuf[2] = {(char*)r.ws.alloc(lo.act_bytes), (char*)r.ws.alloc(lo.act_bytes)};
     int cur = 0;
     const void* dy = dy_in;
@@ -1765,7 +1785,8 @@
     if (d.pack_rows && !r.plan) {
         RUN_CHECK_ARENAS(r, "bert_bwd(row map)");
         bert_pack_pointers(r, d, lo);
-        HS_PROPAGATE(bert_pack_rows(dy_in, dy_packed, M, (long long)Hd * esize(d.dtype), r.pk_T, r.pk_row, r.s));
+        HS_PROPAGATE(bert_pack_rows(dy_in, dy_packed, M, (long long)Hd * esize(d.dtype), r.pk_T, r.pk_row, r.pk_kc + 1, kcols, r.s));
+        r.pk_kcols = kcols;
         dy = dy_packed;
     }
     static const int span = [] { const char* e = getenv("HAMSPINE_WGRAD_LAYERS"); const int v = e ? atoi(e) : 2; return v >= 1 && v <= 8 ? v : 2; }();
@@ -2275,4 +2296,5 @@
 #endif
 }
 void hs_set_wgrad_nt(int32_t on) { hs::g_wgrad_nt = on ? 1 : 0; }
-}
+void hs_set_bert_wgrad_chunks(int32_t on) { hs::g_bert_wgrad_chunks = on ? 1 : 0; }
+}
diff --git a/multimodal-diagnosis-ham-spine_amd/hamspine/csrc/elem.hip b/multimodal-diagnosis-ham-spine_amd/hamspine/csrc/elem.hip
--- a/multimodal-diagnosis-ham-spine_amd/hamspine/csrc/elem.hip
+++ b/multimodal-diagnosis-ham-spine_amd/hamspine/csrc/elem.hip
@@ -719,9 +719,11 @@
 }
 
 __global__ __launch_bounds__(256) void bert_row_map_kernel(const long long* __restrict__ mask, int B, int L, int* __restrict__ map) {
+    __shared__ int s_wave_n[4];
     int* cu = map + 4;
     int* row_of = cu + (B + 1 + 3) / 4 * 4;
     int* packed_of = row_of + (long long)B * L;
+    int* kc_pos = packed_of + (long long)B * L;
     const int lane = threadIdx.x & 63, wave = threadIdx.x >> 6;
     for (int b = wave; b < B; b += 4) {
         int n = 0;
@@ -764,6 +766,31 @@
         }
     }
     for (int t = T + (int)threadIdx.x; t < B * L; t += 256) row_of[t] = t;
+    const int nch = (B * L + 31) / 32;
+    int kc_n = 0;
+    for (int c0 = 0; c0 < nch; c0 += 256) {
+        const int c = c0 + (int)threadIdx.x;
+        long long any = 0;
+#pragma unroll
+        for (int i = 0; i < 32; ++i) {
+            const long long pos = (long long)c * 32 + i;
+            const long long m = mask[min(pos, (long long)B * L - 1)];
+            any |= pos < (long long)B * L ? m : 0;
+        }
+        const bool v = any != 0;
+        const unsigned long long bal = __ballot(v);
+        if (lane == 0) s_wave_n[wave] = __popcll(bal);
+        __syncthreads();
+        int at = kc_n;
+        for (int w = 0; w < wave; ++w) at += s_wave_n[w];
+        if (v) kc_pos[at + __popcll(bal & ((1ull << lane) - 1ull))] = c;
+        kc_n += s_wave_n[0] + s_wave_n[1] + s_wave_n[2] + s_wave_n[3];
+        __syncthreads();
+    }
+    if (threadIdx.x == 0) {
+        map[1] = kc_n;
+        map[2] = 32 * kc_n;
+    }
 }
 __global__ __launch_bounds__(256) void bert_unpack_rows_kernel(const u32x4* __restrict__ y, u32x4* __restrict__ out, long long rows, int cpr,
                                                                const int* __restrict__ packed_of) {
@@ -777,7 +804,9 @@
     }
 }
 __global__ __launch_bounds__(256) void bert_pack_rows_kernel(const u32x4* __restrict__ dy, u32x4* __restrict__ dst, long long rows, int cpr,
-                                                             const int* __restrict__ nrows, const int* __restrict__ row_of) {
+                                                             const int* __restrict__ nrows, const int* __restrict__ row_of,
+                                                             const int* __restrict__ word_src, int* __restrict__ word_dst) {
+    if (word_dst && blockIdx.x == 0 && threadIdx.x == 0) word_dst[0] = word_src[0];
     const long long T = packed_rows(nrows, rows), total = T * cpr;
     for (long long i = (long long)blockIdx.x * 256 + threadIdx.x; i < total; i += (long long)gridDim.x * 256) {
         const long long t = i / cpr;
@@ -789,12 +818,25 @@
 
 __device__ __forceinline__ void transpose_bf16_tile(const unsigned short* __restrict__ src, unsigned short* __restrict__ dst,
                                                     int R, int Cc, long long lds_, long long ldd, int bx, int by,
-                                                    unsigned (*tile)[33], const int* __restrict__ inv) {
+                                                    unsigned (*tile)[33], const int* __restrict__ inv, const int* __restrict__ kc,
+                                                    const int* __restrict__ kc_pos) {
     const int r0 = by * 64, c0 = bx * 64;
+    const int nch = (R + 31) / 32;
+    int kc_n = 0;
+    if (kc) {
+        kc_n = min(max(__builtin_amdgcn_readfirstlane(kc[0]), 0), nch);
+        if (r0 >= max(64, (32 * kc_n + 63) / 64 * 64)) return;
+    }
     for (int i = threadIdx.x; i < 512; i += 256) {
         const int r = i >> 3, ch = i & 7;
         u32x4 v = {0u, 0u, 0u, 0u};
         int sr = r0 + r;
+        if (kc) {
+            const int ci = sr >> 5;
+            int pc = ci < kc_n ? kc_pos[ci] : -1;
+            if (pc >= nch) pc = -1;
+            sr = pc >= 0 ? pc * 32 + (sr & 31) : R;
+        }
         if (inv && sr < R) {
             sr = inv[sr];
             if (sr >= R) sr = -1;
@@ -821,7 +863,7 @@
                                                              unsigned short* __restrict__ dst, int R, int Cc, long long lds_,
                                                              long long ldd) {
     __shared__ unsigned tile[64][33];
-    transpose_bf16_tile(src, dst, R, Cc, lds_, ldd, blockIdx.x, blockIdx.y, tile, nullptr);
+    transpose_bf16_tile(src, dst, R, Cc, lds_, ldd, blockIdx.x, blockIdx.y, tile, nullptr, nullptr, nullptr);
 }
 struct TransposeTable {
     const unsigned short* src[HS_TRANSPOSE_MAX];
@@ -832,6 +874,8 @@
     int count;
     const int* inv;
     unsigned tok_mask;
+    const int *kc, *kc_pos;
+    unsigned kc_mask;
 };
 __global__ __launch_bounds__(256) void transpose_bf16_multi_kernel(const TransposeTable t) {
     __shared__ unsigned tile[64][33];
@@ -840,7 +884,8 @@
     const int local = blockIdx.x - t.first[e];
     const int tx = (t.C[e] + 63) / 64;
     const int* inv = (t.inv && ((t.tok_mask >> e) & 1u)) ? t.inv : nullptr;
-    transpose_bf16_tile(t.src[e], t.dst[e], t.R[e], t.C[e], t.ld_src[e], t.ld_dst[e], local % tx, local / tx, tile, inv);
+    transpose_bf16_tile(t.src[e], t.dst[e], t.R[e], t.C[e], t.ld_src[e], t.ld_dst[e], local % tx, local / tx, tile, inv,
+                        (inv && ((t.kc_mask >> e) & 1u)) ? t.kc : nullptr, t.kc_pos);
 }
 
 __global__ __launch_bounds__(1024) void ce_kernel(const float* __restrict__ logits, const long long* __restrict__ labels,
@@ -1102,7 +1147,8 @@
 }
 
 int transpose_bf16_multi_rows(int count, const void* const* src, void* const* dst, const int32_t* R, const int32_t* Cc,
-                              const int64_t* ld_src, const int64_t* ld_dst, const int* inv, const unsigned char* tok, hipStream_t stream) {
+                              const int64_t* ld_src, const int64_t* ld_dst, const int* inv, const unsigned char* tok, const int* kc,
+                              const int* kc_pos, hipStream_t stream) {
     HS_REQUIRE(count >= 0 && (count == 0 || (src && dst && R && Cc && ld_src && ld_dst)), "transpose_bf16_multi: bad argument");
     for (int base = 0; base < count; base += HS_TRANSPOSE_MAX) {
         TransposeTable t;
@@ -1122,9 +1168,15 @@
             t.first[i] = blocks;
             blocks += ceil_div(Cc[k], 64) * ceil_div(R[k], 64);
             if (inv && tok && tok[k]) t.tok_mask |= 1u << i;
+            if (inv && tok && tok[k] == 2) {
+                HS_REQUIRE(kc && kc_pos, "transpose_bf16_multi: entry %d: chunk-compacted columns need the chunk list", k);
+                t.kc_mask |= 1u << i;
+            }
         }
         t.first[t.count] = blocks;
         t.inv = t.tok_mask ? inv : nullptr;
+        t.kc = t.kc_mask ? kc : nullptr;
+        t.kc_pos = t.kc_mask ? kc_pos : nullptr;
         hipLaunchKernelGGL(transpose_bf16_multi_kernel, dim3(blocks), dim3(256), 0, stream, t);
         HS_LAUNCH_CHECK();
     }
@@ -1150,7 +1202,7 @@
     HS_LAUNCH_CHECK();
     return HS_OK;
 }
-long long bert_row_map_bytes(int B, int L) { return (4ll + (B + 1 + 3) / 4 * 4 + 2ll * B * L) * 4; }
+long long bert_row_map_bytes(int B, int L) { return (4ll + (B + 1 + 3) / 4 * 4 + 2ll * B * L + (((long long)B * L + 31) / 32 + 3) / 4 * 4) * 4; }
 int bert_row_map(const int64_t* mask, int B, int L, int* map, hipStream_t s) {
     HS_REQUIRE(mask && map && B > 0 && L > 0, "bert_row_map: bad argument");
     hipLaunchKernelGGL(bert_row_map_kernel, dim3(1), dim3(256), 0, s, (const long long*)mask, B, L, map);
@@ -1165,11 +1217,11 @@
     return HS_OK;
 }
 int bert_pack_rows(const void* dy, void* dst, long long rows, long long row_bytes, const int* nrows, const int* row_of,
-                   hipStream_t s) {
-    HS_REQUIRE(dy && dst && nrows && row_of && row_bytes % 16 == 0 && al16(dy, dst), "bert_pack_rows: bad argument");
+                   const int* word_src, int* word_dst, hipStream_t s) {
+    HS_REQUIRE(dy && dst && nrows && row_of && row_bytes % 16 == 0 && al16(dy, dst) && (!word_dst || word_src), "bert_pack_rows: bad argument");
     const int cpr = (int)(row_bytes / 16);
     hipLaunchKernelGGL(bert_pack_rows_kernel, dim3(grid_for(rows * cpr)), dim3(256), 0, s, (const u32x4*)dy, (u32x4*)dst, rows, cpr, nrows,
-                       row_of);
+                       row_of, word_src, word_dst);
     HS_LAUNCH_CHECK();
     return HS_OK;
 }
@@ -1411,7 +1463,20 @@
 }
 hs_status hs_transpose_bf16_multi(int32_t count, const void* const* src, void* const* dst, const int32_t* R, const int32_t* Cc,
                                   const int64_t* ld_src, const int64_t* ld_dst, void* stream) {
-    return hs::transpose_bf16_multi_rows(count, src, dst, R, Cc, ld_src, ld_dst, nullptr, nullptr, (hipStream_t)stream);
+    return hs::transpose_bf16_multi_rows(count, src, dst, R, Cc, ld_src, ld_dst, nullptr, nullptr, nullptr, nullptr, (hipStream_t)stream);
+}
+hs_status hs_transpose_bf16_tokens(const void* src, void* dst, int32_t R, int32_t Cc, int64_t ld_src, int64_t ld_dst, const int32_t* packed_of,
+                                   const int32_t* kc_n, const int32_t* kc_pos, void* stream) {
+    HS_REQUIRE(packed_of && (kc_n != nullptr) == (kc_pos != nullptr), "hs_transpose_bf16_tokens: bad argument");
+    const void* s1[1] = {src};
+    void* d1[1] = {dst};
+    const int64_t ls[1] = {ld_src}, ldd[1] = {ld_dst};
+    const unsigned char tok[1] = {(unsigned char)(kc_n ? 2 : 1)};
+    return hs::transpose_bf16_multi_rows(1, s1, d1, &R, &Cc, ls, ldd, packed_of, tok, kc_n, kc_pos, (hipStream_t)stream);
+}
+int64_t hs_bert_row_map_bytes(int32_t B, int32_t L) { return (B > 0 && L > 0) ? hs::bert_row_map_bytes(B, L) : 0; }
+hs_status hs_bert_row_map(const int64_t* mask, int32_t B, int32_t L, int32_t* map, void* stream) {
+    return hs::bert_row_map(mask, B, L, map, (hipStream_t)stream);
 }
 hs_status hs_cross_entropy(const float* logits, const int64_t* labels, const float* weight, float label_smoothing,
                            int32_t B, int32_t C, float* loss, float* dlogits, float* row_loss, void* stream) {
diff --git a/multimodal-diagnosis-ham-spine_amd/hamspine/csrc/gemm.hip b/multimodal-diagnosis-ham-spine_amd/hamspine/csrc/gemm.hip
--- a/multimodal-diagnosis-ham-spine_amd/hamspine/csrc/gemm.hip
+++ b/multimodal-diagnosis-ham-spine_amd/hamspine/csrc/gemm.hip
@@ -1,3 +1,4 @@
+#include <atomic>
 #include <mutex>
 #include <unordered_set>
 #include <vector>
@@ -155,6 +156,7 @@
     return (combo == 0 && (cfg == CFG_64x64 || cfg == CFG_128x64)) || (combo == 3 && (cfg == CFG_64x64 || cfg == CFG_128x64 || cfg == CFG_STEM || cfg == CFG_C3));
 }
 
+static int g_pack_spread = -1;
 struct Prepared {
     GemmArgs a;
     int cfg, combo, split, batch;
@@ -452,6 +454,13 @@
             cnt[{f, p->dtype == HS_BF16 ? 1 : 0}]++;
         }
     }
+    if (a.m_rows) {
+        if (g_pack_spread < 0) {
+            const char* e = getenv("HAMSPINE_PACK_XCD_SPREAD");
+            g_pack_spread = (e && e[0] == '0') ? 0 : 1;
+        }
+        a.pack_spread = (g_pack_spread == 1 && split == 1 && !a.colstats && !a.bnb_partials && !a.stamps && cfg != CFG_C3) ? 1 : 0;
+    }
     dim3 grid(a.tiles_m * a.tiles_n, 1, split > 1 ? split : batch);
     {
         static const bool on = [] { const char* e = getenv("HAMSPINE_PERSISTENT"); return e && e[0] == '1'; }();
@@ -661,7 +670,10 @@
     if (g_group_immediate_hook) HS_PROPAGATE(g_group_immediate_hook(g_group_immediate_ctx));
     return gemm_impl(p, s);
 }
-int gemm_group_add(GemmGroup* g, const hs_gemm_params* p, hipStream_t s) {
+bool gemm_group_takes_k_cols() { return g_dbg_cfg < 0 && !g_dbg_stamps; }
+static std::atomic<long long> g_k_cols_queued{0};
+int gemm_group_add(GemmGroup* g, const hs_gemm_params* p, hipStream_t s, const int* k_cols) {
+    HS_REQUIRE(!k_cols || (g && p && p->a_kind == HS_A_KC && p->b_kind == HS_B_KC), "gemm_group_add: k_cols needs an open group and K-contiguous operands");
     if (!g) return launch_ungrouped(p, s);
     Prepared q;
     const bool big = p->a_kind == HS_A_KC && p->b_kind == HS_B_KC;
@@ -675,6 +687,7 @@
     const bool ok = big ? (q.bf16 && (q.cfg == CFG_256x128 || q.cfg == CFG_P8_256) && q.combo == 0 && q.batch == 1 && q.split == 1 && !q.a.stamps && !q.a.colstats)
                         : (q.bf16 && q.cfg == CFG_64x64 && (q.combo == 2 || q.combo == 5) && q.batch == 1 && !q.a.stamps &&
                            (q.split == 1 || q.a.tickets != nullptr) && !q.a.rowsum[0] && !q.a.colstats);
+    HS_REQUIRE(!k_cols || ok, "gemm_group_add: a problem with chunk-compacted K columns cannot be queued (gemm_group_takes_k_cols)");
     if (!ok) return launch_ungrouped(p, s);
     const long long ngroups = q.split > 1 ? (q.split + kSplitGroup - 1) / kSplitGroup : 0;
     const long long need = q.split > 1 ? (long long)q.a.tiles_m * q.a.tiles_n * (1 + (ngroups > 1 ? ngroups : 0)) : 0;
@@ -683,6 +696,8 @@
         HS_PROPAGATE(gemm_group_flush(g, s));
     }
     if (need > kTicketPool) return launch_ungrouped(p, s);
+    q.a.k_cols = k_cols;
+    if (k_cols) g_k_cols_queued.fetch_add(1, std::memory_order_relaxed);
     g->combo = q.combo;
     if (big) {
         g->cfg = q.cfg;
@@ -703,6 +718,8 @@
 
 extern "C" {
 void hs_gemm_debug_stamps(void* device_buffer) { hs::g_dbg_stamps = (unsigned long long*)device_buffer; }
+void hs_set_pack_xcd_spread(int32_t on) { hs::g_pack_spread = on ? 1 : 0; }
+int64_t hs_gemm_k_cols_queued(void) { return hs::g_k_cols_queued.load(std::memory_order_relaxed); }
 void hs_gemm_debug(int32_t cfg_override, int32_t ablate) {
     hs::g_dbg_cfg = cfg_override;
     hs::g_dbg_ablate = ablate;
diff --git a/multimodal-diagnosis-ham-spine_amd/hamspine/csrc/gemm_core.h b/multimodal-diagnosis-ham-spine_amd/hamspine/csrc/gemm_core.h
--- a/multimodal-diagnosis-ham-spine_amd/hamspine/csrc/gemm_core.h
+++ b/multimodal-diagnosis-ham-spine_amd/hamspine/csrc/gemm_core.h
@@ -69,6 +69,8 @@
     unsigned long long* stamps;
     const int* m_rows;
     const int* drop_rows;
+    int pack_spread;
+    const int* k_cols;
 };
 
 #define HS_STAMP(k)                                                                                              \
@@ -457,14 +459,14 @@
 constexpr bool a_is_rc(int k) { return k == HS_A_RC; }
 constexpr bool b_is_rc(int k) { return k != HS_B_KC; }
 
-__device__ __forceinline__ void tile_from_block(const GemmArgs& a, int& tm, int& tn, int bid) {
-    const int nwg = a.tiles_m * a.tiles_n;
+__device__ __forceinline__ void tile_from_block(const GemmArgs& a, int& tm, int& tn, int bid, int tiles_m) {
+    const int nwg = tiles_m * a.tiles_n;
     const int xcd = bid & 7, q = nwg >> 3, r = nwg & 7;
     const int id = (xcd < r ? xcd * (q + 1) : r * (q + 1) + (xcd - r) * q) + (bid >> 3);
     const int gsz = a.group_m * a.tiles_n;
     const int grp = id / gsz;
     const int first_m = grp * a.group_m;
-    const int gm = min(a.group_m, a.tiles_m - first_m);
+    const int gm = min(a.group_m, tiles_m - first_m);
     const int within = id - grp * gsz;
     tn = within / gm;
     tm = first_m + (within - tn * gm);
@@ -764,13 +766,24 @@
     }
     int m0, n0;
     const int z = bz;
+    int tiles_m = a.tiles_m;
     if (a.m_rows) {
-        tile_from_block(a, tm, tn, bx);
-        if (tm * BM >= __builtin_amdgcn_readfirstlane(a.m_rows[0])) return;
+        const int rows = __builtin_amdgcn_readfirstlane(a.m_rows[0]);
+        if (a.pack_spread) {
+            tiles_m = min(tiles_m, max(0, (rows + BM - 1) / BM));
+            if (bx >= tiles_m * a.tiles_n) return;
+        } else {
+            tile_from_block(a, tm, tn, bx, tiles_m);
+            if (tm * BM >= rows) return;
+        }
     }
 
     long long a_boff = 0, b_boff = 0, d_boff = 0;
     int kbeg = 0, kend = a.K;
+    if (a.k_cols) {
+        const int kc = __builtin_amdgcn_readfirstlane(a.k_cols[0]);
+        kend = min(a.K, max(BK, (kc + BK - 1) / BK * BK));
+    }
     if (a.split_k > 1) {
         kbeg = z * a.k_per_split;
         kend = min(a.K, kbeg + a.k_per_split);
@@ -797,7 +810,7 @@
     int tiles_per_tap = 1;
     bool filtered = false;
     auto setup_tile = [&](const int vb) {
-    tile_from_block(a, tm, tn, vb);
+    tile_from_block(a, tm, tn, vb, tiles_m);
     m0 = tm * BM;
     n0 = tn * BN;
 #pragma unroll
@@ -1500,7 +1513,7 @@
     const int wm = wave >> 1, wn = wave & 1;
     const int l31 = lane & 31, hh = lane >> 5;
     int tm, tn;
-    tile_from_block(a, tm, tn, blockIdx.x);
+    tile_from_block(a, tm, tn, blockIdx.x, a.tiles_m);
     const int m0 = tm * BM, n0 = tn * BN;
     const int z = blockIdx.z;
 
diff --git a/multimodal-diagnosis-ham-spine_amd/hamspine/csrc/gemm_p8.h b/multimodal-diagnosis-ham-spine_amd/hamspine/csrc/gemm_p8.h
--- a/multimodal-diagnosis-ham-spine_amd/hamspine/csrc/gemm_p8.h
+++ b/multimodal-diagnosis-ham-spine_amd/hamspine/csrc/gemm_p8.h
@@ -29,10 +29,16 @@
     const int wm = wave / WGN, wn = wave % WGN;
     const int g = lane >> 4, l15 = lane & 15;
     int tm, tn;
-    tile_from_block(a, tm, tn, bx);
+    int tiles_m = a.tiles_m;
+    if (a.m_rows && a.pack_spread) {
+        tiles_m = min(tiles_m, max(0, (__builtin_amdgcn_readfirstlane(a.m_rows[0]) + BM - 1) / BM));
+        if (bx >= tiles_m * a.tiles_n) return;
+    }
+    tile_from_block(a, tm, tn, bx, tiles_m);
     const int m0 = tm * BM, n0 = tn * BN;
     if (a.m_rows && m0 >= __builtin_amdgcn_readfirstlane(a.m_rows[0])) return;
-    const int ntiles = a.K / BK;
+    int ntiles = a.K / BK;
+    if (a.k_cols) ntiles = max(1, min(ntiles, (__builtin_amdgcn_readfirstlane(a.k_cols[0]) + BK - 1) / BK));
 
     const __amdgpu_buffer_rsrc_t rsA = make_rsrc(a.A, (unsigned)min(a.a_bytes, 0x7fffff00ull));
     const __amdgpu_buffer_rsrc_t rsB = make_rsrc(a.B, (unsigned)min(a.b_bytes, 0x7fffff00ull));
```

Measured after the change: 3188 images/s, median of 6. 4.2% higher.
